# neuroailab/CounterfactualWorldModels

Measured on AMD Instinct MI355X. Metric: predicted frames/sec (2x224x224, ViT-B/8), higher is better.
Workload: dtype bf16; 1 GPU; ViT-base VMAE 8x8, batch=32 synthetic frame pairs (BASELINE configs[1]); predictor=base_8x8patch_2frames_1tube, per_gpu_batch=32, global_batch=32, n_vis=792, mode=parity, lanes=2 (the batch runs as two half batches on two HIP streams inside the library), arithmetic=split-bf16 (hi+lo) MFMA operands, 3 MFMAs/product, fp32 accumulate, parallelism=dp1 (independent frame pairs per rank, no collective), weights=random-init (deterministic synthetic generator)

## Files before the change

counterfactualworldmodels_amd/_lib.py:

```python
from __future__ import annotations

import ctypes as C
import os
import threading
from typing import Optional

import torch

from . import build as _build

MODE_FAST = 1
MODE_PARITY = 2
ERR_INVALID = -1
ERR_HIP = -2
ERR_MASK = -3
KCLASS_GEMM = 0
KCLASS_ATTENTION = 1
KCLASS_GEMM_WIDE = 2
KCLASS_GEMM_NARROW = 3
KCLASS_LAYERNORM, KCLASS_PATCH_GATHER, KCLASS_FILL_MASK, KCLASS_UNEMBED = 4, 5, 6, 7
KCLASS_CROSS_ATTN, KCLASS_SMALL_ATTN = 8, 9

_MODES = {"fast": MODE_FAST, "parity": MODE_PARITY, MODE_FAST: MODE_FAST, MODE_PARITY: MODE_PARITY}

# ... 446 lines not shown
DEV_FLOW_MOTION_STRIDED, DEV_FLOW_MOTION_TILE, DEV_FLOW_MOTION_ROWS16, DEV_FLOW_MOTION_ROWS32, DEV_FLOW_MOTION_ROWS64 = range(5)
DEV_FLOW_COUNT_PLANES, DEV_FLOW_COUNT_PLANES_VEC, DEV_FLOW_COUNT_PACKED, DEV_FLOW_COUNT_PACKED_VEC = range(4)
DEV_FLOW_FINISH_V1, DEV_FLOW_FINISH_V4 = range(2)
DEV_FLOW_ZERO_PLANES, DEV_FLOW_ZERO_PLANES_VEC, DEV_FLOW_ZERO_SCATTER = range(3)
DEV_FLOW_PACK_TRANSPOSE = 0


def new_dev_conj_args(cls):
    a = cls()
    a.struct_size = C.sizeof(cls)
    return a


def new_dev_raft_conv_args() -> CwmDevRaftConvArgs:
    a = CwmDevRaftConvArgs()
    a.struct_size = C.sizeof(CwmDevRaftConvArgs)
    return a


def new_forward_args() -> CwmForwardArgs:
    a = CwmForwardArgs()
    a.struct_size = C.sizeof(CwmForwardArgs)
    return a


def new_conj_forward_args() -> CwmConjForwardArgs:
    a = CwmConjForwardArgs()
    a.struct_size = C.sizeof(CwmConjForwardArgs)
    return a


class CwmKernelStats(C.Structure):
    _fields_ = [("launches", C.c_int64), ("total_ms", C.c_double), ("total_flops", C.c_double)]


SIGNATURES = {
    "cwm_model_create": (C.c_int, [C.POINTER(CwmConfig), C.POINTER(C.c_void_p)]),
    "cwm_model_destroy": (None, [C.c_void_p]),
    "cwm_model_load_weight": (C.c_int, [C.c_void_p, C.c_char_p, C.c_void_p, C.c_int, C.POINTER(C.c_int64), C.c_int]),
    "cwm_model_missing_weights": (C.c_int, [C.c_void_p, C.c_char_p, C.c_int]),
    "cwm_forward": (C.c_int, [C.c_void_p, C.POINTER(CwmForwardArgs)]),
    "cwm_model_set_lanes": (C.c_int, [C.c_void_p, C.c_int]),
    "cwm_model_set_ragged": (C.c_int, [C.c_void_p, C.c_int]),
    "cwm_model_set_option": (C.c_int, [C.c_void_p, C.c_char_p, C.c_int]),
    "cwm_conj_set_option": (C.c_int, [C.c_void_p, C.c_char_p, C.c_int]),
    "cwm_conj_create": (C.c_int, [C.POINTER(CwmConjConfig), C.POINTER(C.c_void_p)]),
    "cwm_conj_create_ex": (C.c_int, [C.POINTER(CwmConjConfig), C.POINTER(CwmConjVariant), C.POINTER(C.c_void_p)]),
    "cwm_conj_destroy": (None, [C.c_void_p]),
    "cwm_conj_load_weight": (C.c_int, [C.c_void_p, C.c_char_p, C.c_void_p, C.c_int, C.POINTER(C.c_int64), C.c_int]),
    "cwm_conj_missing_weights": (C.c_int, [C.c_void_p, C.c_char_p, C.c_int]),
    "cwm_conj_forward": (C.c_int, [C.c_void_p, C.POINTER(CwmConjForwardArgs)]),
    "cwm_conj_set_lanes": (C.c_int, [C.c_void_p, C.c_int]),
    "cwm_conj_timing_enable": (C.c_int, [C.c_void_p, C.c_int, C.c_int]),
    "cwm_conj_timing_collect": (C.c_int, [C.c_void_p, C.c_int, C.POINTER(CwmKernelStats)]),
    "cwm_timing_enable": (C.c_int, [C.c_void_p, C.c_int, C.c_int]),
    "cwm_timing_collect": (C.c_int, [C.c_void_p, C.c_int, C.POINTER(CwmKernelStats)]),
    "cwm_split_bf16": (C.c_int, [C.c_void_p, C.c_int64, C.c_void_p, C.c_void_p, C.c_void_p]),
    "cwm_linear": (
        C.c_int,
        [C.c_void_p, C.c_void_p, C.c_void_p, C.c_void_p, C.c_void_p, C.c_int, C.c_int, C.c_int, C.c_int, C.c_int, C.c_void_p],
    ),
    "cwm_attention": (C.c_int, [C.c_void_p, C.c_void_p, C.c_int, C.c_int, C.c_int, C.c_int, C.c_void_p]),
    "cwm_attention_ragged": (C.c_int, [C.c_void_p, C.c_void_p, C.c_void_p, C.c_int, C.c_int, C.c_int, C.c_int, C.c_void_p]),
    "cwm_layernorm": (C.c_int, [C.c_void_p, C.c_void_p, C.c_void_p, C.c_void_p, C.c_int, C.c_int, C.c_float, C.c_void_p]),
    "cwm_mask_to_perm": (C.c_int, [C.c_void_p, C.c_int, C.c_int, C.c_int, C.c_void_p, C.c_void_p]),
    "cwm_unembed": (
        C.c_int,
        [C.c_void_p, C.c_void_p, C.c_void_p, C.c_int, C.c_int, C.c_int, C.c_int, C.c_int, C.c_int, C.c_int, C.c_void_p, C.c_void_p],
    ),
    "cwm_mask_row_counts": (C.c_int, [C.c_void_p, C.c_int, C.c_int, C.c_void_p, C.c_void_p]),
    "cwm_mask_flip_picks": (C.c_int, [C.c_void_p, C.c_int, C.c_int, C.c_void_p, C.c_int, C.c_void_p]),
    "cwm_prompt_table_expand": (C.c_int, [C.c_void_p] + [C.c_int] * 5 + [C.c_void_p] * 4),
    "cwm_shift_prompts": (
        C.c_int,
        [C.c_void_p] + [C.c_int] * 9 + [C.c_void_p] * 6,
    ),
    "cwm_multi_shift_prompts": (
        C.c_int,
        [C.c_void_p] + [C.c_int] * 10 + [C.c_void_p, C.c_void_p, C.c_int, C.c_void_p, C.c_int] + [C.c_void_p] * 3,
    ),
    "cwm_flow_features": (C.c_int, [C.c_void_p, C.POINTER(C.c_int64)] + [C.c_int] * 6 + [C.c_void_p, C.c_void_p]),
    "cwm_flow_cov": (C.c_int, [C.c_void_p] + [C.c_int] * 6 + [C.c_void_p] * 4),
    "cwm_flow_transform_work_bytes": (C.c_size_t, [C.c_int, C.c_int, C.c_int]),
    "cwm_flow_transform": (C.c_int, [C.c_void_p] + [C.c_int] * 5 + [C.c_float, C.c_int, C.c_int, C.c_float, C.c_void_p, C.c_void_p]),
    "cwm_flow_motion_work_bytes": (C.c_size_t, [C.c_int, C.c_int]),
    "cwm_flow_motion_sum": (C.c_int, [C.c_void_p, C.POINTER(C.c_int64)] + [C.c_int] * 6 + [C.c_float, C.c_void_p, C.c_void_p, C.c_void_p]),
    "cwm_flow_map_finish": (C.c_int, [C.c_void_p, C.c_int, C.c_int, C.c_float, C.c_int, C.c_float, C.c_void_p]),
    "cwm_flow_filter_stats": (C.c_int, [C.c_void_p, C.POINTER(C.c_int64)] + [C.c_int] * 5 + [C.c_void_p, C.POINTER(C.c_int64), C.c_int, C.c_int] + [C.c_float] * 3
                              + [C.c_void_p] * 5),
    "cwm_flow_filter_apply": (C.c_int, [C.c_void_p, C.POINTER(C.c_int64)] + [C.c_int] * 5 + [C.c_void_p, C.c_void_p]),
    "cwm_flow_filter_pack": (C.c_int, [C.c_void_p, C.POINTER(C.c_int64)] + [C.c_int] * 5 + [C.c_void_p, C.c_void_p, C.c_void_p]),
    "cwm_comm_load": (C.c_int, [C.c_char_p]),
    "cwm_comm_version": (C.c_int, []),
    "cwm_comm_unique_id": (C.c_int, [C.c_void_p]),
    "cwm_comm_init": (C.c_int, [C.c_int, C.c_int, C.c_void_p, C.POINTER(C.c_void_p)]),
    "cwm_comm_destroy": (None, [C.c_void_p]),
    "cwm_comm_rank": (C.c_int, [C.c_void_p]),
    "cwm_comm_size": (C.c_int, [C.c_void_p]),
    "cwm_broadcast": (C.c_int, [C.c_void_p, C.c_void_p, C.c_size_t, C.c_int, C.c_void_p]),
    "cwm_allgather": (C.c_int, [C.c_void_p, C.c_void_p, C.c_void_p, C.c_size_t, C.c_void_p]),
    "cwm_allgatherv": (C.c_int, [C.c_void_p, C.c_void_p, C.c_void_p, C.POINTER(C.c_size_t), C.POINTER(C.c_size_t), C.c_void_p]),
    "cwm_allreduce_sum_f32": (C.c_int, [C.c_void_p, C.c_void_p, C.c_size_t, C.c_void_p]),
    "cwm_raft_create": (C.c_int, [C.POINTER(C.c_void_p)]),
    "cwm_raft_destroy": (None, [C.c_void_p]),
    "cwm_raft_load_weight": (C.c_int, [C.c_void_p, C.c_char_p, C.c_void_p, C.c_int, C.POINTER(C.c_int64), C.c_int]),
    "cwm_raft_missing_weights": (C.c_int, [C.c_void_p, C.c_char_p, C.c_int]),
    "cwm_raft_forward": (C.c_int, [C.c_void_p, C.POINTER(CwmRaftForwardArgs)]),
    "cwm_raft_forward_ex": (C.c_int, [C.c_void_p, C.POINTER(CwmRaftForwardExArgs)]),
    "cwm_raft_corr_lookup": (C.c_int, [C.c_void_p, C.c_void_p, C.c_void_p, C.c_int, C.c_int, C.c_int, C.c_void_p, C.c_void_p]),
    "cwm_raft_set_corr": (C.c_int, [C.c_void_p, C.c_int]),
    "cwm_raft_workspace_bytes": (C.c_int, [C.c_void_p, C.POINTER(C.c_uint64)]),
    "cwm_raft_corr_lookup_on_the_fly": (C.c_int, [C.c_void_p, C.c_void_p, C.c_void_p, C.c_int, C.c_int, C.c_int, C.c_void_p, C.c_void_p]),
    "cwm_raft_convex_upsample": (C.c_int, [C.c_void_p, C.c_void_p, C.c_int, C.c_int, C.c_int, C.c_void_p, C.c_void_p]),
    "cwm_raft_head_project": (C.c_int, [C.c_void_p, C.c_void_p, C.c_void_p, C.c_int64, C.c_void_p, C.c_void_p]),
    "cwm_raft_convex_upsample1": (C.c_int, [C.c_void_p, C.c_void_p, C.c_int, C.c_int, C.c_int, C.c_void_p, C.c_void_p]),
    "cwm_raft_forward_interpolate": (C.c_int, [C.c_void_p, C.c_int64, C.c_int64, C.c_int, C.c_int, C.c_int, C.c_void_p, C.c_void_p]),
    "cwm_last_error": (C.c_char_p, []),
    "cwm_version": (C.c_char_p, []),
    "cwm_source_hash": (C.c_char_p, []),
    "cwm_compiler_version": (C.c_char_p, []),
}
DEV_SIGNATURES = {
    "cwm_gemm_tile_override": (C.c_int, [C.c_int] * 6),
    "cwm_dev_gemm_plan": (C.c_int, [C.c_int] * 8 + [C.POINTER(CwmDevGemmPlanOut)]),
    "cwm_dev_flow_forms": (C.c_int, [C.POINTER(C.c_int64)] + [C.c_int] * 5 + [C.c_uint64, C.c_uint64, C.c_int, C.POINTER(C.c_int64), C.c_uint64, C.c_int, C.POINTER(CwmDevFlowFormsOut)]),
    "cwm_bench_gemm": (C.c_int, [C.c_int, C.c_int, C.c_int, C.c_int, C.c_int, C.c_int, C.POINTER(C.c_double)]),
    "cwm_bench_attention": (C.c_int, [C.c_int, C.c_int, C.c_int, C.c_int, C.c_int, C.POINTER(C.c_double)]),
    "cwm_debug_set": (C.c_int, [C.c_char_p, C.c_int]),
    "cwm_debug_get": (C.c_int, [C.c_char_p, C.POINTER(C.c_int)]),
    "cwm_dev_raft_conv": (C.c_int, [C.POINTER(CwmDevRaftConvArgs)]),
    "cwm_dev_raft_corr_lookup_operand": (C.c_int, [C.c_void_p, C.c_void_p, C.c_void_p, C.c_int, C.c_int, C.c_int, C.c_int, C.c_void_p, C.c_void_p]),
    "cwm_dev_raft_corr_lookup_on_the_fly_operand": (C.c_int, [C.c_void_p, C.c_void_p, C.c_void_p, C.c_int, C.c_int, C.c_int, C.c_int, C.c_void_p, C.c_void_p]),
    "cwm_dev_raft_instnorm_stats": (C.c_int, [C.c_void_p, C.c_int, C.c_int, C.c_int, C.c_float, C.c_void_p, C.c_void_p]),
    "cwm_dev_raft_residual_join": (C.c_int, [C.POINTER(CwmDevConvSrc), C.POINTER(CwmDevConvSrc), C.c_int, C.c_int, C.c_void_p, C.c_void_p]),
    "cwm_dev_raft_cnet_split": (C.c_int, [C.c_void_p, C.c_int64, C.c_void_p, C.c_void_p, C.c_void_p]),
    "cwm_dev_raft_motion_finish": (C.c_int, [C.c_void_p, C.c_void_p, C.c_int64, C.c_int, C.c_int, C.c_void_p]),
    "cwm_dev_raft_gru_update": (C.c_int, [C.c_void_p, C.c_void_p, C.c_void_p, C.c_int64, C.c_void_p]),
    "cwm_dev_raft_flow_update": (C.c_int, [C.c_void_p, C.c_void_p, C.c_int, C.c_int64, C.c_void_p]),
    "cwm_dev_gather": (C.c_int, [C.POINTER(CwmDevGatherArgs)]),
    "cwm_dev_conj_cross_attention": (C.c_int, [C.POINTER(CwmDevConjCrossAttentionArgs)]),
    "cwm_dev_conj_small_attention": (C.c_int, [C.POINTER(CwmDevConjSmallAttentionArgs)]),
    "cwm_dev_conj_pad": (C.c_int, [C.POINTER(CwmDevConjPadArgs)]),
    "cwm_dev_gemm": (C.c_int, [C.POINTER(CwmDevGemmArgs)]),
    "cwm_dev_attention": (C.c_int, [C.POINTER(CwmDevAttentionArgs)]),
    "cwm_dev_layernorm": (C.c_int, [C.POINTER(CwmDevLayernormArgs)]),
    "cwm_dev_fill_mask_tokens": (C.c_int, [C.c_void_p] * 4 + [C.c_int] * 4 + [C.c_void_p]),
    "cwm_dev_unembed": (C.c_int, [C.c_void_p, C.c_void_p] + [C.c_int64] * 3 + [C.c_void_p] + [C.c_int] * 7 + [C.c_void_p, C.c_void_p]),
    "cwm_dev_gather_ragged": (C.c_int, [C.POINTER(CwmDevGatherArgs), C.c_int, C.c_void_p]),
    "cwm_dev_attention_ragged": (C.c_int, [C.POINTER(CwmDevAttentionArgs), C.c_void_p]),
    "cwm_dev_fill_mask_tokens_ragged": (C.c_int, [C.c_void_p] * 5 + [C.c_int] * 4 + [C.c_void_p]),
    "cwm_dev_unembed_ragged": (C.c_int, [C.c_void_p, C.c_void_p] + [C.c_int64] * 3 + [C.c_void_p] + [C.c_int] * 8 + [C.c_void_p, C.c_void_p]),
}

OPTION_KEYS = ("gemm_tile", "gemm_debug", "gemm_staged", "gemm_direct", "attn_kernel", "attn_remap", "attn_tail", "attn_ksplit", "prune_last_block", "index_fused",
               "min_lane_rows", "conj_ctx_stream", "conj_attn")
GEMM_DEBUG_TIMING_ONLY = 1 | 2 | 8


def validate_option(key: str, value: int) -> None:
    if key not in OPTION_KEYS:
        raise CwmHipError(-1, "unknown option %s (known: %s)" % (key, ", ".join(OPTION_KEYS)))
    if key == "gemm_debug" and int(value) & GEMM_DEBUG_TIMING_ONLY:
        raise CwmHipError(-1, "gemm_debug bits 1, 2 and 8 are timing-only ablations (wrong outputs): development library only (cwm_debug_set)")


_lib: Optional[C.CDLL] = None
_dev_lib: Optional[C.CDLL] = None
_lock = threading.Lock()


class CwmHipError(RuntimeError):
    def __init__(self, code: int, msg: str):
        super().__init__(msg)
        self.code = code


def library_path() -> str:
    return os.environ.get("CWM_HIP_LIB", _build.LIB_PATH)


def get_lib() -> C.CDLL:
    global _lib
    if _lib is not None:
        return _lib
    with _lock:
        if _lib is not None:
            return _lib
        path = library_path()
        if not os.path.exists(path):
            try:
                _build.build_library()
            except Exception as e:
                raise RuntimeError(
                    "libcwm_hip.so is missing at %s and could not be built (%s). "
                    "Run `python -m counterfactualworldmodels_amd.build`." % (path, e)
                )
        lib = _bind(path)
        if path == _build.LIB_PATH and os.path.isdir(_build.CSRC):
            want = _build.source_hash()
            if lib.cwm_source_hash().decode() != want:
                try:
                    _build.build_library(force=False)
                except Exception as e:
                    raise RuntimeError("libcwm_hip.so at %s was built from other sources (%s != %s) and could not be rebuilt: %s"
                                       % (path, lib.cwm_source_hash().decode(), want, e))
                import _ctypes

                _ctypes.dlclose(lib._handle)
                lib = _bind(path)
                if lib.cwm_source_hash().decode() != want:
                    raise RuntimeError("libcwm_hip.so still does not match the sources after a rebuild")
        _warn_if_unlinted_compiler(lib)
        _lib = lib
        return lib


def _warn_if_unlinted_compiler(lib) -> None:
    try:
        rec = _build.lint_record().get("hipcc")
        comp = lib.cwm_compiler_version().decode()
    except Exception:
        return
    if rec and comp and rec != comp:
        import warnings

        warnings.warn("libcwm_hip.so was compiled by `%s`, but the ISA lint of its hand-counted waits last passed on `%s`: run `python tools/asm_lds_lint.py --record` "
                      "(and the GPU soak, tests/test_soak_gpu.py) before trusting this build" % (comp, rec), RuntimeWarning, stacklevel=3)


def dev_library_path() -> str:
    p = library_path()
    return os.environ.get("CWM_HIP_DEV_LIB", _build.DEV_LIB_PATH if p == _build.LIB_PATH else p[:-3] + "_dev.so")


def get_dev_lib() -> C.CDLL:
    global _dev_lib
    if _dev_lib is not None:
        return _dev_lib
    get_lib()
    with _lock:
        if _dev_lib is None:
            path = dev_library_path()
            if not os.path.exists(path):
                raise RuntimeError("libcwm_hip_dev.so is missing at %s: run `python -m counterfactualworldmodels_amd.build`" % path)
            lib = _bind(path, dict(SIGNATURES, **DEV_SIGNATURES))
            if path == _build.DEV_LIB_PATH and os.path.isdir(_build.CSRC) and lib.cwm_source_hash().decode() != _build.source_hash():
                raise RuntimeError("libcwm_hip_dev.so at %s was built from other sources than the tree holds: run `python -m counterfactualworldmodels_amd.build`" % path)
            _dev_lib = lib
    return _dev_lib


def _bind(path: str, signatures=None) -> C.CDLL:
    lib = C.CDLL(path)
    for name, (res, args) in (signatures or SIGNATURES).items():
        try:
            fn = getattr(lib, name)
        except AttributeError:
            if name == "cwm_source_hash":
                lib.cwm_source_hash = lambda: b"pre-hash"
                continue
            raise
        fn.restype = res
        fn.argtypes = args
    return lib


def check(rc: int, lib: Optional[C.CDLL] = None) -> None:
    if rc != 0:
        msg = (lib or get_lib()).cwm_last_error()
        if not msg and lib is None and _dev_lib is not None:
            msg = _dev_lib.cwm_last_error()
        raise CwmHipError(rc, (msg.decode() if msg else "") + " [cwm_hip rc=%d]" % rc)


def require_gpu() -> None:
    if not torch.cuda.is_available():
        raise RuntimeError(
            "counterfactualworldmodels_amd runs its predictor on an AMD GPU through libcwm_hip.so; "
            "no HIP device is visible and there is no CPU fallback."
        )


def ptr(t: Optional[torch.Tensor]) -> Optional[int]:
    return None if t is None else t.data_ptr()


def current_stream_handle(device=None) -> int:
    return torch.cuda.current_stream(device).cuda_stream
```

counterfactualworldmodels_amd/csrc/dev.hip:

```cpp
#include <atomic>
#include <map>
#include <mutex>
#include <tuple>

#include "../../include/cwm_hip_dev.h"
#include "engine.h"
#include "flow_view.h"

using namespace cwm;

void cwm_set_pretend_device(int d);

namespace {
__global__ void fill_random_bf16_kernel(bf16* dst, int64_t n, unsigned seed, float scale) {
    const int64_t i = (int64_t)blockIdx.x * blockDim.x + threadIdx.x;
    if (i >= n) return;
    unsigned x = (unsigned)i * 2654435761u + seed;
    x ^= x >> 16; x *= 0x7feb352du; x ^= x >> 15; x *= 0x846ca68bu; x ^= x >> 16;
    dst[i] = (bf16)(((float)(x & 0xFFFF) / 32768.0f - 1.0f) * scale);
}
__global__ void fill_random_f32_kernel(float* dst, int64_t n, unsigned seed, float scale) {
    const int64_t i = (int64_t)blockIdx.x * blockDim.x + threadIdx.x;
    if (i >= n) return;
    unsigned x = (unsigned)i * 2654435761u + seed;
// ... 425 lines not shown
    }
    if (rc) return rc;
    CWM_HIP_CHECK(hipStreamSynchronize(s));
    return CWM_OK;
}

extern "C" int cwm_dev_gather(const cwm_dev_gather_args* args) { return dev_gather(args, false, 0, nullptr); }

extern "C" int cwm_dev_gather_ragged(const cwm_dev_gather_args* args, int n_vis_min, int32_t* counts_dev) { return dev_gather(args, true, n_vis_min, counts_dev); }

namespace {
template <int PLANES>
__global__ void stage_operand_kernel(const float* src, int64_t rows, int K, bf16* out) {
    const int64_t i = ((int64_t)blockIdx.x * blockDim.x + threadIdx.x) * 4;
    if (i >= rows * K) return;
    const int64_t r = i / K;
    store_operand4<PLANES>(out, r, K, (int)(i - r * K), *reinterpret_cast<const f32x4*>(src + i));
}
int stage_operand(const float* src, int64_t rows, int K, bf16* out, int planes, hipStream_t s) {
    const unsigned grid = (unsigned)((rows * K / 4 + 255) / 256);
    if (planes == 2)
        hipLaunchKernelGGL(stage_operand_kernel<2>, dim3(grid), dim3(256), 0, s, src, rows, K, out);
    else
        hipLaunchKernelGGL(stage_operand_kernel<1>, dim3(grid), dim3(256), 0, s, src, rows, K, out);
    CWM_HIP_CHECK(hipGetLastError());
    return 0;
}
}

extern "C" int cwm_dev_conj_cross_attention(const cwm_dev_conj_cross_attention_args* args) {
    CWM_REQUIRE(args && args->struct_size == sizeof(cwm_dev_conj_cross_attention_args),
                "cwm_dev_conj_cross_attention: args->struct_size must be sizeof(cwm_dev_conj_cross_attention_args)");
    const cwm_dev_conj_cross_attention_args& a = *args;
    hipStream_t s = (hipStream_t)a.stream;
    CWM_REQUIRE(a.mode == CWM_MODE_FAST || a.mode == CWM_MODE_PARITY, "cwm_dev_conj_cross_attention: bad mode");
    const int planes = a.mode == CWM_MODE_PARITY ? 2 : 1;
    CWM_REQUIRE(a.impl == CWM_DEV_CONJ_VALU || a.impl == CWM_DEV_CONJ_MFMA, "cwm_dev_conj_cross_attention: unknown impl %d", a.impl);
    const bool mfma = a.impl == CWM_DEV_CONJ_MFMA;
    CWM_REQUIRE(a.roles >= 1 && a.roles <= 3 && (mfma || a.roles == 3), "cwm_dev_conj_cross_attention: roles = %d (MFMA: 1, 2 or 3; VALU: 3)", a.roles);
    CWM_REQUIRE(a.qk && a.v && a.qk_src && a.v_src && a.y && a.y_src, "cwm_dev_conj_cross_attention: null argument");
    CWM_REQUIRE(a.B > 0 && a.N > 0 && a.M > 0 && a.heads > 0 && a.head_dim > 0 && (int64_t)a.B * a.N * 4 * a.heads * a.head_dim < (1ll << 31),
                "cwm_dev_conj_cross_attention: bad geometry");
    const int D = a.heads * a.head_dim;
    CWM_REQUIRE(D % 32 == 0, "cwm_dev_conj_cross_attention: operand rows of %d columns (need a multiple of 32)", D);
    if (mfma) {
        CWM_REQUIRE(cross_attention_mfma_ok(a.head_dim, a.M), "cwm_dev_conj_cross_attention: the MFMA form has no kernel for head_dim %d, M %d", a.head_dim, a.M);
        CWM_REQUIRE(cross_attention_mfma_fits(a.B, a.N, a.heads, a.head_dim), "cwm_dev_conj_cross_attention: too large for the MFMA form's 32-bit offsets");
    } else {
        CWM_REQUIRE(cross_attention_ok(a.M, a.head_dim), "cwm_dev_conj_cross_attention: the VALU form refuses M %d, head_dim %d (%zu bytes of LDS)", a.M, a.head_dim,
                    cross_attention_lds_bytes(a.M, a.head_dim));
    }
    const int64_t rows = (int64_t)a.B * a.N;
    Scratch sc;
    CrossAttnParams p;
    memset(&p, 0, sizeof(p));
    p.qk = a.qk, p.v = a.v, p.qk_src = a.qk_src, p.v_src = a.v_src;
    p.B = a.B, p.N = a.N, p.M = a.M, p.heads = a.heads, p.head_dim = a.head_dim, p.scale = a.scale;
    p.y = (bf16*)a.y, p.y_plane = rows * D, p.y_src = (bf16*)a.y_src, p.y_src_plane = (int64_t)a.B * a.M * D;
    int rc;
    if (mfma) {
        bf16* qk_op = sc.get<bf16>((size_t)rows * 2 * D * planes);
        bf16* v_op = sc.get<bf16>((size_t)rows * D * planes);
        p.partial = sc.get<float>(cross_attention_mfma_partial_floats(a.B, a.heads, a.M, a.head_dim));
        CWM_REQUIRE(qk_op && v_op && p.partial, "cwm_dev_conj_cross_attention: out of device memory");
        if ((rc = stage_operand(a.qk, rows, 2 * D, qk_op, planes, s)) || (rc = stage_operand(a.v, rows, D, v_op, planes, s))) return rc;
        p.qk_op = qk_op, p.v_op = v_op;
        if ((rc = launch_cross_attention_mfma_roles(p, planes, s, s, a.roles))) return rc;
    } else {
        p.scores_t = sc.get<float>((size_t)a.B * a.heads * a.M * a.N);
        p.partial = sc.get<float>(cross_attention_partial_floats(a.B, a.heads, a.M, a.head_dim));
        CWM_REQUIRE(p.scores_t && p.partial, "cwm_dev_conj_cross_attention: out of device memory");
        if ((rc = launch_cross_attention(p, planes, s))) return rc;
    }
    CWM_HIP_CHECK(hipStreamSynchronize(s));
    return CWM_OK;
}

extern "C" int cwm_dev_conj_small_attention(const cwm_dev_conj_small_attention_args* args) {
    CWM_REQUIRE(args && args->struct_size == sizeof(cwm_dev_conj_small_attention_args),
                "cwm_dev_conj_small_attention: args->struct_size must be sizeof(cwm_dev_conj_small_attention_args)");
    const cwm_dev_conj_small_attention_args& a = *args;
    hipStream_t s = (hipStream_t)a.stream;
    CWM_REQUIRE(a.mode == CWM_MODE_FAST || a.mode == CWM_MODE_PARITY, "cwm_dev_conj_small_attention: bad mode");
    const int planes = a.mode == CWM_MODE_PARITY ? 2 : 1;
    CWM_REQUIRE(a.impl == CWM_DEV_CONJ_VALU || a.impl == CWM_DEV_CONJ_MFMA, "cwm_dev_conj_small_attention: unknown impl %d", a.impl);
    CWM_REQUIRE(a.qkv && a.o && a.B > 0 && a.heads > 0, "cwm_dev_conj_small_attention: bad argument");
    CWM_REQUIRE(a.n_tok > 0 && a.n_tok <= 64 && a.head_dim > 0 && a.head_dim <= 64, "cwm_dev_conj_small_attention: needs n_tok <= 64 and head_dim <= 64 (got %d, %d)",
                a.n_tok, a.head_dim);
    CWM_REQUIRE(a.impl == CWM_DEV_CONJ_VALU || small_attention_mfma_ok(a.n_tok, a.head_dim), "cwm_dev_conj_small_attention: the MFMA form needs head_dim 32 (got %d)",
                a.head_dim);
    const int D = a.heads * a.head_dim;
    CWM_REQUIRE(D % 4 == 0 && a.ldo % 32 == 0 && a.ldo >= D, "cwm_dev_conj_small_attention: %d columns in operand rows of ldo = %d (a multiple of 32)", D, a.ldo);
    SmallAttnParams p;
    memset(&p, 0, sizeof(p));
    p.qkv = a.qkv;
    p.B = a.B, p.n_tok = a.n_tok, p.heads = a.heads, p.head_dim = a.head_dim;
    p.o = (bf16*)a.o, p.o_plane = (int64_t)a.B * a.n_tok * a.ldo, p.ldo = a.ldo;
    if (int rc = a.impl == CWM_DEV_CONJ_MFMA ? launch_small_attention_mfma(p, planes, s) : launch_small_attention(p, planes, s)) return rc;
    CWM_HIP_CHECK(hipStreamSynchronize(s));
    return CWM_OK;
}

extern "C" int cwm_dev_conj_pad(const cwm_dev_conj_pad_args* args) {
    CWM_REQUIRE(args && args->struct_size == sizeof(cwm_dev_conj_pad_args), "cwm_dev_conj_pad: args->struct_size must be sizeof(cwm_dev_conj_pad_args)");
    const cwm_dev_conj_pad_args& a = *args;
    hipStream_t s = (hipStream_t)a.stream;
    CWM_REQUIRE(a.B > 0, "cwm_dev_conj_pad: bad batch");
    int rc = 0;
    if (a.kind == CWM_DEV_CONJ_PAD_MASK) {
        CWM_REQUIRE(a.mask && a.ext_mask && a.N > 0 && a.P >= 0 && a.vmax >= 0, "cwm_dev_conj_pad: bad pad-mask argument");
        rc = launch_pad_mask(a.mask, a.B, a.N, a.P, a.vmax, a.ext_mask, s);
    } else if (a.kind == CWM_DEV_CONJ_FIX_PAD_ROWS) {
        CWM_REQUIRE(a.x && a.perm && a.token && a.n_rows > 0 && a.D > 0 && a.perm_stride >= a.n_rows && a.n_real >= 0, "cwm_dev_conj_pad: bad fix-pad-rows argument");
        rc = launch_fix_pad_rows(a.x, a.perm, a.B, a.perm_stride, a.n_rows, a.n_real, a.D, a.token, s);
    } else if (a.kind == CWM_DEV_CONJ_ZERO_PAD_OUT_ROWS) {
        CWM_REQUIRE(a.x && a.perm && a.n_rows > 0 && a.D > 0 && a.n_vis >= 0 && a.perm_stride >= a.n_vis + a.n_rows && a.n_real >= 0,
                    "cwm_dev_conj_pad: bad zero-pad-out-rows argument");
        rc = launch_zero_pad_out_rows(a.x, a.perm, a.B, a.perm_stride, a.n_vis, a.n_rows, a.n_real, a.D, s);
    } else if (a.kind == CWM_DEV_CONJ_IMU_APPEND_DUMMY) {
        CWM_REQUIRE(a.imu && a.mask && a.dummy && a.out && a.ext_mask && a.C > 0 && a.L > 0 && a.T > 0 && a.N > 0, "cwm_dev_conj_pad: bad append-dummy argument");
        rc = launch_imu_append_dummy(a.imu, a.mask, a.dummy, a.B, a.C, a.L, a.T, a.N, a.out, a.ext_mask, s);
    } else {
        CWM_REQUIRE(false, "cwm_dev_conj_pad: unknown kind %d", a.kind);
    }
    if (rc) return rc;
    CWM_HIP_CHECK(hipStreamSynchronize(s));
    return CWM_OK;
}

extern "C" int cwm_dev_gemm(const cwm_dev_gemm_args* args) {
    CWM_REQUIRE(args && args->struct_size == sizeof(cwm_dev_gemm_args), "cwm_dev_gemm: args->struct_size must be sizeof(cwm_dev_gemm_args)");
    const cwm_dev_gemm_args& a = *args;
    hipStream_t s = (hipStream_t)a.stream;
    CWM_REQUIRE(a.mode == CWM_MODE_FAST || a.mode == CWM_MODE_PARITY, "cwm_dev_gemm: bad mode");
    const int planes = a.mode == CWM_MODE_PARITY ? 2 : 1;
    CWM_REQUIRE(a.a && a.w && a.M > 0 && a.N > 0 && a.K > 0 && a.epi >= EPI_F32 && a.epi <= EPI_QKV, "cwm_dev_gemm: bad argument");
    CWM_REQUIRE(a.rows_in >= 0 && a.out_row_offset >= 0 && (a.rows_in > 0 || (!a.resid_rowmap && a.out_row_offset == 0)),
                "cwm_dev_gemm: a row map or row offset needs rows_in > 0");
    if (a.rows_in > 0) {
        CWM_REQUIRE(a.M % a.rows_in == 0 && a.rows_in + a.out_row_offset <= a.rows_out, "cwm_dev_gemm: %d rows as samples of %d rows at offset %d of %d", a.M,
                    a.rows_in, a.out_row_offset, a.rows_out);
        CWM_REQUIRE(!a.resid_rowmap || a.map_stride >= a.rows_in, "cwm_dev_gemm: a residual row map of %d entries per sample for %d rows", a.map_stride, a.rows_in);
    }
    GemmParams p;
    memset(&p, 0, sizeof(p));
    p.M = a.M; p.N = a.N; p.K = p.lda = round_up(a.K, 64);
    p.epi = a.epi;
    p.rows_in = a.rows_in; p.rows_out = a.rows_out; p.out_row_offset = a.out_row_offset; p.map_stride = a.map_stride; p.resid_rowmap = a.resid_rowmap;
    if (a.epi == EPI_F32) {
        CWM_REQUIRE(a.C && a.ldc >= a.N && (!a.resid || a.ldr >= a.N), "cwm_dev_gemm: the fp32 output needs C and rows of at least N columns");
        CWM_REQUIRE(!a.resid_rowmap || a.resid, "cwm_dev_gemm: a residual row map without a residual");
        p.C = a.C; p.ldc = a.ldc; p.resid = a.resid; p.ldr = a.ldr;
    } else if (a.epi == EPI_QKV) {
        CWM_REQUIRE(a.q_out && a.k_out && a.v_out && a.heads > 0 && a.head_dim > 0 && a.n_tok > 0 && a.N == 3 * a.heads * a.head_dim && a.M % a.n_tok == 0,
                    "cwm_dev_gemm: the Q/K/V scatter needs the three outputs, N = 3 * heads * head_dim and whole samples of n_tok rows");
        CWM_REQUIRE(planes == 1 || a.qk_plane >= (int64_t)a.M * a.heads * a.head_dim, "cwm_dev_gemm: the lo plane would overlap the hi plane");
        p.q_out = (bf16*)a.q_out; p.k_out = (bf16*)a.k_out; p.v_out = (bf16*)a.v_out; p.qk_plane = a.qk_plane;
        p.qkv_dim = a.heads * a.head_dim; p.heads = a.heads; p.head_dim = a.head_dim; p.n_tok = a.n_tok; p.q_scale = a.q_scale;
    } else {
        CWM_REQUIRE(a.out && a.ldo >= a.N, "cwm_dev_gemm: the operand output needs out and rows of at least N columns");
        p.out_hi = (bf16*)a.out; p.ldo = a.ldo;
    }
    p.tune = &thread_tuning();
    GemmPlan plan;
    if (int rc = gemm_plan(p, planes, 0, gemm_cu_count(), &plan)) return rc;
    if (a.plan_forms) a.plan_forms[0] = plan.staged, a.plan_forms[1] = plan.direct;
    Scratch sc;
    LinearOperands op;
    if (int rc = stage_linear_operands(sc, "cwm_dev_gemm", a.a, a.w, a.bias, a.M, a.N, a.K, planes, s, &op)) return rc;
    p.A = op.A; p.W = op.W;
    p.bias = a.bias ? op.bias : nullptr;
    if (int rc = launch_gemm(p, planes, s)) return rc;
    CWM_HIP_CHECK(hipStreamSynchronize(s));
    return CWM_OK;
}

static int dev_attention(const cwm_dev_attention_args* args, const int* key_len) {
    CWM_REQUIRE(args && args->struct_size == sizeof(cwm_dev_attention_args), "cwm_dev_attention: args->struct_size must be sizeof(cwm_dev_attention_args)");
    const cwm_dev_attention_args& a = *args;
    CWM_REQUIRE(!key_len || a.n_q == 0, "cwm_dev_attention: per-row key counts (key_len) go with queries over all rows (n_q = 0), got n_q = %d", a.n_q);
    hipStream_t s = (hipStream_t)a.stream;
    CWM_REQUIRE(a.mode == CWM_MODE_FAST || a.mode == CWM_MODE_PARITY, "cwm_dev_attention: bad mode");
    const int planes = a.mode == CWM_MODE_PARITY ? 2 : 1;
    CWM_REQUIRE(a.qkv && a.o && a.B > 0 && a.N > 0 && a.H > 0, "cwm_dev_attention: bad argument");
    CWM_REQUIRE(a.q_off >= 0 && a.n_q >= 0 && a.q_off + a.n_q <= a.N && (a.n_q > 0 || a.q_off == 0), "cwm_dev_attention: query rows [%d, %d) of %d tokens", a.q_off,
                a.q_off + a.n_q, a.N);
    const int D = a.H * 64;
    CWM_REQUIRE(a.ldo >= D && a.ldo % (planes == 2 ? 32 : 4) == 0, "cwm_dev_attention: %d columns in operand rows of ldo = %d (a multiple of 32 in parity mode, of 4 in fast mode)",
                D, a.ldo);
    const int64_t qk_plane = (int64_t)a.B * a.N * D;
    Scratch sc;
    bf16* q = sc.get<bf16>(2 * qk_plane);
    bf16* k = sc.get<bf16>(2 * qk_plane);
    bf16* v = sc.get<bf16>(2 * qk_plane);
    CWM_REQUIRE(q && k && v, "cwm_dev_attention: out of device memory");
    if (int rc = launch_qkv_scatter(a.qkv, a.B, a.N, a.H, 0.125f, q, k, v, qk_plane, s)) return rc;
    AttnParams p;
    memset(&p, 0, sizeof(p));
    p.q = q; p.k = k; p.v = v; p.qk_plane = qk_plane;
    p.o = (bf16*)a.o; p.o_plane = (int64_t)a.B * (a.n_q ? a.n_q : a.N) * a.ldo; p.ldo = a.ldo;
    p.n_tok = a.N; p.heads = a.H; p.batch = a.B;
    p.q_off = a.q_off; p.n_q = a.n_q;
    p.key_len = key_len;
    p.tune = &thread_tuning();
    if (int rc = launch_attention(p, planes, s)) return rc;
    CWM_HIP_CHECK(hipStreamSynchronize(s));
    return CWM_OK;
}

extern "C" int cwm_dev_attention(const cwm_dev_attention_args* args) { return dev_attention(args, nullptr); }

extern "C" int cwm_dev_attention_ragged(const cwm_dev_attention_args* args, const int32_t* key_len_dev) {
    CWM_REQUIRE(key_len_dev, "cwm_dev_attention_ragged: null key_len_dev");
    return dev_attention(args, key_len_dev);
}

extern "C" int cwm_dev_layernorm(const cwm_dev_layernorm_args* args) {
    CWM_REQUIRE(args && args->struct_size == sizeof(cwm_dev_layernorm_args), "cwm_dev_layernorm: args->struct_size must be sizeof(cwm_dev_layernorm_args)");
    const cwm_dev_layernorm_args& a = *args;
    hipStream_t s = (hipStream_t)a.stream;
    CWM_REQUIRE(a.mode == CWM_MODE_FAST || a.mode == CWM_MODE_PARITY, "cwm_dev_layernorm: bad mode");
    const int planes = a.mode == CWM_MODE_PARITY ? 2 : 1;
    CWM_REQUIRE(a.x && a.gamma && a.beta && a.out && a.rows > 0 && a.D > 0 && a.ldx >= a.D, "cwm_dev_layernorm: bad argument");
    CWM_REQUIRE(a.rows_out_per_b >= 0 && a.in_offset >= 0 &&
                    (a.rows_out_per_b == 0 ? a.in_offset == 0 : a.rows % a.rows_out_per_b == 0 && a.in_offset + a.rows_out_per_b <= a.rows_in_per_b),
                "cwm_dev_layernorm: %d rows as samples of %d rows at offset %d of %d", a.rows, a.rows_out_per_b, a.in_offset, a.rows_in_per_b);
    LayerNormParams ln;
    memset(&ln, 0, sizeof(ln));
    ln.x = a.x; ln.ldx = a.ldx; ln.gamma = a.gamma; ln.beta = a.beta; ln.eps = a.eps; ln.D = a.D; ln.rows = a.rows;
    ln.rows_out_per_b = a.rows_out_per_b; ln.rows_in_per_b = a.rows_in_per_b; ln.in_offset = a.in_offset;
    ln.out = (bf16*)a.out; ln.out_plane = (int64_t)a.rows * a.ldo; ln.ldo = a.ldo; ln.out_f32 = a.out_f32;
    if (int rc = launch_layernorm(ln, planes, s)) return rc;
    CWM_HIP_CHECK(hipStreamSynchronize(s));
    return CWM_OK;
}

extern "C" int cwm_dev_fill_mask_tokens(float* x_full_dev, const float* mask_token_dev, const float* pos_dev, const int32_t* perm_dev, int B, int Nt, int n_vis,
                                        int D, void* stream) {
    CWM_REQUIRE(x_full_dev && mask_token_dev && pos_dev && perm_dev && B > 0 && D > 0 && n_vis >= 0 && n_vis <= Nt, "cwm_dev_fill_mask_tokens: bad argument");
    if (int rc = launch_fill_mask_tokens(x_full_dev, mask_token_dev, pos_dev, perm_dev, B, Nt, n_vis, D, (hipStream_t)stream)) return rc;
    CWM_HIP_CHECK(hipStreamSynchronize((hipStream_t)stream));
    return CWM_OK;
}

extern "C" int cwm_dev_fill_mask_tokens_ragged(float* x_full_dev, const float* mask_token_dev, const float* pos_dev, const int32_t* perm_dev,
                                               const int32_t* counts_dev, int B, int Nt, int n_vis_min, int D, void* stream) {
    CWM_REQUIRE(x_full_dev && mask_token_dev && pos_dev && perm_dev && B > 0 && Nt > 0 && D > 0, "cwm_dev_fill_mask_tokens_ragged: bad argument");
    if (int rc = launch_fill_mask_tokens_ragged(x_full_dev, mask_token_dev, pos_dev, perm_dev, counts_dev, B, Nt, n_vis_min, D, (hipStream_t)stream)) return rc;
    CWM_HIP_CHECK(hipStreamSynchronize((hipStream_t)stream));
    return CWM_OK;
}

static int dev_unembed(const float* y_tokens_dev, const float* x_dev, int64_t x_stride_b, int64_t x_stride_c, int64_t x_stride_t, const uint8_t* mask_dev, int B, int T,
                       int C, int H, int W, int P, int n_vis_min, int n_vis, float* out_dev, void* stream) {
    CWM_REQUIRE(y_tokens_dev && x_dev && mask_dev && out_dev && B > 0 && T > 0 && C > 0 && H > 0 && W > 0, "cwm_dev_unembed: bad argument");
    CWM_REQUIRE(P > 0 && H % P == 0 && W % P == 0, "cwm_dev_unembed: image size must be divisible by the patch size");
    CWM_REQUIRE(x_stride_c >= (int64_t)H * W && x_stride_t >= 0 && x_stride_b >= 0, "cwm_dev_unembed: channel planes of %d x %d pixels at a stride of %lld", H, W,
                (long long)x_stride_c);
    const int Nt = T * (H / P) * (W / P);
    CWM_REQUIRE(n_vis >= 0 && n_vis <= Nt, "cwm_dev_unembed: n_vis = %d of %d tokens", n_vis, Nt);
    hipStream_t s = (hipStream_t)stream;
    Scratch sc;
    int* perm = sc.get<int>((size_t)B * Nt);
    int* rank = sc.get<int>((size_t)B * Nt);
    int* err = sc.get<int>(4, true);
    int* counts = sc.get<int>((size_t)B);
    CWM_REQUIRE(perm && rank && err && counts, "cwm_dev_unembed: out of device memory");
    int rc;
    if ((rc = n_vis_min > 0 ? launch_mask_to_perm_ragged(mask_dev, B, Nt, n_vis_min, n_vis, perm, err, counts, s) : launch_mask_to_perm(mask_dev, B, Nt, n_vis, perm, err, s)))
        return rc;
    const int y0 = n_vis_min > 0 ? n_vis_min : n_vis;
    if ((rc = launch_perm_to_rank(perm, rank, B, Nt, s))) return rc;
    UnembedParams u;
    memset(&u, 0, sizeof(u));
    u.y = y_tokens_dev; u.x = x_dev; u.sb = x_stride_b; u.st = x_stride_t; u.sc = x_stride_c;
    u.mask = mask_dev; u.rank = rank; u.B = B; u.T = T; u.C = C; u.H = H; u.W = W; u.P = P; u.n_vis = y0; u.Nm = Nt - y0; u.out = out_dev;
    if ((rc = launch_unembed(u, s))) return rc;
    int herr = 0;
    CWM_HIP_CHECK(hipMemcpyAsync(&herr, err, sizeof(int), hipMemcpyDeviceToHost, s));
    CWM_HIP_CHECK(hipStreamSynchronize(s));
    if (herr) {
        if (n_vis_min > 0)
            cwm_set_error("mask rows do not all have between %d and n_vis=%d visible tokens", n_vis_min, n_vis);
        else
            cwm_set_error("mask rows do not all have n_vis=%d visible tokens", n_vis);
        return CWM_ERR_MASK;
    }
    return CWM_OK;
}

extern "C" int cwm_dev_unembed(const float* y_tokens_dev, const float* x_dev, int64_t x_stride_b, int64_t x_stride_c, int64_t x_stride_t, const uint8_t* mask_dev,
                               int B, int T, int C, int H, int W, int P, int n_vis, float* out_dev, void* stream) {
    return dev_unembed(y_tokens_dev, x_dev, x_stride_b, x_stride_c, x_stride_t, mask_dev, B, T, C, H, W, P, 0, n_vis, out_dev, stream);
}

extern "C" int cwm_dev_unembed_ragged(const float* y_tokens_dev, const float* x_dev, int64_t x_stride_b, int64_t x_stride_c, int64_t x_stride_t, const uint8_t* mask_dev,
                                      int B, int T, int C, int H, int W, int P, int n_vis_min, int n_vis, float* out_dev, void* stream) {
    CWM_REQUIRE(n_vis_min > 0, "cwm_dev_unembed_ragged: n_vis_min = %d (a ragged batch has a least count > 0)", n_vis_min);
    return dev_unembed(y_tokens_dev, x_dev, x_stride_b, x_stride_c, x_stride_t, mask_dev, B, T, C, H, W, P, n_vis_min, n_vis, out_dev, stream);
}
```

counterfactualworldmodels_amd/csrc/elementwise.hip:

```cpp
#include "common.h"
#include "kernels.h"
#include <algorithm>

namespace cwm {

template <int PLANES>
__global__ __launch_bounds__(256) void layernorm_kernel(const LayerNormParams p) {
    constexpr int MAXI = 2;
    const int lane = threadIdx.x & 63;
    const int r = blockIdx.x * 4 + (threadIdx.x >> 6);
    if (r >= p.rows) return;
    int in_row = r;
    if (p.rows_out_per_b > 0) {
        const int b = r / p.rows_out_per_b;
        in_row = b * p.rows_in_per_b + p.in_offset + (r - b * p.rows_out_per_b);
    }
    const float* x = p.x + (size_t)in_row * p.ldx;
    f32x4 v[MAXI][2];
    float s = 0.f;
#pragma unroll
    for (int i = 0; i < MAXI; ++i) {
        const int idx = lane * 8 + i * 512;
        if (idx < p.D) {
            v[i][0] = *reinterpret_cast<const f32x4*>(x + idx);
// ... 228 lines not shown
}

template <int PLANES>
__global__ __launch_bounds__(256) void index_gather_kernel(const PatchGatherParams p, const uint8_t* __restrict__ mask, int n_vis, int* __restrict__ perm_out,
                                                           int* __restrict__ rank_out, int* __restrict__ err_rows, int n_vis_min, int* __restrict__ counts) {
    extern __shared__ int vis_tab[];
    __shared__ int wave_tot[4];
    const int b = blockIdx.y, t = threadIdx.x;
    const int L = p.perm_stride ? p.perm_stride : p.Nt;
    const uint8_t* m = mask + (size_t)b * L;
    const int nw = min((int)gridDim.x, 256);
    const bool writer = (t % nw) == (int)blockIdx.x;
    int* pr = perm_out + (size_t)b * L;
    int* rk = rank_out ? rank_out + (size_t)b * L : nullptr;
    const bool vec = (L & 15) == 0 && L <= 256 * 32 && ((uintptr_t)mask & 15) == 0;
    const int per = !vec ? (L + 255) / 256 : L <= 256 * 16 ? 16 : 32;
    const int lo = min(t * per, L), hi = min(lo + per, L);
    u32x4 w0 = u32x4{0x01010101u, 0x01010101u, 0x01010101u, 0x01010101u}, w1 = w0;
    int c = 0;
    if (vec) {
        if (lo < L) w0 = *reinterpret_cast<const u32x4*>(m + lo);
        if (per == 32 && lo + 16 < L) w1 = *reinterpret_cast<const u32x4*>(m + lo + 16);
        auto zero_bytes = [](unsigned x) {
            const unsigned y = (x & 0x7F7F7F7Fu) + 0x7F7F7F7Fu;
            return __popc(~(y | x | 0x7F7F7F7Fu));
        };
#pragma unroll
        for (int q = 0; q < 4; ++q) c += zero_bytes(w0[q]) + zero_bytes(w1[q]);
    } else {
        for (int i = lo; i < hi; ++i) c += (m[i] == 0);
    }
    int total_vis;
    int v = block_exclusive_scan256(c, wave_tot, total_vis);
    auto emit = [&](int i, bool visible) {
        if (visible) {
            if (v < p.n_rows) vis_tab[v] = i;
            if (writer) {
                pr[v] = i;
                if (rk) rk[i] = v;
            }
            ++v;
        } else if (writer) {
            const int pos = total_vis + (i - v);
            pr[pos] = i;
            if (rk) rk[i] = pos;
        }
    };
    if (vec) {
#pragma unroll
        for (int k = 0; k < 32; ++k) {
            if (k < hi - lo) {
                const unsigned word = k < 16 ? w0[(k >> 2) & 3] : w1[(k >> 2) & 3];
                emit(lo + k, ((word >> (8 * (k & 3))) & 0xFFu) == 0);
            }
        }
    } else {
        for (int i = lo; i < hi; ++i) emit(i, m[i] == 0);
    }
    if (blockIdx.x == 0 && t == 0) {
        err_rows[b] = (n_vis_min > 0 ? (total_vis < n_vis_min || total_vis > n_vis) : total_vis != n_vis) ? 1 : 0;
        if (counts) counts[b] = total_vis;
    }
    __syncthreads();

    const int per_row = p.C * p.P;
    const int total = p.n_rows * per_row;
    for (int gid = blockIdx.x * 256 + t; gid < total; gid += gridDim.x * 256) {
        const int i = gid / per_row;
        patch_gather_item<PLANES>(p, b, (int64_t)b * p.n_rows + i, gid - i * per_row, i < total_vis ? vis_tab[i] : p.Nt);
    }
}

int launch_index_gather(const PatchGatherParams& p, const uint8_t* mask, int n_vis, int* perm, int* rank, int* err_rows, int planes, hipStream_t stream,
                        int n_vis_min, int* counts) {
    CWM_REQUIRE(n_vis_min == 0 || (n_vis_min > 0 && n_vis_min <= n_vis && counts), "index_gather: ragged rows need 0 < n_vis_min <= n_vis and a count array");
    CWM_REQUIRE(p.P % 4 == 0 && p.W % 4 == 0, "index_gather: patch size and width must be multiples of 4");
    CWM_REQUIRE(p.C == 3 || !p.normalize, "index_gather: imagenet normalisation needs 3 channels");
    CWM_REQUIRE(p.ld >= p.C * p.P * p.P && p.ld % 4 == 0, "index_gather: bad ld");
    CWM_REQUIRE(mask && perm && err_rows && p.n_rows > 0 && p.n_rows <= 12000, "index_gather: bad argument (rows per sample: %d)", p.n_rows);
    const int per_sample = (p.n_rows * p.C * p.P + 255) / 256;
    const dim3 grid((unsigned)per_sample, (unsigned)p.B);
    const size_t smem = (size_t)p.n_rows * sizeof(int);
    if (planes == 1)
        hipLaunchKernelGGL(index_gather_kernel<1>, grid, dim3(256), smem, stream, p, mask, n_vis, perm, rank, err_rows, n_vis_min, counts);
    else
        hipLaunchKernelGGL(index_gather_kernel<2>, grid, dim3(256), smem, stream, p, mask, n_vis, perm, rank, err_rows, n_vis_min, counts);
    CWM_HIP_CHECK(hipGetLastError());
    return 0;
}

__global__ __launch_bounds__(256) void fill_mask_tokens4_kernel(float* x_full, const float* mask_token, const float* pos, const int* perm, int Nt,
                                                                 int n_vis, int D, int64_t rows, int64_t rows_q) {
    const int d4 = D / 4;
    const int64_t gid = (int64_t)blockIdx.x * blockDim.x + threadIdx.x;
    if (gid >= rows_q * d4) return;
    const int64_t r0 = gid / d4;
    const int c4 = (int)(gid - r0 * d4);
    const int nm = Nt - n_vis;
    const float4 mt = *reinterpret_cast<const float4*>(mask_token + c4 * 4);
    constexpr int R = 8;
    size_t orow[R];
    int tau[R];
    bool live[R];
#pragma unroll
    for (int i = 0; i < R; ++i) {
        const int64_t row = r0 + i * rows_q;
        live[i] = row < rows;
        const int64_t rr = live[i] ? row : 0;
        const int b = (int)(rr / nm), j = (int)(rr - (int64_t)b * nm);
        orow[i] = (size_t)b * Nt + n_vis + j;
        tau[i] = perm[orow[i]];
    }
    float4 pe[R];
#pragma unroll
    for (int i = 0; i < R; ++i) pe[i] = *reinterpret_cast<const float4*>(pos + (size_t)tau[i] * D + c4 * 4);
#pragma unroll
    for (int i = 0; i < R; ++i)
        if (live[i]) *reinterpret_cast<float4*>(x_full + orow[i] * D + c4 * 4) = make_float4(mt.x + pe[i].x, mt.y + pe[i].y, mt.z + pe[i].z, mt.w + pe[i].w);
}

int launch_fill_mask_tokens(float* x_full, const float* mask_token, const float* pos, const int* perm, int B, int Nt, int n_vis, int D, hipStream_t stream) {
    CWM_REQUIRE(D % 4 == 0, "fill_mask_tokens: D must be a multiple of 4");
    const int64_t rows = (int64_t)B * (Nt - n_vis), rows_q = (rows + 7) / 8;
    if (rows == 0) return 0;
    hipLaunchKernelGGL(fill_mask_tokens4_kernel, dim3((unsigned)((rows_q * (D / 4) + 255) / 256)), dim3(256), 0, stream, x_full, mask_token, pos, perm, Nt,
                       n_vis, D, rows, rows_q);
    CWM_HIP_CHECK(hipGetLastError());
    return 0;
}

__global__ __launch_bounds__(256) void fill_mask_tokens_ragged_kernel(float* x_full, const float* mask_token, const float* pos, const int* perm,
                                                                      const int* counts, int Nt, int n_vis_min, int D, int64_t total) {
    const int d4 = D / 4;
    const int64_t gid = (int64_t)blockIdx.x * blockDim.x + threadIdx.x;
    if (gid >= total) return;
    const int64_t row = gid / d4;
    const int c4 = (int)(gid - row * d4);
    const int nm = Nt - n_vis_min;
    const int b = (int)(row / nm), j = n_vis_min + (int)(row - (int64_t)b * nm);
    if (j < counts[b]) return;
    const size_t orow = (size_t)b * Nt + j;
    const float4 mt = *reinterpret_cast<const float4*>(mask_token + c4 * 4);
    const float4 pe = *reinterpret_cast<const float4*>(pos + (size_t)perm[orow] * D + c4 * 4);
    *reinterpret_cast<float4*>(x_full + orow * D + c4 * 4) = make_float4(mt.x + pe.x, mt.y + pe.y, mt.z + pe.z, mt.w + pe.w);
}

int launch_fill_mask_tokens_ragged(float* x_full, const float* mask_token, const float* pos, const int* perm, const int* counts, int B, int Nt, int n_vis_min,
                                   int D, hipStream_t stream) {
    CWM_REQUIRE(D % 4 == 0 && counts && n_vis_min > 0 && n_vis_min <= Nt, "fill_mask_tokens (ragged): bad argument");
    const int64_t total = (int64_t)B * (Nt - n_vis_min) * (D / 4);
    if (total == 0) return 0;
    hipLaunchKernelGGL(fill_mask_tokens_ragged_kernel, dim3((unsigned)((total + 255) / 256)), dim3(256), 0, stream, x_full, mask_token, pos, perm, counts, Nt,
                       n_vis_min, D, total);
    CWM_HIP_CHECK(hipGetLastError());
    return 0;
}

struct __attribute__((packed, aligned(4))) Float4A4 {
    float v[4];
};

__global__ __launch_bounds__(256) void unembed_kernel(const UnembedParams p) {
    const int w4 = p.W / 4;
    const int64_t total = (int64_t)p.B * p.T * p.C * p.H * w4;
    const int64_t gid = (int64_t)blockIdx.x * blockDim.x + threadIdx.x;
    if (gid >= total) return;
    int64_t r = gid;
    const int x4 = (int)(r % w4); r /= w4;
    const int y = (int)(r % p.H); r /= p.H;
    const int c = (int)(r % p.C); r /= p.C;
    const int t = (int)(r % p.T);
    const int b = (int)(r / p.T);
    const int x0 = x4 * 4;
    const int gw = p.W / p.P;
    const int n = (p.H / p.P) * gw;
    const int Nt = p.T * n;
    const int tau = t * n + (y / p.P) * gw + (x0 / p.P);
    Float4A4 o;
    if (p.mask[(size_t)b * Nt + tau]) {
        const int j = max(p.rank[(size_t)b * Nt + tau] - p.n_vis, 0);
        const float* yp = p.y + ((size_t)b * p.Nm + j) * (p.P * p.P * p.C) + ((y % p.P) * p.P + (x0 % p.P)) * p.C + c;
        o = Float4A4{{yp[0], yp[p.C], yp[2 * p.C], yp[3 * p.C]}};
    } else {
        o = *reinterpret_cast<const Float4A4*>(p.x + b * p.sb + t * p.st + c * p.sc + (int64_t)y * p.W + x0);
    }
    *reinterpret_cast<Float4A4*>(p.out + ((((size_t)b * p.T + t) * p.C + c) * p.H + y) * p.W + x0) = o;
}

__global__ __launch_bounds__(256) void unembed3_kernel(const UnembedParams p) {
    const int w4 = p.W / 4, hh = p.H / 2;
    const int64_t total = (int64_t)p.B * p.T * hh * w4;
    const int64_t gid = (int64_t)blockIdx.x * blockDim.x + threadIdx.x;
    if (gid >= total) return;
    int64_t r = gid;
    const int x4 = (int)(r % w4); r /= w4;
    const int y0 = (int)(r % hh); r /= hh;
    const int t = (int)(r % p.T);
    const int b = (int)(r / p.T);
    const int x0 = x4 * 4;
    const int gw = p.W / p.P;
    const int n = (p.H / p.P) * gw;
    const int Nt = p.T * n;
    float4 o[2][3];
#pragma unroll
    for (int k = 0; k < 2; ++k) {
        const int y = y0 + k * hh;
        const int tau = t * n + (y / p.P) * gw + (x0 / p.P);
        if (p.mask[(size_t)b * Nt + tau]) {
            const int j = max(p.rank[(size_t)b * Nt + tau] - p.n_vis, 0);
            const float4* yp = reinterpret_cast<const float4*>(p.y + ((size_t)b * p.Nm + j) * (p.P * p.P * 3) + ((y % p.P) * p.P + (x0 % p.P)) * 3);
            const float4 a = yp[0], bb = yp[1], c = yp[2];
            o[k][0] = make_float4(a.x, a.w, bb.z, c.y);
            o[k][1] = make_float4(a.y, bb.x, bb.w, c.z);
            o[k][2] = make_float4(a.z, bb.y, c.x, c.w);
        } else {
            const float* src = p.x + b * p.sb + t * p.st + (int64_t)y * p.W + x0;
#pragma unroll
            for (int c = 0; c < 3; ++c) o[k][c] = *reinterpret_cast<const float4*>(src + c * p.sc);
        }
    }
#pragma unroll
    for (int k = 0; k < 2; ++k) {
        float* dst = p.out + (((size_t)b * p.T + t) * 3 * p.H + y0 + k * hh) * p.W + x0;
#pragma unroll
        for (int c = 0; c < 3; ++c) {
            const f32x4 v = f32x4{o[k][c].x, o[k][c].y, o[k][c].z, o[k][c].w};
            __builtin_nontemporal_store(v, reinterpret_cast<f32x4*>(dst + (size_t)c * p.H * p.W));
        }
    }
}

int launch_unembed(const UnembedParams& p, hipStream_t stream) {
    CWM_REQUIRE(p.P % 4 == 0 && p.W % 4 == 0, "unembed: patch size and width must be multiples of 4");
    if (p.C == 3 && p.H % 2 == 0 && (((uintptr_t)p.y | (uintptr_t)p.out | (uintptr_t)p.x) & 15) == 0 && (p.sc % 4 == 0) && (p.sb % 4 == 0) && (p.st % 4 == 0)) {
        const int64_t total3 = (int64_t)p.B * p.T * (p.H / 2) * (p.W / 4);
        hipLaunchKernelGGL(unembed3_kernel, dim3((unsigned)((total3 + 255) / 256)), dim3(256), 0, stream, p);
        CWM_HIP_CHECK(hipGetLastError());
        return 0;
    }
    const int64_t total = (int64_t)p.B * p.T * p.C * p.H * (p.W / 4);
    hipLaunchKernelGGL(unembed_kernel, dim3((unsigned)((total + 255) / 256)), dim3(256), 0, stream, p);
    CWM_HIP_CHECK(hipGetLastError());
    return 0;
}

__global__ __launch_bounds__(256) void shift_prompts_x_kernel(const ShiftPromptParams p) {
    const int w4 = p.W / 4, h4 = p.H / 4;
    const int64_t total = (int64_t)p.B * p.S * p.T * p.C * h4 * w4;
    const int64_t gid = (int64_t)blockIdx.x * blockDim.x + threadIdx.x;
    if (gid >= total) return;
    int64_t r = gid;
    const int x4 = (int)(r % w4); r /= w4;
    const int yq = (int)(r % h4); r /= h4;
    const int c = (int)(r % p.C); r /= p.C;
    const int t = (int)(r % p.T);
    const int i = (int)(r / p.T);
    const int b = i / p.S;
    const int x0 = x4 * 4, y = yq * 4;
    int ft = p.fix_passive == 1 ? 0 : t;
    int sy = y, sx = x0;
    const int gw = p.W / p.P, gh = p.H / p.P, n = gh * gw;
    if (t == p.frame) {
        const int dy = p.shifts[2 * i], dx = p.shifts[2 * i + 1];
        const int pi = y / p.P - dy, pj = x0 / p.P - dx;
        if (pi >= 0 && pi < gh && pj >= 0 && pj < gw && p.active[(size_t)i * p.T * n + (size_t)p.frame * n + pi * gw + pj] == 0) {
            sy = y - dy * p.P;
            sx = x0 - dx * p.P;
        }
    }
    if (p.fix_passive == 2) {
        if (p.masks[(size_t)i * p.T * n + (size_t)t * n + (sy / p.P) * gw + sx / p.P] == 0) ft = 0;
    }
    const float* src = p.x + ((((size_t)b * p.T + ft) * p.C + c) * p.H + sy) * p.W + sx;
    float* dst = p.x_out + ((((size_t)i * p.T + t) * p.C + c) * p.H + y) * p.W + x0;
    f32x4 v[4];
#pragma unroll
    for (int k = 0; k < 4; ++k) v[k] = *reinterpret_cast<const f32x4*>(src + (size_t)k * p.W);
#pragma unroll
    for (int k = 0; k < 4; ++k) __builtin_nontemporal_store(v[k], reinterpret_cast<f32x4*>(dst + (size_t)k * p.W));
}

__global__ __launch_bounds__(256) void shift_prompts_mask_kernel(const ShiftPromptParams p) {
    const int gw = p.W / p.P, gh = p.H / p.P, n = gh * gw, Nt = p.T * n;
    const int64_t total = (int64_t)p.B * p.S * Nt;
    const int64_t gid = (int64_t)blockIdx.x * blockDim.x + threadIdx.x;
    if (gid >= total) return;
    const int i = (int)(gid / Nt), tau = (int)(gid - (int64_t)i * Nt);
    const int t = tau / n, hw = tau - t * n;
    const uint8_t act = p.active[gid];
    const uint8_t m1 = act ? p.masks[gid] : 1;
    uint8_t mp = act;
    if (t == p.frame) {
        const int dy = p.shifts[2 * i], dx = p.shifts[2 * i + 1];
        const int pi = hw / gw - dy, pj = hw % gw - dx;
        mp = (pi >= 0 && pi < gh && pj >= 0 && pj < gw) ? p.active[(size_t)i * Nt + (size_t)t * n + pi * gw + pj] : 1;
    }
    p.mask_out[gid] = (m1 && mp) ? 1 : 0;
}

__global__ __launch_bounds__(256) void prompt_table_expand_kernel(const int* __restrict__ table, int S, int gh, int gw, int T, int frame, uint8_t* __restrict__ active,
                                                                  uint8_t* __restrict__ passive, int* __restrict__ shifts) {
    const int n = gh * gw;
    const int Nt = T * n;
    const int64_t gid = (int64_t)blockIdx.x * blockDim.x + threadIdx.x;
    if (gid >= (int64_t)S * Nt) return;
    const int i = (int)(gid / Nt), tau = (int)(gid - (int64_t)i * Nt);
// ... 223 lines not shown
```

counterfactualworldmodels_amd/csrc/engine.h:

```cpp
#pragma once
#include <math.h>
#include <stdio.h>
#include <string.h>

#include <algorithm>
#include <map>
#include <string>
#include <vector>

#include "../../include/cwm_hip.h"
#include "common.h"
#include "kernels.h"

namespace cwm {

static inline int round_up(int v, int m) { return (v + m - 1) / m * m; }

struct LinearW {
    bf16* w = nullptr;
    bf16* w_il = nullptr;
    int64_t plane = 0;
    int N = 0, K = 0, Npad = 0, Kpad = 0;
    float* bias = nullptr;
};

struct BlockW {
    float *ln1_g = nullptr, *ln1_b = nullptr, *ln2_g = nullptr, *ln2_b = nullptr;
    LinearW qkv, proj, fc1, fc2;
};

enum SlotKind { SLOT_MATRIX, SLOT_VECTOR, SLOT_IGNORED };

struct Slot {
    SlotKind kind = SLOT_VECTOR;
    std::vector<int64_t> shape;
    LinearW* lin = nullptr;
    float* dst = nullptr;
    int repeat = 1;
    int64_t numel = 0;
    bool loaded = false;
    bool optional = false;
};

struct EventPair {
    hipEvent_t a, b;
    double flops;
    int sub;
};

struct KernelTimer {
    bool enabled = false;
    std::vector<EventPair> pool;
    size_t used = 0;
    cwm_kernel_stats acc = {0, 0.0, 0.0};
};

struct StreamBuffers {
    bf16 *hbuf = nullptr, *gbuf = nullptr, *qbuf = nullptr, *kbuf = nullptr, *vbuf = nullptr;
    float* qkv_f32 = nullptr;
};

struct StreamW {
    int enc_dim = 0, dec_dim = 0, enc_heads = 0, dec_heads = 0, n_tok = 0, max_pad = 0, out_dim = 0, embed_k = 0, embed_kpad = 0;
    std::vector<BlockW> enc, dec;
    LinearW embed, e2d, head;
    float *enc_norm_g = nullptr, *enc_norm_b = nullptr, *dec_norm_g = nullptr, *dec_norm_b = nullptr;
    float *mask_token = nullptr, *null_enc = nullptr;
    float *pos_enc_ext = nullptr, *pos_dec_ext = nullptr;
    int n_slots() const { return n_tok + max_pad; }
};

struct StreamWs {
    uint8_t* ext_mask = nullptr;
    int* perm = nullptr;
    bf16* tokens_in = nullptr;
    float *x_enc = nullptr, *x_dec = nullptr;
    StreamBuffers sb;
};

template <typename Visit>
int for_each_stream_buffer(const StreamW& S, StreamWs& w, int vcap, int mlp_ratio, bool small, Visit&& visit) {
    const size_t rows_e = (size_t)vcap, rows_d = (size_t)S.n_slots();
    const size_t act = std::max(rows_e * S.enc_dim, rows_d * S.dec_dim);
    int rc;
    if ((rc = visit(w.ext_mask, rows_d)) || (rc = visit(w.perm, rows_d)) || (rc = visit(w.tokens_in, 2 * rows_e * S.embed_kpad)) ||
        (rc = visit(w.x_enc, rows_e * S.enc_dim)) || (rc = visit(w.x_dec, rows_d * S.dec_dim)) || (rc = visit(w.sb.hbuf, 2 * act)) ||
        (rc = visit(w.sb.gbuf, 2 * act * mlp_ratio)))
        return rc;
    if (small) return visit(w.sb.qkv_f32, 3 * act);
    if ((rc = visit(w.sb.qbuf, 2 * act)) || (rc = visit(w.sb.kbuf, 2 * act))) return rc;
    return visit(w.sb.vbuf, 2 * act);
}

constexpr int kMinLaneRows = 3000;
constexpr int kMinLaneRowsConj = 12000;

struct Lanes {
    static constexpr int kMax = 4;
    hipStream_t streams[kMax - 1] = {};
    hipEvent_t ev_fork = nullptr, ev_join[kMax - 1] = {};
    int forked = 1;
    ~Lanes();
    int fork(hipStream_t caller, int n_lanes);
    hipStream_t stream(int l, hipStream_t caller) const { return l == 0 ? caller : streams[l - 1]; }
    int join(hipStream_t caller);
};

struct Engine {
    int device = 0;
    int overlapped = 0;
    Tuning tune = thread_tuning();
    float ln_eps = 1e-6f;
    std::map<std::string, Slot> slots;
    uint64_t loads = 0;
    std::vector<void*> allocs;
    std::vector<void*> ws_allocs;
    uint64_t ws_bytes = 0;
    KernelTimer timers[CWM_KCLASS_COUNT];
    struct SplitKWs {
        float* slabs;
        unsigned* counts;
        uint64_t last_use;
    };
    uint64_t splitk_clock = 0;
    static constexpr size_t kMaxSplitKStreams = 8;
    std::map<hipStream_t, SplitKWs> splitk_ws;

    ~Engine();
    int alloc(void** p, size_t bytes, bool zero, bool workspace);
    template <typename T>
    int ws(T** p, size_t count) {
        void* v = nullptr;
        if (int rc = alloc(&v, count * sizeof(T), true, true)) return rc;
        *p = (T*)v;
        return 0;
    }
    int free_workspace();

    int make_linear(LinearW& L, int N, int K, bool bias);
    int make_vec(float** v, int n);
    void add_matrix_slot(const std::string& key, LinearW* L, std::vector<int64_t> shape);
    void add_vec_slot(const std::string& key, float* dst, std::vector<int64_t> shape, int repeat = 1);
    void add_ignored_slot(const std::string& key, std::vector<int64_t> shape);
    int make_block(BlockW& b, const std::string& pre, int D, int hidden);
    int make_sinusoid(float** dst, int n_pos, int d, int extra_rows = 0);
    int make_pos_embedding_f32(float** dst, int n_pos, int d, int extra_rows = 0);
    int make_stream(StreamW& S, const std::string& pre, int embed_k, std::vector<int64_t> embed_shape, int depth_e, int depth_d, int mlp_ratio,
                    bool sinusoid_f64, bool null_tokens);

    int load_weight(const char* key, const float* data, int on_device, const int64_t* shape, int ndim);
    int missing_weights(char* buf, int buflen);
    int require_weights(const char* fn);
    int set_option(const char* fn, const char* key, int value);

    int run_gemm(const GemmParams& p, int planes, hipStream_t s);
    int attach_splitk_workspace(GemmParams& p, hipStream_t s);
    int run_attention(const AttnParams& p, int planes, hipStream_t s);
    int run_layernorm(const LayerNormParams& p, int planes, hipStream_t s);
    int run_patch_gather(const PatchGatherParams& p, int planes, hipStream_t s);
    int run_index_gather(const PatchGatherParams& p, const uint8_t* mask, int n_vis, int* perm, int* rank, int* err_rows, int planes, hipStream_t s,
                         int n_vis_min = 0, int* counts = nullptr);
    int run_fill_mask_tokens(float* x_full, const float* mask_token, const float* pos, const int* perm, int B, int Nt, int n_vis, int D, hipStream_t s);
    int run_unembed(const UnembedParams& p, hipStream_t s);
    template <typename F>
    int timed(int kclass, double work, hipStream_t s, F&& launch) {
        EventPair* e = nullptr;
        if (int rc = timer_begin(kclass, work, s, &e)) return rc;
        if (int rc = launch()) return rc;
        return timer_end(e, s);
    }
    int timer_begin(int kclass, double work, hipStream_t s, EventPair** out);
    int timer_end(EventPair* e, hipStream_t s);
    int layernorm_to(const float* x, int rows, int D, const float* g, const float* b, bf16* out, int planes, hipStream_t s);
    int linear_f32(const bf16* A, int rows, int K, const LinearW& L, float* C, const float* resid, int planes, hipStream_t s);
    int linear_operand(const bf16* A, int rows, int K, const LinearW& L, bf16* out, int planes, hipStream_t s);
    int linear_gelu(const bf16* A, int rows, int K, const LinearW& L, bf16* out, int planes, hipStream_t s);
    int run_mlp(const float* ln_g, const float* ln_b, const LinearW& fc1, const LinearW& fc2, float* x, int B, int n_tok, int D, int planes, StreamBuffers& sb,
                hipStream_t s, int n_keep = 0);
    int run_block(const BlockW& w, float* x, int B, int n_tok, int D, int H, int planes, StreamBuffers& sb, hipStream_t s, int n_keep = 0,
                  const int* key_len = nullptr);
    int run_block_small(const BlockW& w, float* x, int B, int n_tok, int D, int H, int planes, StreamBuffers& sb, hipStream_t s);
    int embed_stream(const StreamW& S, const StreamWs& w, int B, int n_vis, int planes, hipStream_t s);
    int to_decoder(const StreamW& S, const StreamWs& w, int B, int n_vis, int planes, hipStream_t s, const int* counts = nullptr, int n_vis_min = 0);
    int head_rows(const StreamW& S, const StreamWs& w, int B, int n_out, float* out, int planes, hipStream_t s);

    int timing_enable(int kclass, int enable);
    int timing_collect(int kclass, cwm_kernel_stats* out);
};

template <typename Args>
int copy_args(Args& dst, const Args* src, size_t min_size, const char* fn, const char* note = "") {
    CWM_REQUIRE(src->struct_size >= min_size && src->struct_size <= 4096, "%s: args->struct_size = %u is not a %s_args (set it to sizeof(%s_args)%s)", fn,
                src->struct_size, fn, fn, note);
    memset(&dst, 0, sizeof(dst));
    memcpy(&dst, src, std::min<size_t>(src->struct_size, sizeof(dst)));
    return 0;
}

struct WsAlloc {
    Engine& E;
    size_t batch;
    template <typename T>
    int operator()(T*& p, size_t per_b) const { return E.ws(&p, per_b * batch); }
};
struct WsShift {
    size_t b0;
    template <typename T>
    int operator()(T*& p, size_t per_b) const {
        p += per_b * b0;
        return 0;
    }
};

GemmParams gemm_base(const bf16* A, int lda, const LinearW& L, int M, int planes);

int launch_pack_weight(const float* src, int N, int K, bf16* hi, bf16* il, int Npad, int Kpad, hipStream_t stream);

struct Scratch {
    std::vector<void*> ptrs;
    ~Scratch() {
        for (void* p : ptrs) (void)hipFree(p);
    }
    template <typename T>
    T* get(size_t count, bool zero = false) {
        void* p = nullptr;
        if (hipMalloc(&p, count * sizeof(T) + 16) != hipSuccess) return nullptr;
        ptrs.push_back(p);
        if (zero) (void)hipMemset(p, 0, count * sizeof(T));
        return (T*)p;
    }
};
struct LinearOperands {
    bf16 *A, *W;
    float* bias;
    int Kp, Np;
};
int stage_linear_operands(Scratch& sc, const char* who, const float* a, const float* w, const float* bias, int M, int N, int K, int planes, hipStream_t s,
                          LinearOperands* out);
int launch_qkv_scatter(const float* qkv, int B, int N, int H, float scale, bf16* q, bf16* k, bf16* v, int64_t qk_plane, hipStream_t s);

}
```

counterfactualworldmodels_amd/csrc/engine.hip:

```cpp
#include <stdarg.h>

#include "engine.h"

using namespace cwm;

static thread_local char g_err[1024] = "";

void cwm_set_error(const char* fmt, ...) {
    va_list ap;
    va_start(ap, fmt);
    vsnprintf(g_err, sizeof(g_err), fmt, ap);
    va_end(ap);
}

extern "C" const char* cwm_last_error(void) { return g_err; }

#include <mutex>
#include <set>
int cwm_set_max_lds(const void* kernel, int bytes) {
    static std::mutex mu;
    static std::set<std::pair<int, const void*>> done;
    int dev = 0;
    CWM_HIP_CHECK(hipGetDevice(&dev));
    std::lock_guard<std::mutex> lock(mu);
    if (done.count({dev, kernel})) return 0;
    CWM_HIP_CHECK(hipFuncSetAttribute(kernel, hipFuncAttributeMaxDynamicSharedMemorySize, bytes));
    done.insert({dev, kernel});
    return 0;
}
static thread_local int g_pretend_device = -1;
void cwm_set_pretend_device(int d) { g_pretend_device = d; }
int cwm_require_device(int handle_device, const char* what) {
    int cur = -1;
    CWM_HIP_CHECK(hipGetDevice(&cur));
    if (g_pretend_device >= 0) cur = g_pretend_device;
    CWM_REQUIRE(cur == handle_device, "%s: the handle was created on HIP device %d but the calling thread's current device is %d (hipSetDevice(%d) first)", what,
                handle_device, cur, handle_device);
    return 0;
}
extern "C" const char* cwm_version(void) { return "cwm_hip 0.10.4 gfx950"; }
#ifndef CWM_SRC_HASH
#define CWM_SRC_HASH "unknown"
#endif
extern "C" const char* cwm_source_hash(void) { return CWM_SRC_HASH; }
#ifndef CWM_HIPCC_VERSION
#define CWM_HIPCC_VERSION "unknown"
#endif
extern "C" const char* cwm_compiler_version(void) { return CWM_HIPCC_VERSION; }

namespace cwm {

const Tuning& default_tuning() {
    static const Tuning t;
    return t;
}
Tuning& thread_tuning() {
    static thread_local Tuning t;
    return t;
}
namespace {
struct TuningField { const char* name; int Tuning::*member; };
}
static const TuningField* tuning_field(const char* key) {
    typedef TuningField Field;
    static const Field fields[] = {{"gemm_tile", &Tuning::gemm_tile}, {"gemm_debug", &Tuning::gemm_debug}, {"gemm_staged", &Tuning::gemm_staged},
                                   {"gemm_direct", &Tuning::gemm_direct}, {"attn_kernel", &Tuning::attn_kernel}, {"attn_remap", &Tuning::attn_remap},
                                   {"attn_tail", &Tuning::attn_tail}, {"attn_ksplit", &Tuning::attn_ksplit}, {"prune_last_block", &Tuning::prune_last_block}, {"index_fused", &Tuning::index_fused},
                                   {"min_lane_rows", &Tuning::min_lane_rows}, {"conj_ctx_stream", &Tuning::conj_ctx_stream}, {"conj_attn", &Tuning::conj_attn}};
    for (const Field& f : fields)
        if (!strcmp(key, f.name)) return &f;
    return nullptr;
}
int tuning_set(Tuning& t, const char* key, int value) {
    const TuningField* f = tuning_field(key);
    if (!f) return -1;
    t.*(f->member) = value;
    return 0;
}
int tuning_set_production(Tuning& t, const char* key, int value) {
    if (!strcmp(key, "gemm_debug") && (value & (1 | 2 | 8))) return -2;
    return tuning_set(t, key, value);
}
int tuning_get(const Tuning& t, const char* key, int* value) {
    const TuningField* f = tuning_field(key);
    if (!f) return -1;
    *value = t.*(f->member);
    return 0;
}

__global__ void pack_weight_kernel(const float* src, int N, int K, bf16* hi, bf16* il, int Npad, int Kpad) {
    const int64_t i = (int64_t)blockIdx.x * blockDim.x + threadIdx.x;
    if (i >= (int64_t)Npad * Kpad) return;
    const int n = (int)(i / Kpad), k = (int)(i - (int64_t)n * Kpad);
    float v = (n < N && k < K) ? src[(size_t)n * K + k] : 0.f;
    if (hi) store_operand<1>(hi, n, Kpad, k, v);
    if (il) store_operand<2>(il, n, Kpad, k, v);
}

int launch_pack_weight(const float* src, int N, int K, bf16* hi, bf16* il, int Npad, int Kpad, hipStream_t stream) {
    const int64_t total = (int64_t)Npad * Kpad;
    hipLaunchKernelGGL(pack_weight_kernel, dim3((unsigned)((total + 255) / 256)), dim3(256), 0, stream, src, N, K, hi, il, Npad, Kpad);
    CWM_HIP_CHECK(hipGetLastError());
    return 0;
}

Engine::~Engine() {
    (void)hipDeviceSynchronize();
    for (void* p : allocs) (void)hipFree(p);
    for (void* p : ws_allocs) (void)hipFree(p);
    for (auto& kv : splitk_ws) {
        (void)hipFree(kv.second.slabs);
        (void)hipFree(kv.second.counts);
    }
    for (auto& t : timers)
        for (auto& e : t.pool) {
            (void)hipEventDestroy(e.a);
            (void)hipEventDestroy(e.b);
        }
}

int Engine::alloc(void** p, size_t bytes, bool zero, bool workspace) {
    CWM_HIP_CHECK(hipMalloc(p, bytes ? bytes : 16));
    (workspace ? ws_allocs : allocs).push_back(*p);
    if (workspace) ws_bytes += bytes;
    if (zero) CWM_HIP_CHECK(hipMemset(*p, 0, bytes ? bytes : 16));
    return 0;
}

int Engine::free_workspace() {
    CWM_HIP_CHECK(hipDeviceSynchronize());
    for (void* p : ws_allocs) (void)hipFree(p);
    ws_allocs.clear();
    ws_bytes = 0;
    return 0;
}

int Engine::make_linear(LinearW& L, int N, int K, bool bias) {
    L.N = N;
    L.K = K;
    L.Npad = round_up(N, 256);
    L.Kpad = round_up(K, 64);
    L.plane = (int64_t)L.Npad * L.Kpad;
    void* p;
    if (int rc = alloc(&p, (size_t)L.plane * sizeof(bf16), true, false)) return rc;
    L.w = (bf16*)p;
    if (int rc = alloc(&p, (size_t)2 * L.plane * sizeof(bf16), true, false)) return rc;
    L.w_il = (bf16*)p;
    if (bias) {
        if (int rc = alloc(&p, (size_t)L.Npad * sizeof(float), true, false)) return rc;
        L.bias = (float*)p;
    }
    return 0;
}

int Engine::make_vec(float** v, int n) {
    void* p;
    if (int rc = alloc(&p, (size_t)n * sizeof(float), true, false)) return rc;
    *v = (float*)p;
    return 0;
}

void Engine::add_matrix_slot(const std::string& key, LinearW* L, std::vector<int64_t> shape) {
    Slot s;
    s.kind = SLOT_MATRIX;
    s.shape = shape;
    s.lin = L;
    s.numel = (int64_t)L->N * L->K;
    slots[key] = s;
}

void Engine::add_vec_slot(const std::string& key, float* dst, std::vector<int64_t> shape, int repeat) {
    Slot s;
    s.kind = SLOT_VECTOR;
    s.shape = shape;
    s.dst = dst;
    s.repeat = repeat;
    s.numel = 1;
    for (auto d : shape) s.numel *= d;
    slots[key] = s;
}

void Engine::add_ignored_slot(const std::string& key, std::vector<int64_t> shape) {
    Slot s;
    s.kind = SLOT_IGNORED;
    s.shape = shape;
    s.numel = 1;
    for (auto d : shape) s.numel *= d;
    slots[key] = s;
}

int Engine::make_block(BlockW& b, const std::string& pre, int D, int hidden) {
    int rc;
    if ((rc = make_vec(&b.ln1_g, D)) || (rc = make_vec(&b.ln1_b, D)) || (rc = make_vec(&b.ln2_g, D)) || (rc = make_vec(&b.ln2_b, D)))
        return rc;
    if ((rc = make_linear(b.qkv, 3 * D, D, true)) || (rc = make_linear(b.proj, D, D, true)) || (rc = make_linear(b.fc1, hidden, D, true)) ||
        (rc = make_linear(b.fc2, D, hidden, true)))
        return rc;
    add_vec_slot(pre + "norm1.weight", b.ln1_g, {D});
    add_vec_slot(pre + "norm1.bias", b.ln1_b, {D});
    add_vec_slot(pre + "norm2.weight", b.ln2_g, {D});
    add_vec_slot(pre + "norm2.bias", b.ln2_b, {D});
    add_vec_slot(pre + "attn.q_bias", b.qkv.bias, {D});
    add_vec_slot(pre + "attn.v_bias", b.qkv.bias + 2 * D, {D});
    add_matrix_slot(pre + "attn.qkv.weight", &b.qkv, {3 * D, D});
    add_matrix_slot(pre + "attn.proj.weight", &b.proj, {D, D});
    add_vec_slot(pre + "attn.proj.bias", b.proj.bias, {D});
    add_matrix_slot(pre + "mlp.fc1.weight", &b.fc1, {hidden, D});
    add_vec_slot(pre + "mlp.fc1.bias", b.fc1.bias, {hidden});
    add_matrix_slot(pre + "mlp.fc2.weight", &b.fc2, {D, hidden});
    add_vec_slot(pre + "mlp.fc2.bias", b.fc2.bias, {D});
    return 0;
}

int Engine::make_sinusoid(float** dst, int n_pos, int d, int extra_rows) {
    std::vector<float> tab((size_t)(n_pos + extra_rows) * d, 0.f);
    for (int pos = 0; pos < n_pos; ++pos)
        for (int j = 0; j < d; ++j) {
            const double ang = (double)pos / pow(10000.0, 2.0 * (double)(j / 2) / (double)d);
            tab[(size_t)pos * d + j] = (float)((j & 1) ? cos(ang) : sin(ang));
        }
// ... 58 lines not shown
}

int Engine::load_weight(const char* key, const float* data, int on_device, const int64_t* shape, int ndim) {
    CWM_REQUIRE(key && data && shape, "load_weight: null argument");
    if (int rc = cwm_require_device(device, "load_weight")) return rc;
    auto it = slots.find(key);
    CWM_REQUIRE(it != slots.end(), "unexpected key in state_dict: %s", key);
    Slot& s = it->second;
    bool same = (int)s.shape.size() == ndim;
    for (int i = 0; same && i < ndim; ++i) same = s.shape[i] == shape[i];
    CWM_REQUIRE(same, "size mismatch for %s", key);
    if (s.kind == SLOT_IGNORED) {
        s.loaded = true;
        return CWM_OK;
    }
    if (s.kind == SLOT_VECTOR) {
        for (int r = 0; r < s.repeat; ++r)
            CWM_HIP_CHECK(hipMemcpy(s.dst + (size_t)r * s.numel, data, (size_t)s.numel * sizeof(float),
                                    on_device ? hipMemcpyDeviceToDevice : hipMemcpyHostToDevice));
    } else {
        LinearW& L = *s.lin;
        const float* src = data;
        float* tmp = nullptr;
        if (!on_device) {
            CWM_HIP_CHECK(hipMalloc((void**)&tmp, (size_t)s.numel * sizeof(float)));
            hipError_t e = hipMemcpy(tmp, data, (size_t)s.numel * sizeof(float), hipMemcpyHostToDevice);
            if (e != hipSuccess) {
                (void)hipFree(tmp);
                cwm_set_error("hipMemcpy failed: %s", hipGetErrorString(e));
                return CWM_ERR_HIP;
            }
            src = tmp;
        }
        const int64_t total = (int64_t)L.Npad * L.Kpad;
        hipLaunchKernelGGL(pack_weight_kernel, dim3((unsigned)((total + 255) / 256)), dim3(256), 0, 0, src, L.N, L.K, L.w, L.w_il, L.Npad,
                           L.Kpad);
        hipError_t e = hipDeviceSynchronize();
        if (tmp) (void)hipFree(tmp);
        if (e != hipSuccess) {
            cwm_set_error("pack_weight failed: %s", hipGetErrorString(e));
            return CWM_ERR_HIP;
        }
    }
    s.loaded = true;
    ++loads;
    return CWM_OK;
}

int Engine::missing_weights(char* buf, int buflen) {
    int missing = 0;
    if (buf && buflen > 0) buf[0] = 0;
    for (auto& kv : slots)
        if (!kv.second.loaded && !kv.second.optional) {
            if (!missing && buf && buflen > 0) snprintf(buf, buflen, "%s", kv.first.c_str());
            ++missing;
        }
    return missing;
}

int Engine::require_weights(const char* fn) {
    char miss[256];
    const int nmiss = missing_weights(miss, sizeof(miss));
    CWM_REQUIRE(nmiss == 0, "%s: %d state-dict tensors not loaded (first: %s)", fn, nmiss, miss);
    return 0;
}

int Engine::set_option(const char* fn, const char* key, int value) {
    const int rc = tuning_set_production(tune, key, value);
    CWM_REQUIRE(rc != -2, "%s: gemm_debug bits 1, 2 and 8 are timing-only ablations (wrong outputs): development library only (cwm_debug_set)", fn);
    CWM_REQUIRE(rc == 0, "%s: unknown option %s", fn, key);
    return 0;
}

Lanes::~Lanes() {
    for (auto s : streams)
        if (s) (void)hipStreamDestroy(s);
    if (ev_fork) (void)hipEventDestroy(ev_fork);
    for (auto e : ev_join)
        if (e) (void)hipEventDestroy(e);
}

int Lanes::fork(hipStream_t caller, int n_lanes) {
    CWM_REQUIRE(n_lanes >= 1 && n_lanes <= kMax, "Lanes::fork: %d lanes", n_lanes);
    if (n_lanes >= 2) {
        if (!ev_fork) CWM_HIP_CHECK(hipEventCreateWithFlags(&ev_fork, hipEventDisableTiming));
        CWM_HIP_CHECK(hipEventRecord(ev_fork, caller));
        for (int l = 1; l < n_lanes; ++l) {
            if (!streams[l - 1]) {
                CWM_HIP_CHECK(hipStreamCreateWithFlags(&streams[l - 1], hipStreamNonBlocking));
                CWM_HIP_CHECK(hipEventCreateWithFlags(&ev_join[l - 1], hipEventDisableTiming));
            }
            CWM_HIP_CHECK(hipStreamWaitEvent(streams[l - 1], ev_fork, 0));
        }
    }
    forked = n_lanes;
    return 0;
}

int Lanes::join(hipStream_t caller) {
    const int n = forked;
    forked = 1;
    for (int l = 1; l < n; ++l) {
        CWM_HIP_CHECK(hipEventRecord(ev_join[l - 1], streams[l - 1]));
        CWM_HIP_CHECK(hipStreamWaitEvent(caller, ev_join[l - 1], 0));
    }
    return 0;
}

int Engine::timer_begin(int kclass, double flops, hipStream_t s, EventPair** out) {
    KernelTimer& t = timers[kclass];
    *out = nullptr;
    if (!t.enabled) return 0;
    if (t.used == t.pool.size()) {
        EventPair e;
        CWM_HIP_CHECK(hipEventCreate(&e.a));
        CWM_HIP_CHECK(hipEventCreate(&e.b));
        t.pool.push_back(e);
    }
    EventPair& e = t.pool[t.used++];
    e.flops = flops;
    e.sub = 0;
    CWM_HIP_CHECK(hipEventRecord(e.a, s));
    *out = &e;
    return 0;
}

int Engine::timer_end(EventPair* e, hipStream_t s) {
    if (e) CWM_HIP_CHECK(hipEventRecord(e->b, s));
    return 0;
}

int Engine::attach_splitk_workspace(GemmParams& p, hipStream_t s) {
    auto it = splitk_ws.find(s);
    if (it == splitk_ws.end()) {
        if (splitk_ws.size() >= kMaxSplitKStreams) {
            auto victim = splitk_ws.begin();
            for (auto w = splitk_ws.begin(); w != splitk_ws.end(); ++w)
                if (w->second.last_use < victim->second.last_use) victim = w;
            const SplitKWs old = victim->second;
            splitk_ws.erase(victim);
            (void)hipFree(old.slabs);
            (void)hipFree(old.counts);
        }
        SplitKWs w = {nullptr, nullptr, 0};
        if (int rc = splitk_workspace_alloc(&w.slabs, &w.counts, s)) return rc;
        it = splitk_ws.emplace(s, w).first;
    }
    it->second.last_use = ++splitk_clock;
    p.sk2_slabs = it->second.slabs;
    p.sk2_count = it->second.counts;
    return 0;
}

int Engine::run_gemm(const GemmParams& p_in, int planes, hipStream_t s) {
    GemmParams p = p_in;
    p.overlapped = overlapped;
    p.tune = &tune;
    GemmPlan plan;
    if (int rc = gemm_plan(p, planes, 0, gemm_cu_count(), &plan)) return rc;
    if (plan.splits_k())
        if (int rc = attach_splitk_workspace(p, s)) return rc;
    for (int i = 0; i < plan.nparts; ++i) {
        const GemmPlan::Part& part = plan.part[i];
        EventPair* e;
        if (int rc = timer_begin(CWM_KCLASS_GEMM, 2.0 * part.M * (double)p.N * p.K, s, &e)) return rc;
        if (e) e->sub = part.kernel == GEMM_KERNEL_8PHASE ? CWM_KCLASS_GEMM_WIDE : CWM_KCLASS_GEMM_NARROW;
        if (int rc = launch_gemm_part(p, planes, plan, i, s)) return rc;
        if (int rc = timer_end(e, s)) return rc;
    }
    return 0;
}

int Engine::run_attention(const AttnParams& p_in, int planes, hipStream_t s) {
    AttnParams p = p_in;
    p.tune = &tune;
    EventPair* e;
    const double fl = 4.0 * (double)p.n_tok * p.n_tok * 64.0 * p.heads * p.batch;
    if (int rc = timer_begin(CWM_KCLASS_ATTENTION, fl, s, &e)) return rc;
    if (int rc = launch_attention(p, planes, s)) return rc;
    return timer_end(e, s);
}

int Engine::run_layernorm(const LayerNormParams& p, int planes, hipStream_t s) {
    if (tune.gemm_debug & 8) return 0;
    return timed(CWM_KCLASS_LAYERNORM, (double)p.rows * p.D * (4.0 + 2.0 * planes), s, [&] { return launch_layernorm(p, planes, s); });
}

int Engine::run_patch_gather(const PatchGatherParams& p, int planes, hipStream_t s) {
    return timed(CWM_KCLASS_PATCH_GATHER, (double)p.B * p.n_rows * p.C * p.P * p.P * (4.0 + 2.0 * planes), s, [&] { return launch_patch_gather(p, planes, s); });
}

int Engine::run_index_gather(const PatchGatherParams& p, const uint8_t* mask, int n_vis, int* perm, int* rank, int* err_rows, int planes, hipStream_t s,
                             int n_vis_min, int* counts) {
    const int L = p.perm_stride ? p.perm_stride : p.Nt;
    return timed(CWM_KCLASS_PATCH_GATHER, (double)p.B * p.n_rows * p.C * p.P * p.P * (4.0 + 2.0 * planes) + (double)p.B * L * (1.0 + 4.0 + (rank ? 4.0 : 0.0)), s,
                 [&] { return launch_index_gather(p, mask, n_vis, perm, rank, err_rows, planes, s, n_vis_min, counts); });
}

int Engine::run_fill_mask_tokens(float* x_full, const float* mask_token, const float* pos, const int* perm, int B, int Nt, int n_vis, int D,
                                 hipStream_t s) {
    return timed(CWM_KCLASS_FILL_MASK, (double)B * (Nt - n_vis) * D * 4.0, s,
                 [&] { return launch_fill_mask_tokens(x_full, mask_token, pos, perm, B, Nt, n_vis, D, s); });
}

int Engine::run_unembed(const UnembedParams& p, hipStream_t s) {
    return timed(CWM_KCLASS_UNEMBED, (double)p.B * p.T * p.C * p.H * p.W * 8.0, s, [&] { return launch_unembed(p, s); });
}

int Engine::timing_enable(int kclass, int enable) {
    CWM_REQUIRE(kclass >= 0 && kclass < CWM_KCLASS_COUNT, "timing_enable: bad kernel class");
    KernelTimer& t = timers[kclass];
    t.enabled = enable != 0;
    while (enable && t.pool.size() < 512) {
        EventPair e;
        CWM_HIP_CHECK(hipEventCreate(&e.a));
        CWM_HIP_CHECK(hipEventCreate(&e.b));
        e.flops = 0;
        e.sub = 0;
        t.pool.push_back(e);
    }
    return CWM_OK;
}

int Engine::timing_collect(int kclass, cwm_kernel_stats* out) {
    CWM_REQUIRE(out && kclass >= 0 && kclass < CWM_KCLASS_COUNT, "timing_collect: bad argument");
    KernelTimer& t = timers[kclass];
    for (size_t i = 0; i < t.used; ++i) {
        CWM_HIP_CHECK(hipEventSynchronize(t.pool[i].b));
        float ms = 0.f;
        CWM_HIP_CHECK(hipEventElapsedTime(&ms, t.pool[i].a, t.pool[i].b));
        t.acc.launches += 1;
        t.acc.total_ms += ms;
        t.acc.total_flops += t.pool[i].flops;
        if (t.pool[i].sub > 0 && t.pool[i].sub < CWM_KCLASS_COUNT) {
            cwm_kernel_stats& sa = timers[t.pool[i].sub].acc;
            sa.launches += 1;
            sa.total_ms += ms;
            sa.total_flops += t.pool[i].flops;
        }
    }
    t.used = 0;
    *out = t.acc;
    t.acc = {0, 0.0, 0.0};
    return CWM_OK;
}

GemmParams gemm_base(const bf16* A, int lda, const LinearW& L, int M, int planes) {
    GemmParams p;
    memset(&p, 0, sizeof(p));
    p.A = A;
    p.lda = lda;
    p.W = planes == 2 ? L.w_il : L.w;
    p.M = M;
    p.N = L.N;
    p.K = L.Kpad;
    p.bias = L.bias;
    return p;
}

int Engine::layernorm_to(const float* x, int rows, int D, const float* g, const float* b, bf16* out, int planes, hipStream_t s) {
    LayerNormParams ln;
    memset(&ln, 0, sizeof(ln));
    ln.x = x; ln.ldx = D; ln.gamma = g; ln.beta = b; ln.eps = ln_eps; ln.D = D; ln.rows = rows;
    ln.out = out; ln.out_plane = (int64_t)rows * D; ln.ldo = D;
    return run_layernorm(ln, planes, s);
}

int Engine::linear_f32(const bf16* A, int rows, int K, const LinearW& L, float* C, const float* resid, int planes, hipStream_t s) {
    GemmParams g = gemm_base(A, K, L, rows, planes);
    g.epi = EPI_F32; g.C = C; g.ldc = L.N; g.resid = resid; g.ldr = L.N;
    return run_gemm(g, planes, s);
}

int Engine::linear_operand(const bf16* A, int rows, int K, const LinearW& L, bf16* out, int planes, hipStream_t s) {
    GemmParams g = gemm_base(A, K, L, rows, planes);
    g.epi = EPI_BF16; g.out_hi = out; g.out_plane = (int64_t)rows * L.N; g.ldo = L.N;
    return run_gemm(g, planes, s);
}

int Engine::linear_gelu(const bf16* A, int rows, int K, const LinearW& L, bf16* out, int planes, hipStream_t s) {
    GemmParams g = gemm_base(A, K, L, rows, planes);
    g.epi = EPI_BF16_GELU; g.out_hi = out; g.out_plane = (int64_t)rows * L.N; g.ldo = L.N;
    return run_gemm(g, planes, s);
}

namespace {
struct KeptRows {
    bool part;
    int n_out, first;
    KeptRows(int n_tok, int n_keep) : part(n_keep > 0 && n_keep < n_tok), n_out(part ? n_keep : n_tok), first(n_tok - n_out) {}
};
}

static int residual_gemm(Engine& E, const bf16* A, int K, const LinearW& L, float* x, int B, int n_tok, const KeptRows& kr, int planes, hipStream_t s) {
    GemmParams r = gemm_base(A, K, L, B * kr.n_out, planes);
    r.epi = EPI_F32; r.C = x; r.ldc = L.N; r.resid = x; r.ldr = L.N;
    if (kr.part) { r.rows_in = kr.n_out; r.rows_out = n_tok; r.out_row_offset = kr.first; }
    return E.run_gemm(r, planes, s);
}

int Engine::run_mlp(const float* ln_g, const float* ln_b, const LinearW& fc1, const LinearW& fc2, float* x, int B, int n_tok, int D, int planes,
                    StreamBuffers& sb, hipStream_t s, int n_keep) {
    const KeptRows kr(n_tok, n_keep);
    const int Mo = B * kr.n_out;
    int rc;
    LayerNormParams ln;
    memset(&ln, 0, sizeof(ln));
    ln.x = x; ln.ldx = D; ln.gamma = ln_g; ln.beta = ln_b; ln.eps = ln_eps; ln.D = D; ln.rows = Mo;
    ln.out = sb.hbuf; ln.out_plane = (int64_t)Mo * D; ln.ldo = D;
    if (kr.part) { ln.rows_out_per_b = kr.n_out; ln.rows_in_per_b = n_tok; ln.in_offset = kr.first; }
    if ((rc = run_layernorm(ln, planes, s))) return rc;
    if ((rc = linear_gelu(sb.hbuf, Mo, D, fc1, sb.gbuf, planes, s))) return rc;
    return residual_gemm(*this, sb.gbuf, fc1.N, fc2, x, B, n_tok, kr, planes, s);
}

int Engine::run_block(const BlockW& w, float* x, int B, int n_tok, int D, int H, int planes, StreamBuffers& sb, hipStream_t s, int n_keep, const int* key_len) {
    const int M = B * n_tok;
    const int64_t hplane = (int64_t)M * D;
    const KeptRows kr(n_tok, n_keep);
    int rc;
    if ((rc = layernorm_to(x, M, D, w.ln1_g, w.ln1_b, sb.hbuf, planes, s))) return rc;

    GemmParams g = gemm_base(sb.hbuf, D, w.qkv, M, planes);
    g.epi = EPI_QKV;
    g.rows_in = n_tok; g.rows_out = n_tok; g.map_stride = n_tok;
    g.q_out = sb.qbuf; g.k_out = sb.kbuf; g.v_out = sb.vbuf;
    g.qk_plane = hplane;
    g.qkv_dim = D; g.heads = H; g.head_dim = D / H; g.n_tok = n_tok;
    g.q_scale = 1.0f / sqrtf((float)(D / H));
    if ((rc = run_gemm(g, planes, s))) return rc;

    AttnParams a;
    memset(&a, 0, sizeof(a));
    a.q = sb.qbuf; a.k = sb.kbuf; a.v = sb.vbuf; a.qk_plane = hplane;
    a.o = sb.hbuf; a.o_plane = (int64_t)B * kr.n_out * D; a.ldo = D; a.n_tok = n_tok; a.heads = H; a.batch = B;
    if (kr.part) { a.q_off = kr.first; a.n_q = kr.n_out; }
    a.key_len = key_len;
    if ((rc = run_attention(a, planes, s))) return rc;

    if ((rc = residual_gemm(*this, sb.hbuf, D, w.proj, x, B, n_tok, kr, planes, s))) return rc;
    return run_mlp(w.ln2_g, w.ln2_b, w.fc1, w.fc2, x, B, n_tok, D, planes, sb, s, n_keep);
}

int Engine::run_block_small(const BlockW& w, float* x, int B, int n_tok, int D, int H, int planes, StreamBuffers& sb, hipStream_t s) {
    const int M = B * n_tok;
    int rc;
    if ((rc = layernorm_to(x, M, D, w.ln1_g, w.ln1_b, sb.hbuf, planes, s))) return rc;
    GemmParams g = gemm_base(sb.hbuf, D, w.qkv, M, planes);
    g.epi = EPI_F32; g.C = sb.qkv_f32; g.ldc = 3 * D;
    if ((rc = run_gemm(g, planes, s))) return rc;

    SmallAttnParams a;
    memset(&a, 0, sizeof(a));
    a.qkv = sb.qkv_f32; a.B = B; a.n_tok = n_tok; a.heads = H; a.head_dim = D / H;
    a.o = sb.hbuf; a.o_plane = (int64_t)M * D; a.ldo = D;
    if ((rc = timed(CWM_KCLASS_SMALL_ATTN, 4.0 * (double)B * H * n_tok * n_tok * (D / H), s, [&] {
             return (tune.conj_attn && small_attention_mfma_ok(n_tok, D / H) && D % 32 == 0) ? launch_small_attention_mfma(a, planes, s) : launch_small_attention(a, planes, s);
         })))
        return rc;

    if ((rc = linear_f32(sb.hbuf, M, D, w.proj, x, x, planes, s))) return rc;
    return run_mlp(w.ln2_g, w.ln2_b, w.fc1, w.fc2, x, B, n_tok, D, planes, sb, s);
}

int Engine::embed_stream(const StreamW& S, const StreamWs& w, int B, int n_vis, int planes, hipStream_t s) {
    const int next = S.n_slots();
    GemmParams g = gemm_base(w.tokens_in, S.embed_kpad, S.embed, B * n_vis, planes);
    g.epi = EPI_F32; g.C = w.x_enc; g.ldc = S.enc_dim;
    g.resid = S.pos_enc_ext; g.ldr = S.enc_dim; g.resid_rowmap = w.perm; g.rows_in = n_vis; g.rows_out = n_vis; g.map_stride = next;
    if (int rc = run_gemm(g, planes, s)) return rc;
    if (S.max_pad == 0) return 0;
    return launch_fix_pad_rows(w.x_enc, w.perm, B, next, n_vis, S.n_tok, S.enc_dim, S.null_enc, s);
}

int Engine::to_decoder(const StreamW& S, const StreamWs& w, int B, int n_vis, int planes, hipStream_t s, const int* counts, int n_vis_min) {
    const int next = S.n_slots();
    int rc;
    if ((rc = layernorm_to(w.x_enc, B * n_vis, S.enc_dim, S.enc_norm_g, S.enc_norm_b, w.sb.hbuf, planes, s))) return rc;
    GemmParams g = gemm_base(w.sb.hbuf, S.enc_dim, S.e2d, B * n_vis, planes);
    g.epi = EPI_F32; g.C = w.x_dec; g.ldc = S.dec_dim;
    g.resid = S.pos_dec_ext; g.ldr = S.dec_dim; g.resid_rowmap = w.perm; g.rows_in = n_vis; g.rows_out = next; g.map_stride = next;
    if ((rc = run_gemm(g, planes, s))) return rc;
    if (counts)
        return timed(CWM_KCLASS_FILL_MASK, (double)B * (next - n_vis_min) * S.dec_dim * 4.0, s,
                     [&] { return launch_fill_mask_tokens_ragged(w.x_dec, S.mask_token, S.pos_dec_ext, w.perm, counts, B, next, n_vis_min, S.dec_dim, s); });
    return run_fill_mask_tokens(w.x_dec, S.mask_token, S.pos_dec_ext, w.perm, B, next, n_vis, S.dec_dim, s);
}

int Engine::head_rows(const StreamW& S, const StreamWs& w, int B, int n_out, float* out, int planes, hipStream_t s) {
    const int next = S.n_slots();
    LayerNormParams ln;
    memset(&ln, 0, sizeof(ln));
    ln.x = w.x_dec; ln.ldx = S.dec_dim; ln.gamma = S.dec_norm_g; ln.beta = S.dec_norm_b; ln.eps = ln_eps; ln.D = S.dec_dim;
    ln.rows = B * n_out; ln.rows_out_per_b = n_out; ln.rows_in_per_b = next; ln.in_offset = next - n_out;
    ln.out = w.sb.hbuf; ln.out_plane = (int64_t)B * n_out * S.dec_dim; ln.ldo = S.dec_dim;
    if (int rc = run_layernorm(ln, planes, s)) return rc;
    GemmParams g = gemm_base(w.sb.hbuf, S.dec_dim, S.head, B * n_out, planes);
    g.epi = EPI_F32; g.C = out; g.ldc = S.out_dim;
    return run_gemm(g, planes, s);
}

}
```

counterfactualworldmodels_amd/csrc/gemm.hip:

```cpp
#include <atomic>
#include <map>
#include <mutex>
#include <tuple>
#include <utility>

#include "gemm_device.h"
#include <cstdio>
#include <algorithm>

namespace cwm {

#ifdef CWM_GEMM_PROF
__device__ unsigned long long g_gemm_blocks[8192 * 4];
int gemm_prof_dump() {
    static unsigned long long h[8192 * 4];
    if (hipMemcpyFromSymbol(h, HIP_SYMBOL(g_gemm_blocks), sizeof(h)) != hipSuccess) return -1;
    FILE* f = fopen("/tmp/gemm_blocks.bin", "wb");
    if (!f) return -1;
    fwrite(h, 1, sizeof(h), f);
    fclose(f);
    return 0;
}
#define GEMM_PROF_BEGIN() const unsigned long long prof_t0 = __builtin_amdgcn_s_memtime(), prof_r0 = __builtin_amdgcn_s_memrealtime(); unsigned long long prof_main = 0
#define GEMM_PROF_MAIN() prof_main = __builtin_amdgcn_s_memtime() - prof_t0
// ... 65 lines not shown
        w_src[jj] = (unsigned)(n0 + (wperm ? w_row_perm(row) : row)) * (unsigned)(p.K * PLANES) + logical * 8;
    }
    auto issue_tile = [&](int stage, int k0) {
        char* sb = smem + stage * STAGE_BYTES;
        const bf16* ab = p.A + k0;
        const bf16* wb = p.W + k0;
#pragma unroll
        for (int jj = 0; jj < NIA; ++jj)
            __builtin_amdgcn_global_load_lds((gbl_void*)(ab + a_src[jj]), (lds_void*)(sb + (wave * NIA + jj) * 1024), 16, 0, 0);
#pragma unroll
        for (int jj = 0; jj < NIB; ++jj)
            __builtin_amdgcn_global_load_lds((gbl_void*)(wb + w_src[jj]), (lds_void*)(sb + A_BYTES + (wave * NIB + jj) * 1024), 16, 0, 0);
    };
    f32x4 acc[FM][FN];
#pragma unroll
    for (int i = 0; i < FM; ++i)
#pragma unroll
        for (int j = 0; j < FN; ++j) acc[i][j] = f32x4{0.f, 0.f, 0.f, 0.f};

    const int frow = lane & 15, fq = lane >> 4;
    int a_base[2], b_base[2];
#pragma unroll
    for (int half = 0; half < 2; ++half) {
        a_base[half] = lds_off<64>(wr * (16 * FM) + frow, half * 4 + fq);
        b_base[half] = A_BYTES + lds_off<64>(wc * (16 * FN) + frow, half * 4 + fq);
    }

    const int nk_all = p.K / BK;
    const int kt0 = (STAGES > 2) ? (int)((int64_t)nk_all * part / nsplit) : 0;
    const int nk = (STAGES > 2) ? (int)((int64_t)nk_all * (part + 1) / nsplit) - kt0 : nk_all;
#pragma unroll
    for (int st = 0; st < STAGES - 1; ++st)
        if (st < nk) issue_tile(st, (kt0 + st) * 64);
    for (int t = 0; t < nk; ++t) {
        const int cur = STAGES == 2 ? (t & 1) : t % STAGES;
        if constexpr (STAGES == 2) {
            __syncthreads();
            if (t + 1 < nk) issue_tile(cur ^ 1, (t + 1) * 64);
        } else {
            constexpr int PER = NIA + NIB;
            const int younger = min(nk - 1 - t, STAGES - 2);
            if (younger >= 2) asm volatile("s_waitcnt vmcnt(%0)" ::"n"(2 * PER) : "memory");
            else if (younger == 1) asm volatile("s_waitcnt vmcnt(%0)" ::"n"(PER) : "memory");
            else asm volatile("s_waitcnt vmcnt(0)" ::: "memory");
            __builtin_amdgcn_sched_barrier(0);
            __builtin_amdgcn_s_barrier();
            __builtin_amdgcn_sched_barrier(0);
            if (t + STAGES - 1 < nk) issue_tile((t + STAGES - 1) % STAGES, (kt0 + t + STAGES - 1) * 64);
        }
        const char* base = smem + cur * STAGE_BYTES;
        constexpr int KSTEPS = BK / 32, UNITS = KSTEPS * FM, DIST = (PLANES == 1) ? 3 : 2;
        bf16x8 bfr[KSTEPS][PLANES][FN];
        bf16x8 afu[UNITS][PLANES];
#pragma unroll
        for (int pl = 0; pl < PLANES; ++pl)
#pragma unroll
            for (int j = 0; j < FN; ++j) bfr[0][pl][j] = *reinterpret_cast<const bf16x8*>(base + b_base[pl] + j * 2048);
#pragma unroll
        for (int u = 0; u < DIST && u < UNITS; ++u)
#pragma unroll
            for (int pl = 0; pl < PLANES; ++pl)
                afu[u][pl] = *reinterpret_cast<const bf16x8*>(base + a_base[PLANES == 1 ? u / FM : pl] + (u % FM) * 2048);
#pragma unroll
        for (int u = 0; u < UNITS; ++u) {
            const int kk = u / FM, i = u % FM;
            if (u + DIST < UNITS) {
#pragma unroll
                for (int pl = 0; pl < PLANES; ++pl)
                    afu[u + DIST][pl] =
                        *reinterpret_cast<const bf16x8*>(base + a_base[PLANES == 1 ? (u + DIST) / FM : pl] + ((u + DIST) % FM) * 2048);
            }
            if (PLANES == 1 && KSTEPS == 2 && u == FM - DIST) {
#pragma unroll
                for (int j = 0; j < FN; ++j) bfr[KSTEPS - 1][0][j] = *reinterpret_cast<const bf16x8*>(base + b_base[1] + j * 2048);
            }
#pragma unroll
            for (int j = 0; j < FN; ++j) {
                if constexpr (PLANES == 2) {
                    acc[i][j] = __builtin_amdgcn_mfma_f32_16x16x32_bf16(bfr[kk][0][j], afu[u][1], acc[i][j], 0, 0, 0);
                    acc[i][j] = __builtin_amdgcn_mfma_f32_16x16x32_bf16(bfr[kk][1][j], afu[u][0], acc[i][j], 0, 0, 0);
                }
                acc[i][j] = __builtin_amdgcn_mfma_f32_16x16x32_bf16(bfr[kk][0][j], afu[u][0], acc[i][j], 0, 0, 0);
            }
            __builtin_amdgcn_sched_barrier(0);
        }
    }
    if (p.debug & 2) {
#pragma unroll
        for (int i = 0; i < FM; ++i)
#pragma unroll
            for (int j = 0; j < FN; ++j) asm volatile("" ::"v"(acc[i][j]));
        return;
    }
    GEMM_PROF_MAIN();
    static_assert(STAGES <= 4, "the counted waits above cover at most 3 tiles in flight");
    if constexpr (STAGES > 2) {
        if (nsplit > 1) {
            const int tile_id = (int)blockIdx.x / nsplit;
            float* slab = sk_slabs + ((size_t)tile_id * nsplit + part) * (BM * BN) + (size_t)wave * (FM * FN * 256) + lane * 4;
#pragma unroll
            for (int i = 0; i < FM; ++i)
#pragma unroll
                for (int j = 0; j < FN; ++j) *reinterpret_cast<f32x4*>(slab + (i * FN + j) * 256) = acc[i][j];
            asm volatile("s_waitcnt vmcnt(0)" ::: "memory");
            __syncthreads();
            int* flag = reinterpret_cast<int*>(smem);
            if (tid == 0) {
                __builtin_amdgcn_fence(__ATOMIC_RELEASE, "agent");
                asm volatile("s_waitcnt vmcnt(0)" ::: "memory");
                const unsigned prev = __hip_atomic_fetch_add(sk_count + tile_id, 1u, __ATOMIC_RELAXED, __HIP_MEMORY_SCOPE_AGENT);
                const bool last = prev == (unsigned)(nsplit - 1);
                if (last) {
                    __builtin_amdgcn_fence(__ATOMIC_ACQUIRE, "agent");
                    asm volatile("s_waitcnt vmcnt(0)" ::: "memory");
                    __hip_atomic_store(sk_count + tile_id, 0u, __ATOMIC_RELAXED, __HIP_MEMORY_SCOPE_AGENT);
                }
                *flag = last ? 1 : 0;
            }
            __syncthreads();
            if (*flag == 0) return;
            const float* base_slab = sk_slabs + (size_t)tile_id * nsplit * (BM * BN) + (size_t)wave * (FM * FN * 256) + lane * 4;
#pragma unroll
            for (int i = 0; i < FM; ++i)
#pragma unroll
                for (int j = 0; j < FN; ++j) acc[i][j] = *reinterpret_cast<const f32x4*>(base_slab + (i * FN + j) * 256);
            for (int q = 1; q < nsplit; ++q) {
                const float* sl = base_slab + (size_t)q * (BM * BN);
#pragma unroll
                for (int i = 0; i < FM; ++i)
#pragma unroll
                    for (int j = 0; j < FN; ++j) acc[i][j] += *reinterpret_cast<const f32x4*>(sl + (i * FN + j) * 256);
            }
        }
    }
    if (p.direct) {
        __syncthreads();
        int4* tab = reinterpret_cast<int4*>(smem);
        epilogue_row_table(p, tab, m0, BM, tid);
        __syncthreads();
        epilogue_direct_tile<PLANES, FM, FN>(p, acc, tab, wr * (16 * FM), n0 + wc * (16 * FN), lane);
    } else if (p.staged) {
        __syncthreads();
        int4* tab = reinterpret_cast<int4*>(smem + NWAVES * 8192);
        epilogue_row_table(p, tab, m0, BM, tid);
        __syncthreads();
        epilogue_staged<PLANES, FM, FN>(p, acc, smem + wave * 8192, tab, wr * (16 * FM), n0 + wc * (16 * FN), lane);
    } else {
        epilogue_rows<PLANES, FM, FN>(p, acc, m0, n0, wr, wc, lane);
    }
    GEMM_PROF_END();
}


template <int PLANES, bool HALF>
__device__ __forceinline__ void gemm8p_tile(const GemmParams& p, char* smem, int m0, int n0) {
    GEMM_PROF_BEGIN();
    constexpr int HALF_BYTES = 128 * 128;
    constexpr int BUF_BYTES = 4 * HALF_BYTES;
    const int tid = threadIdx.x;
    const int lane = tid & 63;
    const int wave = __builtin_amdgcn_readfirstlane(tid >> 6);
    const int wr = wave >> 2, wc = wave & 3;

    const bool wperm = p.direct && p.epi != EPI_F32;
    unsigned src[4][2];
#pragma unroll
    for (int h = 0; h < 2; ++h)
#pragma unroll
        for (int jj = 0; jj < 2; ++jj) {
            const int row = wave * 16 + jj * 8 + lane / 8;
            const int logical = (lane % 8) ^ lds_swizzle<64>(row);
            src[h][jj] = (unsigned)(p.m_offset + min(m0 + h * 128 + row, p.M - 1)) * (unsigned)(p.lda * PLANES) + logical * 8;
            src[2 + h][jj] = (unsigned)(n0 + h * 128 + (wperm ? w_row_perm(row) : row)) * (unsigned)(p.K * PLANES) + logical * 8;
        }
    auto stage = [&](auto half_c, int buf, int kt) {
        constexpr int half = decltype(half_c)::value;
        const bf16* gb = (half < 2 ? p.A : p.W) + (size_t)kt * 64;
        char* sb = smem + buf * BUF_BYTES + half * HALF_BYTES + wave * 2048;
#pragma unroll
        for (int jj = 0; jj < 2; ++jj)
            __builtin_amdgcn_global_load_lds((gbl_void*)(gb + src[half][jj]), (lds_void*)(sb + jj * 1024), 16, 0, 0);
    };
    using H_A0 = std::integral_constant<int, 0>;
    using H_A1 = std::integral_constant<int, 1>;
    using H_W0 = std::integral_constant<int, 2>;
    using H_W1 = std::integral_constant<int, 3>;

    const int frow = lane & 15, fq = lane >> 4;
    int a_base[2], b_base[2];
#pragma unroll
    for (int h = 0; h < 2; ++h) {
        a_base[h] = lds_off<64>(wr * 64 + frow, h * 4 + fq);
        b_base[h] = 2 * HALF_BYTES + lds_off<64>(wc * 32 + frow, h * 4 + fq);
    }
    bf16x8 af[2][4], bw0[2][2], bw1[2][2];
    auto read_a = [&](const char* base, int qm) {
#pragma unroll
        for (int h = 0; h < 2; ++h)
#pragma unroll
            for (int i = 0; i < 4; ++i) af[h][i] = *reinterpret_cast<const bf16x8*>(base + qm * HALF_BYTES + a_base[h] + i * 2048);
    };
    auto read_w = [&](const char* base, int qn, bf16x8 (&bw)[2][2]) {
#pragma unroll
        for (int h = 0; h < 2; ++h)
#pragma unroll
            for (int j = 0; j < 2; ++j) bw[h][j] = *reinterpret_cast<const bf16x8*>(base + qn * HALF_BYTES + b_base[h] + j * 2048);
    };

    f32x4 acc[2][2][4][2];
#pragma unroll
    for (int a = 0; a < 2; ++a)
#pragma unroll
        for (int b = 0; b < 2; ++b)
#pragma unroll
            for (int i = 0; i < 4; ++i)
#pragma unroll
                for (int j = 0; j < 2; ++j) acc[a][b][i][j] = f32x4{0.f, 0.f, 0.f, 0.f};

    auto mfma_quadrant = [&](f32x4 (&c)[4][2], const bf16x8 (&bw)[2][2]) {
        __builtin_amdgcn_s_setprio(1);
        if constexpr (PLANES == 1) {
#pragma unroll
            for (int h = 0; h < 2; ++h)
#pragma unroll
                for (int i = 0; i < 4; ++i)
#pragma unroll
                    for (int j = 0; j < 2; ++j) c[i][j] = __builtin_amdgcn_mfma_f32_16x16x32_bf16(bw[h][j], af[h][i], c[i][j], 0, 0, 0);
        } else {
#pragma unroll
            for (int i = 0; i < 4; ++i)
#pragma unroll
                for (int j = 0; j < 2; ++j) {
                    c[i][j] = __builtin_amdgcn_mfma_f32_16x16x32_bf16(bw[0][j], af[1][i], c[i][j], 0, 0, 0);
                    c[i][j] = __builtin_amdgcn_mfma_f32_16x16x32_bf16(bw[1][j], af[0][i], c[i][j], 0, 0, 0);
                    c[i][j] = __builtin_amdgcn_mfma_f32_16x16x32_bf16(bw[0][j], af[0][i], c[i][j], 0, 0, 0);
                }
        }
        __builtin_amdgcn_s_setprio(0);
    };
#define CWM_PHASE_BARRIER()                   \
    do {                                      \
        __builtin_amdgcn_sched_barrier(0);    \
        __builtin_amdgcn_s_barrier();         \
        __builtin_amdgcn_sched_barrier(0);    \
    } while (0)

    const int nk = p.K / (64 / PLANES);
    if constexpr (!HALF) {
        stage(H_A0{}, 0, 0);
        stage(H_W0{}, 0, 0);
        stage(H_W1{}, 0, 0);
        stage(H_A1{}, 0, 0);
        if (nk > 1) {
            stage(H_A0{}, 1, 1);
            stage(H_W0{}, 1, 1);
            stage(H_W1{}, 1, 1);
            asm volatile("s_waitcnt vmcnt(6)" ::: "memory");
        } else {
            asm volatile("s_waitcnt vmcnt(0)" ::: "memory");
        }
    } else {
        stage(H_A0{}, 0, 0);
        stage(H_W0{}, 0, 0);
        stage(H_A1{}, 0, 0);
        if (nk > 1) {
            stage(H_A0{}, 1, 1);
            stage(H_W0{}, 1, 1);
            asm volatile("s_waitcnt vmcnt(4)" ::: "memory");
        } else {
            asm volatile("s_waitcnt vmcnt(0)" ::: "memory");
        }
    }
    CWM_PHASE_BARRIER();
    if (wr == 1) CWM_PHASE_BARRIER();

    for (int t = 0; t < nk; ++t) {
        const int buf = t & 1;
        const char* base = smem + buf * BUF_BYTES;
        read_w(base, 0, bw0);
        read_a(base, 0);
        if (t + 1 < nk) stage(H_A1{}, buf ^ 1, t + 1);
        CWM_PHASE_BARRIER();
        mfma_quadrant(acc[0][0], bw0);
        CWM_PHASE_BARRIER();
        if constexpr (!HALF) read_w(base, 1, bw1);
        if (t + 2 < nk) stage(H_A0{}, buf, t + 2);
        CWM_PHASE_BARRIER();
        if constexpr (!HALF) mfma_quadrant(acc[0][1], bw1);
        CWM_PHASE_BARRIER();
        read_a(base, 1);
        if (t + 2 < nk) stage(H_W0{}, buf, t + 2);
        CWM_PHASE_BARRIER();
        if constexpr (!HALF) mfma_quadrant(acc[1][1], bw1);
        CWM_PHASE_BARRIER();
        if (t + 2 >= nk) {
            asm volatile("s_waitcnt vmcnt(0)" ::: "memory");
        } else if constexpr (HALF) {
            asm volatile("s_waitcnt vmcnt(4)" ::: "memory");
        } else {
            stage(H_W1{}, buf, t + 2);
            asm volatile("s_waitcnt vmcnt(6)" ::: "memory");
        }
        CWM_PHASE_BARRIER();
        mfma_quadrant(acc[1][0], bw0);
        CWM_PHASE_BARRIER();
    }
    if (wr == 0) CWM_PHASE_BARRIER();
#undef CWM_PHASE_BARRIER

    if (p.debug & 2) {
#pragma unroll
        for (int qm = 0; qm < 2; ++qm)
#pragma unroll
            for (int qn = 0; qn < 2; ++qn)
#pragma unroll
                for (int i = 0; i < 4; ++i)
#pragma unroll
                    for (int j = 0; j < 2; ++j) asm volatile("" ::"v"(acc[qm][qn][i][j]));
        return;
    }
    GEMM_PROF_MAIN();
    if (p.direct) {
        int4* tab = reinterpret_cast<int4*>(smem);
        epilogue_row_table(p, tab, m0, 256, tid);
        __syncthreads();
        if constexpr (HALF)
            epilogue_direct<PLANES, 2>(
                p, [&](int pi, int i, int j) { return acc[pi][0][i][j]; }, [&](int pi) { return pi * 128 + wr * 64; }, [&](int) { return n0 + wc * 32; }, tab, lane);
        else
            epilogue_direct<PLANES, 4>(
                p, [&](int pi, int i, int j) { return acc[pi >> 1][pi & 1][i][j]; }, [&](int pi) { return (pi >> 1) * 128 + wr * 64; },
                [&](int pi) { return n0 + (pi & 1) * 128 + wc * 32; }, tab, lane);
        GEMM_PROF_END();
        return;
    }
    if (p.staged) {
        int4* tab = reinterpret_cast<int4*>(smem + 8 * 8192);
        epilogue_row_table(p, tab, m0, 256, tid);
        __syncthreads();
        if constexpr (HALF)
            epilogue_piece_seq<PLANES, 2>(
                p, [&](int pi, int i, int j) { return acc[pi][0][i][j]; }, [&](int pi) { return pi * 128 + wr * 64; }, [&](int) { return n0 + wc * 32; },
                smem + wave * 8192, tab, lane);
        else
            epilogue_piece_seq<PLANES, 4>(
                p, [&](int pi, int i, int j) { return acc[pi >> 1][pi & 1][i][j]; }, [&](int pi) { return (pi >> 1) * 128 + wr * 64; },
                [&](int pi) { return n0 + (pi & 1) * 128 + wc * 32; }, smem + wave * 8192, tab, lane);
        GEMM_PROF_END();
        return;
    }
    const int ncol = (lane >> 4) * 4;
#pragma unroll
    for (int qm = 0; qm < 2; ++qm)
#pragma unroll
        for (int i = 0; i < 4; ++i) {
            const int m = m0 + qm * 128 + wr * 64 + i * 16 + (lane & 15);
            if (m >= p.M) continue;
            const RowMap rm = map_row(p, m + p.m_offset);
#pragma unroll
            for (int qn = 0; qn < 2; ++qn)
#pragma unroll
                for (int j = 0; j < 2; ++j) {
                    const int nb = n0 + qn * 128 + wc * 32 + j * 16;
                    if (nb >= p.N) continue;
                    epilogue_frag<PLANES>(p, rm, nb, ncol, acc[qm][qn][i][j]);
                }
        }
}

template <int PLANES>
__global__ __launch_bounds__(512, 2) void gemm8p_kernel(const GemmParams p) {
    extern __shared__ __attribute__((aligned(16))) char smem[];
    const int tiles_m = (p.M + 255) / 256;
    const int tiles_n = (p.N + 255) / 256;
    const int id = xcd_remap(blockIdx.x, tiles_m * tiles_n);
    constexpr int GROUP_M = 4;
    const int group_sz = GROUP_M * tiles_n;
    const int g = id / group_sz;
    const int first_m = g * GROUP_M;
    const int gm = min(tiles_m - first_m, GROUP_M);
    const int in_g = id - g * group_sz;
    const int m0 = (first_m + (in_g % gm)) * 256, n0 = (in_g / gm) * 256;
    if (n0 + 128 >= p.N && !(p.debug & 1024)) gemm8p_tile<PLANES, true>(p, smem, m0, n0);
    else gemm8p_tile<PLANES, false>(p, smem, m0, n0);
}

int splitk_workspace_alloc(float** slabs, unsigned** counts, hipStream_t stream) {
    CWM_HIP_CHECK(hipMalloc((void**)slabs, (size_t)kSplitKSlots * 128 * 128 * sizeof(float)));
    CWM_HIP_CHECK(hipMalloc((void**)counts, kSplitKSlots * sizeof(unsigned)));
    CWM_HIP_CHECK(hipMemsetAsync(*counts, 0, kSplitKSlots * sizeof(unsigned), stream));
    return 0;
}

static inline const Tuning& tn(const GemmParams& p) { return p.tune ? *p.tune : default_tuning(); }

int gemm_cu_count() {
    static int cus = 0;
    if (cus == 0) {
        int dev = 0;
        hipDeviceProp_t prop;
        if (hipGetDevice(&dev) != hipSuccess || hipGetDeviceProperties(&prop, dev) != hipSuccess) return 256;
        cus = prop.multiProcessorCount & ~7;
        if (cus < 8) cus = 256;
    }
    return cus;
}

int gemm_plan(const GemmParams& p, int planes, int forced_cfg, int cus, GemmPlan* plan) {
    const Tuning& t = tn(p);
    CWM_REQUIRE(planes == 1 || planes == 2, "gemm: planes must be 1 or 2");
    CWM_REQUIRE(p.K % 64 == 0, "gemm: K=%d must be a multiple of 64", p.K);
    CWM_REQUIRE(p.lda % 8 == 0, "gemm: lda=%d must be a multiple of 8", p.lda);
    CWM_REQUIRE(p.M > 0 && p.N > 0, "gemm: empty problem M=%d N=%d", p.M, p.N);
    CWM_REQUIRE(p.N % 16 == 0, "gemm: N=%d must be a multiple of 16", p.N);
    if (p.epi == EPI_F32) {
        CWM_REQUIRE(p.ldc % 4 == 0 && (!p.resid || p.ldr % 4 == 0), "gemm: ldc/ldr must be multiples of 4");
    } else if (p.epi == EPI_QKV) {
        CWM_REQUIRE(p.rows_in == p.n_tok && p.N == 3 * p.qkv_dim && p.head_dim % 4 == 0, "gemm: bad QKV epilogue setup");
        CWM_REQUIRE(p.qkv_dim % 16 == 0, "gemm: QKV epilogue needs the model width (%d) to be a multiple of 16", p.qkv_dim);
    } else {
        CWM_REQUIRE(p.ldo % 4 == 0, "gemm: ldo must be a multiple of 4");
        CWM_REQUIRE(planes == 1 || p.ldo % 32 == 0, "gemm: split-bf16 output rows are whole [32 hi | 32 lo] blocks: ldo=%d must be a multiple of 32", p.ldo);
    }
    plan->staged = 0;
    if (t.gemm_staged) {
        if (p.epi == EPI_F32) plan->staged = 1;
        else if (p.epi == EPI_QKV) plan->staged = (p.qkv_dim % 32 == 0 && p.head_dim % 32 == 0);
        else plan->staged = (p.ldo % 8 == 0);
    }
    CWM_REQUIRE((int64_t)(p.m_offset + p.M) * p.lda * planes < (1ll << 32) && (int64_t)(((p.N + 255) / 256) * 256) * p.K * planes < (1ll << 32),
                "gemm: operand too large for 32-bit element offsets (M=%d lda=%d N=%d K=%d planes=%d): split the batch", p.m_offset + p.M, p.lda,
                p.N, p.K, planes);
    plan->direct = (t.gemm_direct && plan->staged && (p.epi != EPI_F32 || t.gemm_direct >= 2)) ? 1 : 0;

    int cfg = forced_cfg > 0 ? forced_cfg : t.gemm_tile;
    if (cfg == 0 && t.tile_hook) cfg = t.tile_hook(p.M, p.N, p.K, p.epi, p.overlapped ? 1 : 0);
    if (cfg == 0) {
        cfg = 1;
        const bool bf16_out = p.epi != EPI_F32;
        const bool half_ok = !(t.gemm_debug & 1024) && p.N >= 384 && p.N % 256 == 128;
        if (p.K >= ((bf16_out && !(t.gemm_debug & 512)) ? 256 : 512) && p.M >= 512 && (p.N >= 1024 || (p.N >= 512 && p.N % 256 == 0) || half_ok)) {
            const int64_t tiles_m = (p.M + 255) / 256, tiles_n = (p.N + 255) / 256;
            const int64_t tiles = (half_ok && p.N % 256 == 128) ? tiles_m * (tiles_n - 1) + (tiles_m * 3 + 4) / 5 : tiles_m * tiles_n;
            if (tiles < cus) {
                const bool long_or_direct = bf16_out || p.K >= 1024;
                cfg = (tiles * 2 >= cus || (p.overlapped && long_or_direct && tiles * 5 >= cus * 2)) ? 4 : 1;
            } else if (p.overlapped && !(t.gemm_debug & 128)) {
                cfg = 4;
            } else {
                const int last = (int)(tiles % cus);
                const bool full_enough = (bf16_out || p.K >= 1024) ? last * 2 >= cus : last * 5 >= cus * 4;
                if (last == 0 || full_enough) cfg = 4;
                else if (half_ok && p.N < 512) cfg = tiles < 2 * cus ? 1 : 4;
                else if (p.K >= 1024 || p.N >= 1024) cfg = 6;
            }
        }
    }
    plan->nparts = 1;
    plan->part[0].m_offset = p.m_offset;
    plan->part[0].M = p.M;
    if (cfg == 6) {
        const int tiles_n = (p.N + 255) / 256, tiles_m = (p.M + 255) / 256;
        const int rounds = (tiles_m * tiles_n) / cus;
        const int big_rows = std::min(tiles_m - 1, rounds * cus / tiles_n);
        if (rounds >= 1 && big_rows >= 1) {
            plan->nparts = 2;
            plan->part[0].M = big_rows * 256;
            plan->part[1].m_offset = p.m_offset + big_rows * 256;
            plan->part[1].M = p.M - big_rows * 256;
        } else {
            cfg = 1;
        }
    }
    CWM_REQUIRE(cfg == 1 || cfg == 4 || cfg == 6, "gemm: unknown tile configuration %d (1: 128x128, 4: 256x256 8-phase, 6: mixed)", cfg);
    plan->cfg = cfg;
    for (int i = 0; i < plan->nparts; ++i) {
        GemmPlan::Part& part = plan->part[i];
        part.splitk = 1;
        if (cfg == 4 || (cfg == 6 && i == 0)) {
            part.kernel = GEMM_KERNEL_8PHASE;
            continue;
        }
        part.kernel = GEMM_KERNEL_128;
        const int tiles128 = ((part.M + 127) / 128) * ((p.N + 127) / 128);
        if ((t.gemm_debug & 4) || tiles128 > cus) continue;
        const int bm = (tiles128 * 2 <= cus && part.M > 64 && !(t.gemm_debug & 256)) ? 64 : 128;
        part.kernel = bm == 64 ? GEMM_KERNEL_DEEP64 : GEMM_KERNEL_DEEP128;
        if (t.gemm_debug & 32) continue;
        const int tiles = ((part.M + bm - 1) / bm) * ((p.N + 127) / 128);
        const int nk_all = p.K / (64 / planes);
        const int sk = std::min(std::min(cus / tiles, nk_all / 12), 8);
        if (sk >= 3) part.splitk = sk;
    }
    return 0;
}

int launch_gemm_part(const GemmParams& p_in, int planes, const GemmPlan& plan, int i, hipStream_t stream) {
    typedef void (*kern_t)(const GemmParams);
    struct Shape {
        kern_t kernel[2];
        int bm, bn, threads;
        size_t smem;
    };
    static const Shape shapes[4] = {
        {{gemm_bf16_kernel<1, 128, 128, 2, 4>, gemm_bf16_kernel<2, 128, 128, 2, 4>}, 128, 128, 512, (size_t)2 * (128 + 128) * 128 + 4096},
        {{gemm_bf16_kernel<1, 128, 128, 2, 4, 4>, gemm_bf16_kernel<2, 128, 128, 2, 4, 4>}, 128, 128, 512, (size_t)4 * (128 + 128) * 128},
        {{gemm_bf16_kernel<1, 64, 128, 1, 4, 4>, gemm_bf16_kernel<2, 64, 128, 1, 4, 4>}, 64, 128, 256, (size_t)4 * (64 + 128) * 128},
        {{gemm8p_kernel<1>, gemm8p_kernel<2>}, 256, 256, 512, (size_t)2 * 4 * 128 * 128},
    };
    static_assert((size_t)2 * (128 + 128) * 128 + 4096 >= (size_t)8 * 8192 + (size_t)128 * 16 + (size_t)128 * 8,
                  "gemm: dynamic LDS too small for the staged epilogue (wave buffers + row table)");
    const GemmPlan::Part& part = plan.part[i];
    const Shape& k = shapes[part.kernel];
    GemmParams p = p_in;
    p.m_offset = part.m_offset;
    p.M = part.M;
    p.splitk = part.splitk;
    p.staged = plan.staged;
    p.direct = plan.direct;
    p.debug = tn(p).gemm_debug;
    CWM_REQUIRE(part.splitk == 1 || (p.sk2_slabs && p.sk2_count), "gemm: a launch that splits K needs the caller's split-K workspace");
    if (int rc = cwm_set_max_lds((const void*)k.kernel[planes - 1], (int)k.smem)) return rc;
    const int tiles = ((p.M + k.bm - 1) / k.bm) * ((p.N + k.bn - 1) / k.bn);
    hipLaunchKernelGGL(k.kernel[planes - 1], dim3(tiles * part.splitk), dim3(k.threads), k.smem, stream, p);
    CWM_HIP_CHECK(hipGetLastError());
    return 0;
}

int launch_gemm(const GemmParams& p_in, int planes, hipStream_t stream) {
    GemmPlan plan;
    if (int rc = gemm_plan(p_in, planes, 0, gemm_cu_count(), &plan)) return rc;
    GemmParams p = p_in;
    if (plan.splits_k() && !p.sk2_slabs) {
        struct Ws { float* slabs; unsigned* counts; };
        static std::mutex mu;
        static std::map<std::pair<int, hipStream_t>, Ws> table;
        int dev = 0;
        CWM_HIP_CHECK(hipGetDevice(&dev));
        std::lock_guard<std::mutex> lock(mu);
        auto it = table.find(std::make_pair(dev, stream));
        if (it == table.end()) {
            Ws w = {nullptr, nullptr};
            if (int rc = splitk_workspace_alloc(&w.slabs, &w.counts, stream)) return rc;
            it = table.emplace(std::make_pair(dev, stream), w).first;
        }
        p.sk2_slabs = it->second.slabs;
        p.sk2_count = it->second.counts;
    }
    for (int i = 0; i < plan.nparts; ++i)
        if (int rc = launch_gemm_part(p, planes, plan, i, stream)) return rc;
    return 0;
}

}
```

counterfactualworldmodels_amd/csrc/kernels.h:

```cpp
#pragma once
#include "common.h"

namespace cwm {

struct Tuning {
    int gemm_tile = 0;
    int gemm_debug = 0;
    int gemm_staged = 1;
    int gemm_direct = 1;
    int attn_kernel = 0;
    int attn_remap = 1;
    int attn_tail = 1;
    int attn_ksplit = 1;
    int index_fused = 1;
    int prune_last_block = 1;
    int min_lane_rows = 0;
    int conj_ctx_stream = 1;
    int conj_attn = 1;
    int (*tile_hook)(int M, int N, int K, int epi, int overlapped) = nullptr;
};
const Tuning& default_tuning();
Tuning& thread_tuning();
int tuning_set(Tuning& t, const char* key, int value);
int tuning_set_production(Tuning& t, const char* key, int value);
int tuning_get(const Tuning& t, const char* key, int* value);

enum GemmEpilogue : int {
    EPI_F32 = 0,
    EPI_BF16_GELU = 1,
    EPI_BF16 = 2,
    EPI_QKV = 3,
};

struct GemmParams {
    const bf16* A;
    const bf16* W;
    int lda;
    int M, N, K;
    int m_offset;
    const float* bias;
    int epi;
    int rows_in, rows_out, map_stride;
    int out_row_offset;
    const int* resid_rowmap;
    float* C;
    int ldc;
    const float* resid;
    int ldr;
    bf16* out_hi;
    int64_t out_plane;
    int ldo;
    bf16* q_out;
    bf16* k_out;
    bf16* v_out;
    int64_t qk_plane;
    int qkv_dim, heads, head_dim, n_tok;
    float q_scale;
    int splitk;
    float* sk2_slabs;
    unsigned* sk2_count;
    int staged;
    int direct;
    int overlapped;
    int debug;
    const Tuning* tune;
};

constexpr int kSplitKSlots = 512;
int splitk_workspace_alloc(float** slabs, unsigned** counts, hipStream_t stream);
enum GemmKernel : int {
    GEMM_KERNEL_128 = 0,
    GEMM_KERNEL_DEEP128 = 1,
    GEMM_KERNEL_DEEP64 = 2,
    GEMM_KERNEL_8PHASE = 3,
};
struct GemmPlan {
    int cfg;
    int nparts;
    struct Part {
        int m_offset, M;
        int kernel;
        int splitk;
    } part[2];
    int staged, direct;
    bool splits_k() const { return part[0].splitk > 1 || (nparts == 2 && part[1].splitk > 1); }
};
int gemm_plan(const GemmParams& p, int planes, int forced_cfg, int cus, GemmPlan* plan);
int launch_gemm_part(const GemmParams& p, int planes, const GemmPlan& plan, int i, hipStream_t stream);
int launch_gemm(const GemmParams& p, int planes, hipStream_t stream);
int gemm_cu_count();
int gemm_prof_dump();

struct AttnParams {
    const bf16* q;
    const bf16* k;
    const bf16* v;
    int64_t qk_plane;
    bf16* o;
    int64_t o_plane;
    int ldo;
    int n_tok, heads, batch;
    int remap;
    int q_off, n_q;
    int ks_main, ks_parts, ks_nqb;
    float* ks_scratch;
    int tail_split;
    const Tuning* tune;
    const int* key_len;
};

int launch_attention(const AttnParams& p, int planes, hipStream_t stream);
int attention_pipe_prof(int i);
int launch_attention_pipe(const AttnParams& p, int planes, hipStream_t stream);

struct LayerNormParams {
    const float* x;
    int ldx;
    const float* gamma;
    const float* beta;
    float eps;
    int D;
    int rows;
    int rows_out_per_b, rows_in_per_b, in_offset;
    bf16* out;
    int64_t out_plane;
    int ldo;
    float* out_f32;
};

int launch_layernorm(const LayerNormParams& p, int planes, hipStream_t stream);

int launch_mask_to_perm(const uint8_t* mask, int B, int Nt, int n_vis, int* perm, int* err, hipStream_t stream);
int launch_mask_row_counts(const uint8_t* mask, int B, int Nt, int* counts, hipStream_t stream);
int launch_mask_flip_picks(uint8_t* mask, int B, int Nt, const int* table, int n_rows, hipStream_t stream);

struct PatchGatherParams {
    const float* x;
    int64_t sb, sc, st;
    int normalize;
    int C, H, W, P;
    const int* perm;
    int Nt, n_rows;
    int perm_stride;
    int B;
    bf16* out;
    int64_t out_plane;
    int ld;
};

int launch_patch_gather(const PatchGatherParams& p, int planes, hipStream_t stream);

struct FlowRgbGatherParams {
    const float* fwd;
    const float* bwd;
    int64_t f_sb, f_sc, b_sb, b_sc;
    const float* x;
    int64_t sb, sc;
    int normalize;
    int H, W, P;
    const int* perm;
    int Nt, n_rows, perm_stride, B;
    bf16* out;
    int64_t out_plane;
    int ld;
};
int launch_flow_rgb_gather(const FlowRgbGatherParams& p, int planes, hipStream_t stream);
int launch_index_gather(const PatchGatherParams& p, const uint8_t* mask, int n_vis, int* perm, int* rank, int* err_rows, int planes, hipStream_t stream,
                        int n_vis_min = 0, int* counts = nullptr);
int launch_mask_to_perm_ragged(const uint8_t* mask, int B, int Nt, int n_vis_min, int n_vis, int* perm, int* err, int* counts, hipStream_t stream);

int launch_fill_mask_tokens(float* x_full, const float* mask_token, const float* pos, const int* perm, int B, int Nt, int n_vis, int D, hipStream_t stream);
int launch_fill_mask_tokens_ragged(float* x_full, const float* mask_token, const float* pos, const int* perm, const int* counts, int B, int Nt, int n_vis_min,
                                   int D, hipStream_t stream);

struct UnembedParams {
    const float* y;
    const float* x;
    int64_t sb, sc, st;
    const uint8_t* mask;
    const int* rank;
    int B, T, C, H, W, P, n_vis, Nm;
    float* out;
};

int launch_unembed(const UnembedParams& p, hipStream_t stream);

struct ShiftPromptParams {
    const float* x;
    int B, S, T, C, H, W, P, frame, fix_passive;
    const uint8_t* active;
    const uint8_t* masks;
    const int* shifts;
    float* x_out;
    uint8_t* mask_out;
};

int launch_shift_prompts(const ShiftPromptParams& p, hipStream_t stream);
int launch_prompt_table_expand(const int* table, int S, int gh, int gw, int T, int frame, uint8_t* active, uint8_t* passive, int* shifts, hipStream_t stream);

constexpr int kMultiShiftMaxSteps = 8;
struct MultiShiftParams {
    const float* x;
    int B, S, K, T, C, H, W, P, frame, fix_passive, mask_steps;
    const uint8_t* points;
    const uint8_t* masks;
    const int* shifts;
    float* x_out;
    uint8_t* mask_out;
};

int launch_multi_shift_prompts(const MultiShiftParams& p, hipStream_t stream);

struct SmallAttnParams {
    const float* qkv;
    int B, n_tok, heads, head_dim;
    bf16* o;
    int64_t o_plane;
    int ldo;
};
int launch_small_attention(const SmallAttnParams& p, int planes, hipStream_t stream);
int launch_small_attention_mfma(const SmallAttnParams& p, int planes, hipStream_t stream);
bool small_attention_mfma_ok(int n_tok, int head_dim);

int launch_pad_mask(const uint8_t* mask, int B, int N, int P, int vmax, uint8_t* ext_mask, hipStream_t stream);
int launch_fix_pad_rows(float* x, const int* perm, int B, int perm_stride, int n_rows, int n_real, int D, const float* token, hipStream_t stream);
int launch_zero_pad_out_rows(float* y, const int* perm, int B, int perm_stride, int n_vis, int n_out, int n_real, int D, hipStream_t stream);

struct ImuGatherParams {
    const float* imu;
    int B, C, L, tubelet;
    const int* perm;
    int perm_stride, n_rows, n_real;
    bf16* out;
    int64_t out_plane;
    int ld;
};
int launch_imu_gather(const ImuGatherParams& p, int planes, hipStream_t stream);
int launch_imu_append_dummy(const float* imu, const uint8_t* mask, const float* dummy, int B, int C, int L, int T, int n, float* out, uint8_t* mask_out,
                            hipStream_t stream);

struct CrossAttnParams {
    const float* qk;
    const float* v;
    const bf16* qk_op;
    const bf16* v_op;
    const float* qk_src;
    const float* v_src;
    int B, N, M, heads, head_dim;
    float scale;
    bf16* y;
    int64_t y_plane;
    bf16* y_src;
    int64_t y_src_plane;
    float* scores_t;
    float* partial;
};
int launch_cross_attention(const CrossAttnParams& p, int planes, hipStream_t stream);
size_t cross_attention_partial_floats(int B, int heads, int M, int head_dim);
size_t cross_attention_lds_bytes(int M, int head_dim);
bool cross_attention_ok(int M, int head_dim);
int launch_cross_attention_mfma(const CrossAttnParams& p, int planes, hipStream_t stream);
int launch_cross_attention_mfma_roles(const CrossAttnParams& p, int planes, hipStream_t stream_a, hipStream_t stream_b, int roles);
bool cross_attention_mfma_ok(int head_dim, int M);
bool cross_attention_mfma_fits(int B, int N, int heads, int head_dim);
size_t cross_attention_mfma_partial_floats(int B, int heads, int M, int head_dim);

int launch_perm_to_rank(const int* perm, int* rank, int B, int Nt, hipStream_t stream);

int launch_split_bf16(const float* x, int64_t n, bf16* hi, bf16* lo, hipStream_t stream);

struct ConvSrc {
    const float* p;
    int ld, C;
    const float* stats;
    int relu;
    const float* gate;
    int gate_ld;
    const float* coords;
};
struct ImageSrc {
    const float* base[2];
    int64_t sb[2], st[2], sc[2];
    int P, ppg;
    float scale;
};
struct Im2colParams {
    ConvSrc src[2];
    int nsrc;
    ImageSrc image;
    int img0;
    int n_img, H, W, OH, OW, kh, kw, stride, pad_h, pad_w;
    int c_lo, c_hi;
    bf16* A;
    int Kpad;
};
struct CorrLookupParams {
    const float* pyr[4];
    int h[4], w[4], levels;
    const float* coords;
    int64_t M;
    bf16* A;
    int Kpad;
    float* out;
    int out_ld;
};
struct CorrOnTheFlyParams {
    const float* fmap1;
    const float* fmap2[4];
    int h[4], w[4];
    const float* coords;
    int64_t M, hw8;
    bf16* A;
    int Kpad;
    float* out;
    int out_ld;
};
struct ConvexUpParams {
    const float* coords;
    const float* value;
    const float* mask;
    int mask_ld;
    float mask_scale;
    int C, P, ppg, h8, w8;
    float* out;
    int64_t out_sb, out_st, out_sc;
};
// ... 35 lines not shown
```

counterfactualworldmodels_amd/csrc/model.hip:

```cpp
#include <stddef.h>

#include "engine.h"

using namespace cwm;

struct ModelWs {
    StreamWs st;
    int* rank = nullptr;
    int* err = nullptr;
    int* counts = nullptr;
};

struct cwm_model {
    Engine eng;
    cwm_config cfg;
    StreamW st;
    int ws_batch = 0, ws_nvis = 0;
    ModelWs ws;
    int lanes = 2;
    int ragged_min = 0;
    static constexpr int kMaxLanes = Lanes::kMax;
    Lanes lane_set;
};

namespace {

template <typename Visit>
int for_each_buffer(const cwm_model* m, ModelWs& w, int n_vis_cap, Visit&& visit) {
    if (int rc = for_each_stream_buffer(m->st, w.st, n_vis_cap, m->cfg.mlp_ratio, false, visit)) return rc;
    return visit(w.rank, (size_t)m->st.n_tok);
}

int ensure_workspace(cwm_model* m, int B, int n_vis) {
    if (B <= m->ws_batch && n_vis <= m->ws_nvis && m->ws_batch > 0) return 0;
    Engine& E = m->eng;
    const int Bc = std::max(B, m->ws_batch), Nv = std::max(n_vis, m->ws_nvis);
    m->ws_batch = 0;
    int rc;
    if ((rc = E.free_workspace()) || (rc = for_each_buffer(m, m->ws, Nv, WsAlloc{E, (size_t)Bc}))) return rc;
    if ((rc = E.ws(&m->ws.err, (size_t)2 * Bc + 8))) return rc;
    m->ws.counts = m->ws.err + Bc + 4;
    m->ws_batch = Bc;
    m->ws_nvis = Nv;
    CWM_HIP_CHECK(hipDeviceSynchronize());
    return 0;
}

ModelWs lane_ws(const cwm_model* m, int b0) {
    ModelWs w = m->ws;
    (void)for_each_buffer(m, w, m->ws_nvis, WsShift{(size_t)b0});
    w.err += b0;
    w.counts += b0;
    return w;
}

}

extern "C" int cwm_model_create(const cwm_config* cfg, cwm_model** out) {
    CWM_REQUIRE(cfg && out, "cwm_model_create: null argument");
    const cwm_config& c = *cfg;
    CWM_REQUIRE(c.patch > 0 && c.img_h % c.patch == 0 && c.img_w % c.patch == 0, "image size (%d,%d) must be divisible by patch size %d",
                c.img_h, c.img_w, c.patch);
    CWM_REQUIRE(c.patch % 4 == 0 && c.img_w % 4 == 0, "patch size must be a multiple of 4");
    CWM_REQUIRE(c.enc_heads > 0 && c.dec_heads > 0 && c.enc_dim == 64 * c.enc_heads && c.dec_dim == 64 * c.dec_heads,
                "this build supports head_dim 64 only (enc %d/%d, dec %d/%d)", c.enc_dim, c.enc_heads, c.dec_dim, c.dec_heads);
    CWM_REQUIRE(c.enc_dim <= 1024 && c.dec_dim <= 1024 && c.enc_dim % 64 == 0 && c.dec_dim % 64 == 0, "embed dims must be multiples of 64, <= 1024");
    CWM_REQUIRE(c.in_chans == 3 && c.num_frames >= 1 && c.mlp_ratio >= 1 && c.enc_depth >= 1 && c.dec_depth >= 1, "unsupported config");
    cwm_model* m = new cwm_model();
    m->cfg = c;
    Engine& E = m->eng;
    E.ln_eps = c.ln_eps;
    CWM_HIP_CHECK(hipGetDevice(&E.device));
    StreamW& S = m->st;
    S.enc_dim = c.enc_dim; S.dec_dim = c.dec_dim; S.enc_heads = c.enc_heads; S.dec_heads = c.dec_heads;
    S.n_tok = (c.img_h / c.patch) * (c.img_w / c.patch) * c.num_frames; S.out_dim = c.in_chans * c.patch * c.patch;
    const int rc = E.make_stream(S, "", c.in_chans * c.patch * c.patch, {c.enc_dim, c.in_chans, 1, c.patch, c.patch}, c.enc_depth, c.dec_depth, c.mlp_ratio,
                                 true, false);
    if (rc) {
        cwm_model_destroy(m);
        return rc;
    }
    *out = m;
    return CWM_OK;
}

extern "C" void cwm_model_destroy(cwm_model* m) { delete m; }

extern "C" int cwm_model_load_weight(cwm_model* m, const char* key, const float* data, int on_device, const int64_t* shape, int ndim) {
    CWM_REQUIRE(m, "cwm_model_load_weight: null model");
    return m->eng.load_weight(key, data, on_device, shape, ndim);
}

extern "C" int cwm_model_missing_weights(cwm_model* m, char* buf, int buflen) { return m->eng.missing_weights(buf, buflen); }


static int forward_lane(cwm_model* m, const cwm_forward_args* a, int b0, int B, ModelWs lw, hipStream_t s, int stage_lo, int stage_hi) {
    const cwm_config& c = m->cfg;
    const StreamW& S = m->st;
    StreamWs& w = lw.st;
    const int rg_min = m->ragged_min;
    const int* counts = rg_min > 0 ? lw.counts : nullptr;
    const int Nt = S.n_tok, Nv = a->n_vis, Nm = Nt - (rg_min > 0 ? rg_min : Nv);
    const int Nret = Nm > 0 ? Nm : Nt;
    Engine& E = m->eng;
    const int planes = a->mode == CWM_MODE_PARITY ? 2 : 1;
    const float* x_in = a->x_dev + (int64_t)b0 * a->x_stride_b;
    const uint8_t* mask_in = a->mask_dev + (size_t)b0 * Nt;
    float* y_tokens = a->y_tokens_dev + (size_t)b0 * Nret * S.out_dim;
    int rc;
    auto in_range = [&](int st) { return st >= stage_lo && st < stage_hi; };
    const int st_e2d = c.enc_depth + 1, st_head = c.enc_depth + c.dec_depth + 2;

    if (in_range(0)) {
    PatchGatherParams pg;
    memset(&pg, 0, sizeof(pg));
    pg.x = x_in; pg.sb = a->x_stride_b; pg.sc = a->x_stride_c; pg.st = a->x_stride_t; pg.normalize = a->normalize;
    pg.C = c.in_chans; pg.H = c.img_h; pg.W = c.img_w; pg.P = c.patch; pg.perm = w.perm; pg.Nt = Nt; pg.n_rows = Nv; pg.B = B;
    pg.out = w.tokens_in; pg.out_plane = (int64_t)B * Nv * S.embed_kpad; pg.ld = S.embed_kpad;
    if (E.tune.index_fused) {
        if ((rc = E.run_index_gather(pg, mask_in, Nv, w.perm, a->y_video_dev ? lw.rank : nullptr, lw.err, planes, s, rg_min, lw.counts))) return rc;
    } else {
        CWM_HIP_CHECK(hipMemsetAsync(lw.err, 0, (size_t)B * sizeof(int), s));
        if ((rc = rg_min > 0 ? launch_mask_to_perm_ragged(mask_in, B, Nt, rg_min, Nv, w.perm, lw.err, lw.counts, s) : launch_mask_to_perm(mask_in, B, Nt, Nv, w.perm, lw.err, s)))
            return rc;
        if ((rc = E.run_patch_gather(pg, planes, s))) return rc;
        if (a->y_video_dev && (rc = launch_perm_to_rank(w.perm, lw.rank, B, Nt, s))) return rc;
    }
    if ((rc = E.embed_stream(S, w, B, Nv, planes, s))) return rc;
    }

    for (int i = 0; i < c.enc_depth; ++i)
        if (in_range(1 + i) && (rc = E.run_block(S.enc[i], w.x_enc, B, Nv, S.enc_dim, S.enc_heads, planes, w.sb, s, 0, counts))) return rc;

    if (in_range(st_e2d) && (rc = E.to_decoder(S, w, B, Nv, planes, s, counts, rg_min))) return rc;

    const bool pruned = Nm > 0 && E.tune.prune_last_block;
    for (int i = 0; i < c.dec_depth; ++i) {
        const int keep = (i == c.dec_depth - 1 && pruned) ? Nm : 0;
        if (in_range(st_e2d + 1 + i) && (rc = E.run_block(S.dec[i], w.x_dec, B, Nt, S.dec_dim, S.dec_heads, planes, w.sb, s, keep))) return rc;
    }
    if (!in_range(st_head)) return CWM_OK;
    if ((rc = E.head_rows(S, w, B, Nret, y_tokens, planes, s))) return rc;

    if (a->y_video_dev) {
        const float* xr = a->xraw_dev ? a->xraw_dev + (int64_t)b0 * a->x_stride_b : x_in;
        UnembedParams u;
        memset(&u, 0, sizeof(u));
        u.y = y_tokens; u.x = xr; u.sb = a->x_stride_b; u.sc = a->x_stride_c; u.st = a->x_stride_t;
        u.mask = mask_in; u.rank = lw.rank; u.B = B; u.T = c.num_frames; u.C = c.in_chans; u.H = c.img_h; u.W = c.img_w;
        u.P = c.patch; u.n_vis = Nt - Nm; u.Nm = Nm;
        u.out = a->y_video_dev + (size_t)b0 * c.num_frames * c.in_chans * c.img_h * c.img_w;
        if ((rc = E.run_unembed(u, s))) return rc;
    }
    return CWM_OK;
}

extern "C" int cwm_forward(cwm_model* m, const cwm_forward_args* a_in) {
    CWM_REQUIRE(m && a_in, "cwm_forward: null argument");
    cwm_forward_args a_copy;
    if (int rc = copy_args(a_copy, a_in, offsetof(cwm_forward_args, stream) + sizeof(void*), "cwm_forward", "; callers built against the 0.5 header must be rebuilt"))
        return rc;
    const cwm_forward_args* a = &a_copy;
    if (int rc = cwm_require_device(m->eng.device, "cwm_forward")) return rc;
    CWM_REQUIRE(a->x_dev && a->mask_dev && a->y_tokens_dev, "cwm_forward: x_dev, mask_dev and y_tokens_dev are required");
    CWM_REQUIRE(a->mode == CWM_MODE_FAST || a->mode == CWM_MODE_PARITY, "cwm_forward: bad mode %d", a->mode);
    const cwm_config& c = m->cfg;
    const int B = a->batch, Nt = m->st.n_tok, Nv = a->n_vis, Nm = Nt - Nv;
    CWM_REQUIRE(B > 0, "cwm_forward: batch must be positive");
    CWM_REQUIRE(m->ragged_min <= Nv, "cwm_forward: the handle takes rows of at least %d visible tokens (cwm_model_set_ragged), more than the call's cap n_vis = %d",
                m->ragged_min, Nv);
    CWM_REQUIRE(Nv > 0 && Nm >= 0, "cwm_forward: need 0 < n_vis (%d) <= num tokens (%d)", Nv, Nt);
    CWM_REQUIRE(Nm > 0 || !a->y_video_dev, "cwm_forward: no token is masked, there is no predicted patch to un-embed");
    CWM_REQUIRE(!a->y_video_dev || a->xraw_dev || a->normalize, "cwm_forward: y_video_dev needs the raw frames (xraw_dev) when normalize=0");
    if (int rc = m->eng.require_weights("cwm_forward")) return rc;
    if (int rc = ensure_workspace(m, B, Nv)) return rc;
    hipStream_t s = (hipStream_t)a->stream;

    const int min_rows = m->eng.tune.min_lane_rows > 0 ? m->eng.tune.min_lane_rows : kMinLaneRows;
    int n_lanes = 1;
    while (n_lanes < m->lanes && n_lanes < B && (int64_t)(B / (n_lanes + 1)) * Nv >= min_rows) ++n_lanes;
    int first[cwm_model::kMaxLanes + 1];
    for (int l = 0; l <= n_lanes; ++l) first[l] = (int)(((int64_t)B * l + n_lanes - 1) / n_lanes);
    if (int rc = m->lane_set.fork(s, n_lanes)) return rc;
    m->eng.overlapped = n_lanes >= 2;
    int rc = 0;
    const int n_stages = c.enc_depth + c.dec_depth + 3;
    for (int st = 0; st < n_stages && !rc; ++st)
        for (int l = 0; l < n_lanes && !rc; ++l)
            rc = forward_lane(m, a, first[l], first[l + 1] - first[l], lane_ws(m, first[l]), m->lane_set.stream(l, s), st, st + 1);
    m->eng.overlapped = 0;
    if (int jrc = m->lane_set.join(s)) return jrc;
    if (rc) return rc;

    if (a->check) {
        std::vector<int> herr((size_t)B, 0);
        CWM_HIP_CHECK(hipMemcpyAsync(herr.data(), m->ws.err, (size_t)B * sizeof(int), hipMemcpyDeviceToHost, s));
        CWM_HIP_CHECK(hipStreamSynchronize(s));
        if (m->ragged_min > 0 && std::any_of(herr.begin(), herr.end(), [](int e) { return e != 0; })) {
            cwm_set_error("mask rows do not all have between %d (cwm_model_set_ragged) and n_vis=%d visible tokens", m->ragged_min, Nv);
            return CWM_ERR_MASK;
        }
        if (std::any_of(herr.begin(), herr.end(), [](int e) { return e != 0; })) {
            cwm_set_error("mask rows do not all have n_vis=%d visible tokens (shape '[%d, -1, %d]' is invalid for the gathered input)", Nv, B,
                          c.enc_dim);
            return CWM_ERR_MASK;
        }
    }
    return CWM_OK;
}

extern "C" int cwm_model_set_lanes(cwm_model* m, int lanes) {
    CWM_REQUIRE(m && lanes >= 1 && lanes <= cwm_model::kMaxLanes, "cwm_model_set_lanes: lanes must be 1 .. %d", cwm_model::kMaxLanes);
    m->lanes = lanes;
    return CWM_OK;
}

extern "C" int cwm_model_set_ragged(cwm_model* m, int n_vis_min) {
    CWM_REQUIRE(m && n_vis_min >= 0 && n_vis_min <= m->st.n_tok, "cwm_model_set_ragged: n_vis_min must be 0 (rectangular batches) or a visible count up to %d",
                m ? m->st.n_tok : 0);
    m->ragged_min = n_vis_min;
    return CWM_OK;
}

extern "C" int cwm_model_set_option(cwm_model* m, const char* key, int value) {
    CWM_REQUIRE(m && key, "cwm_model_set_option: null argument");
    return m->eng.set_option("cwm_model_set_option", key, value);
}

extern "C" int cwm_timing_enable(cwm_model* m, int kclass, int enable) {
    CWM_REQUIRE(m, "cwm_timing_enable: null model");
    return m->eng.timing_enable(kclass, enable);
}

extern "C" int cwm_timing_collect(cwm_model* m, int kclass, cwm_kernel_stats* out) {
    CWM_REQUIRE(m, "cwm_timing_collect: null model");
    return m->eng.timing_collect(kclass, out);
}

namespace {
template <int PLANES>
__global__ void pad_split_rows_kernel(const float* src, int rows, int K, bf16* out, int Kpad) {
    const int64_t i = (int64_t)blockIdx.x * blockDim.x + threadIdx.x;
    if (i >= (int64_t)rows * Kpad) return;
    const int r = (int)(i / Kpad), k = (int)(i - (int64_t)r * Kpad);
    const float v = k < K ? src[(size_t)r * K + k] : 0.f;
    store_operand<PLANES>(out, r, Kpad, k, v);
}

__global__ void qkv_scatter_kernel(const float* qkv, int B, int N, int H, float scale, bf16* q, bf16* k, bf16* v_out, int64_t qk_plane) {
    const int64_t i = (int64_t)blockIdx.x * blockDim.x + threadIdx.x;
    const int D = H * 64;
    if (i >= (int64_t)B * N * 3 * D) return;
    const int c = (int)(i % (3 * D));
    const int64_t row = i / (3 * D);
    const int b = (int)(row / N), n = (int)(row - (int64_t)b * N);
    const int which = c / D, cc = c - which * D, h = cc / 64, d = cc - h * 64;
    float v = qkv[i];
    if (which == 0) v *= scale;
    bf16 hi, lo;
    split_bf16(v, hi, lo);
    bf16* dst = which == 0 ? q : which == 1 ? k : v_out;
    const size_t o = ((size_t)(b * H + h) * N + n) * 64 + d;
    dst[o] = hi;
    dst[o + qk_plane] = lo;
}

template <int PLANES>
__global__ void merge_planes_kernel(const bf16* in, float* out, int rows, int ld, int ld_in) {
    const int64_t i = (int64_t)blockIdx.x * blockDim.x + threadIdx.x;
    if (i >= (int64_t)rows * ld) return;
    const int r = (int)(i / ld), c = (int)(i - (int64_t)r * ld);
    const bf16* s = in + a_pos<PLANES>(r, ld_in, c);
    out[i] = (float)s[0] + (PLANES == 2 ? (float)s[kLoOffset] : 0.f);
}

__global__ void key_len_check_kernel(const int* key_len, int B, int N, int* bad) {
    const int b = blockIdx.x * blockDim.x + threadIdx.x;
    if (b < B && (key_len[b] < 1 || key_len[b] > N)) bad[0] = 1;
}

template <int PLANES>
__global__ void merge_planes_ragged_kernel(const bf16* in, float* out, int B, int N, int ld, const int* key_len, const int* bad) {
    const int64_t i = (int64_t)blockIdx.x * blockDim.x + threadIdx.x;
    if (i >= (int64_t)B * N * ld || bad[0]) return;
    const int r = (int)(i / ld), c = (int)(i - (int64_t)r * ld);
    const int b = r / N;
    if (r - b * N >= key_len[b]) return;
    const bf16* s = in + a_pos<PLANES>(r, ld, c);
    out[i] = (float)s[0] + (PLANES == 2 ? (float)s[kLoOffset] : 0.f);
}
}

int cwm::stage_linear_operands(Scratch& sc, const char* who, const float* a, const float* w, const float* bias, int M, int N, int K, int planes, hipStream_t s,
                               LinearOperands* out) {
    const int Kp = round_up(K, 64), Np = round_up(N, 256);
    out->Kp = Kp;
    out->Np = Np;
    out->A = sc.get<bf16>((size_t)2 * M * Kp);
    out->W = sc.get<bf16>((size_t)2 * Np * Kp);
    out->bias = sc.get<float>(Np, true);
    CWM_REQUIRE(out->A && out->W && out->bias, "%s: out of device memory", who);
    const unsigned gridA = (unsigned)(((int64_t)M * Kp + 255) / 256);
    if (planes == 2)
        hipLaunchKernelGGL(pad_split_rows_kernel<2>, dim3(gridA), dim3(256), 0, s, a, M, K, out->A, Kp);
    else
        hipLaunchKernelGGL(pad_split_rows_kernel<1>, dim3(gridA), dim3(256), 0, s, a, M, K, out->A, Kp);
    if (int rc = launch_pack_weight(w, N, K, planes == 1 ? out->W : nullptr, planes == 2 ? out->W : nullptr, Np, Kp, s)) return rc;
    if (bias) CWM_HIP_CHECK(hipMemcpyAsync(out->bias, bias, (size_t)N * sizeof(float), hipMemcpyDeviceToDevice, s));
    return 0;
}

int cwm::launch_qkv_scatter(const float* qkv, int B, int N, int H, float scale, bf16* q, bf16* k, bf16* v, int64_t qk_plane, hipStream_t s) {
    const int64_t total = (int64_t)B * N * 3 * H * 64;
    hipLaunchKernelGGL(qkv_scatter_kernel, dim3((unsigned)((total + 255) / 256)), dim3(256), 0, s, qkv, B, N, H, scale, q, k, v, qk_plane);
    CWM_HIP_CHECK(hipGetLastError());
    return 0;
}

extern "C" int cwm_split_bf16(const float* x_dev, int64_t n, void* hi_dev, void* lo_dev, void* stream) {
    CWM_REQUIRE(x_dev && hi_dev && n >= 0, "cwm_split_bf16: bad argument");
    return launch_split_bf16(x_dev, n, (bf16*)hi_dev, (bf16*)lo_dev, (hipStream_t)stream);
}

extern "C" int cwm_linear(const float* a_dev, const float* w_dev, const float* bias_dev, const float* resid_dev, float* c_dev, int M,
                          int N, int K, int gelu, int mode, void* stream) {
    CWM_REQUIRE(a_dev && w_dev && c_dev && M > 0 && N > 0 && K > 0, "cwm_linear: bad argument");
    CWM_REQUIRE(mode == CWM_MODE_FAST || mode == CWM_MODE_PARITY, "cwm_linear: bad mode");
    hipStream_t s = (hipStream_t)stream;
    const int planes = mode == CWM_MODE_PARITY ? 2 : 1;
    Scratch sc;
    LinearOperands op;
    if (int rc = stage_linear_operands(sc, "cwm_linear", a_dev, w_dev, bias_dev, M, N, K, planes, s, &op)) return rc;
    const int ldg = round_up(N, 32);
    bf16* G = gelu ? sc.get<bf16>((size_t)2 * M * ldg) : nullptr;
    CWM_REQUIRE(!gelu || G, "cwm_linear: out of device memory");
    GemmParams p;
    memset(&p, 0, sizeof(p));
    p.A = op.A; p.lda = op.Kp; p.W = op.W;
    p.M = M; p.N = N; p.K = op.Kp; p.bias = op.bias;
    if (gelu) {
        p.epi = EPI_BF16_GELU; p.out_hi = G; p.ldo = ldg;
    } else {
// ... 188 lines not shown
```

Before: 1932 frames/s.

## Precompute decoder-block-0 QKV for mask tokens into a cached table and gather

Decoder block 0 sees mask-token rows whose input is only mask_token plus a positional embedding, so their layernorm and QKV projection depend on position alone. This change computes them once per weight load into a per-position table. Each forward then runs layernorm and the QKV GEMM only on the visible rows and scatters the masked rows' Q/K/V from the table with a gather kernel. It also adds a half-height GEMM tile variant for the last M tile, to avoid wasted MFMA work on partial row blocks. The costs are extra persistent memory, a one-time table build, and new branches in the QKV validation and epilogue paths.

```diff
diff --git a/counterfactualworldmodels_amd/_lib.py b/counterfactualworldmodels_amd/_lib.py
--- a/counterfactualworldmodels_amd/_lib.py
+++ b/counterfactualworldmodels_amd/_lib.py
@@ -622,7 +622,7 @@
     "cwm_dev_unembed_ragged": (C.c_int, [C.c_void_p, C.c_void_p] + [C.c_int64] * 3 + [C.c_void_p] + [C.c_int] * 8 + [C.c_void_p, C.c_void_p]),
 }
 
-OPTION_KEYS = ("gemm_tile", "gemm_debug", "gemm_staged", "gemm_direct", "attn_kernel", "attn_remap", "attn_tail", "attn_ksplit", "prune_last_block", "index_fused",
+OPTION_KEYS = ("gemm_tile", "gemm_debug", "gemm_staged", "gemm_direct", "attn_kernel", "attn_remap", "attn_tail", "attn_ksplit", "prune_last_block", "mask_token_tables","index_fused",
                "min_lane_rows", "conj_ctx_stream", "conj_attn")
 GEMM_DEBUG_TIMING_ONLY = 1 | 2 | 8
 
diff --git a/counterfactualworldmodels_amd/csrc/dev.hip b/counterfactualworldmodels_amd/csrc/dev.hip
--- a/counterfactualworldmodels_amd/csrc/dev.hip
+++ b/counterfactualworldmodels_amd/csrc/dev.hip
@@ -601,9 +601,11 @@
         CWM_REQUIRE(!a.resid_rowmap || a.resid, "cwm_dev_gemm: a residual row map without a residual");
         p.C = a.C; p.ldc = a.ldc; p.resid = a.resid; p.ldr = a.ldr;
     } else if (a.epi == EPI_QKV) {
-        CWM_REQUIRE(a.q_out && a.k_out && a.v_out && a.heads > 0 && a.head_dim > 0 && a.n_tok > 0 && a.N == 3 * a.heads * a.head_dim && a.M % a.n_tok == 0,
-                    "cwm_dev_gemm: the Q/K/V scatter needs the three outputs, N = 3 * heads * head_dim and whole samples of n_tok rows");
-        CWM_REQUIRE(planes == 1 || a.qk_plane >= (int64_t)a.M * a.heads * a.head_dim, "cwm_dev_gemm: the lo plane would overlap the hi plane");
+        CWM_REQUIRE(a.q_out && a.k_out && a.v_out && a.heads > 0 && a.head_dim > 0 && a.n_tok > 0 && a.N == 3 * a.heads * a.head_dim &&
+                        (a.rows_in > 0 ? a.rows_in <= a.n_tok : a.M % a.n_tok == 0),
+                    "cwm_dev_gemm: the Q/K/V scatter needs the three outputs, N = 3 * heads * head_dim and whole samples of n_tok rows (or of their first rows_in)");
+        CWM_REQUIRE(planes == 1 || a.qk_plane >= (int64_t)(a.rows_in > 0 ? a.M / a.rows_in : a.M / a.n_tok) * a.n_tok * a.heads * a.head_dim,
+                    "cwm_dev_gemm: the lo plane would overlap the hi plane");
         p.q_out = (bf16*)a.q_out; p.k_out = (bf16*)a.k_out; p.v_out = (bf16*)a.v_out; p.qk_plane = a.qk_plane;
         p.qkv_dim = a.heads * a.head_dim; p.heads = a.heads; p.head_dim = a.head_dim; p.n_tok = a.n_tok; p.q_scale = a.q_scale;
     } else {
diff --git a/counterfactualworldmodels_amd/csrc/elementwise.hip b/counterfactualworldmodels_amd/csrc/elementwise.hip
--- a/counterfactualworldmodels_amd/csrc/elementwise.hip
+++ b/counterfactualworldmodels_amd/csrc/elementwise.hip
@@ -404,6 +404,63 @@
     if (total == 0) return 0;
     hipLaunchKernelGGL(fill_mask_tokens_ragged_kernel, dim3((unsigned)((total + 255) / 256)), dim3(256), 0, stream, x_full, mask_token, pos, perm, counts, Nt,
                        n_vis_min, D, total);
+    CWM_HIP_CHECK(hipGetLastError());
+    return 0;
+}
+
+__global__ __launch_bounds__(256) void dec0_gather_kernel(const bf16* tab, const int* perm, bf16* q, bf16* k, bf16* v, int64_t qk_plane, int Nt, int n_vis, int H,
+                                                          int planes, int64_t rows, int64_t rows_q) {
+    const int cpr = 3 * planes * H * 8;
+    const int64_t gid = (int64_t)blockIdx.x * blockDim.x + threadIdx.x;
+    if (gid >= rows_q * cpr) return;
+    const int64_t r0 = gid / cpr;
+    const int c = (int)(gid - r0 * cpr);
+    const int e = c & 7, h = (c >> 3) % H, wp = (c >> 3) / H;
+    const int which = wp / planes, pl = wp - which * planes;
+    const int nm = Nt - n_vis;
+    const bf16* src = tab + ((size_t)wp * H + h) * Nt * 64 + e * 8;
+    bf16* dst = (which == 0 ? q : which == 1 ? k : v) + (size_t)pl * qk_plane + e * 8;
+    constexpr int R = 4;
+    typedef __attribute__((ext_vector_type(4))) unsigned u32x4;
+    size_t orow[R];
+    int tau[R];
+    bool live[R];
+#pragma unroll
+    for (int i = 0; i < R; ++i) {
+        const int64_t row = r0 + i * rows_q;
+        live[i] = row < rows;
+        const int64_t rr = live[i] ? row : 0;
+        const int b = (int)(rr / nm), j = n_vis + (int)(rr - (int64_t)b * nm);
+        orow[i] = ((size_t)b * H + h) * Nt + j;
+        tau[i] = perm[(size_t)b * Nt + j];
+    }
+    u32x4 val[R];
+#pragma unroll
+    for (int i = 0; i < R; ++i) val[i] = *reinterpret_cast<const u32x4*>(src + (size_t)min(max(tau[i], 0), Nt - 1) * 64);
+#pragma unroll
+    for (int i = 0; i < R; ++i)
+        if (live[i]) *reinterpret_cast<u32x4*>(dst + orow[i] * 64) = val[i];
+}
+
+int launch_dec0_gather(const bf16* tab, const int* perm, bf16* q, bf16* k, bf16* v, int64_t qk_plane, int B, int Nt, int n_vis, int H, int planes, hipStream_t stream) {
+    CWM_REQUIRE(tab && perm && q && k && v && B > 0 && H > 0 && n_vis >= 0 && n_vis <= Nt && (planes == 1 || planes == 2) && qk_plane % 8 == 0,
+                "dec0_gather: bad argument");
+    const int64_t rows = (int64_t)B * (Nt - n_vis), rows_q = (rows + 3) / 4;
+    if (rows == 0) return 0;
+    const int64_t total = rows_q * 3 * planes * H * 8;
+    hipLaunchKernelGGL(dec0_gather_kernel, dim3((unsigned)((total + 255) / 256)), dim3(256), 0, stream, tab, perm, q, k, v, qk_plane, Nt, n_vis, H, planes, rows, rows_q);
+    CWM_HIP_CHECK(hipGetLastError());
+    return 0;
+}
+
+__global__ void iota_kernel(int* perm, int n) {
+    const int i = blockIdx.x * blockDim.x + threadIdx.x;
+    if (i < n) perm[i] = i;
+}
+
+int launch_iota(int* perm, int n, hipStream_t stream) {
+    CWM_REQUIRE(perm && n > 0, "iota: bad argument");
+    hipLaunchKernelGGL(iota_kernel, dim3((unsigned)((n + 255) / 256)), dim3(256), 0, stream, perm, n);
     CWM_HIP_CHECK(hipGetLastError());
     return 0;
 }
diff --git a/counterfactualworldmodels_amd/csrc/engine.h b/counterfactualworldmodels_amd/csrc/engine.h
--- a/counterfactualworldmodels_amd/csrc/engine.h
+++ b/counterfactualworldmodels_amd/csrc/engine.h
@@ -125,6 +125,12 @@
     uint64_t splitk_clock = 0;
     static constexpr size_t kMaxSplitKStreams = 8;
     std::map<hipStream_t, SplitKWs> splitk_ws;
+    struct Dec0Table {
+        bf16* qkv = nullptr;
+        uint64_t loads = 0;
+        bool built = false;
+    };
+    Dec0Table dec0_tab[2];
 
     ~Engine();
     int alloc(void** p, size_t bytes, bool zero, bool workspace);
@@ -153,7 +159,7 @@
     int require_weights(const char* fn);
     int set_option(const char* fn, const char* key, int value);
 
-    int run_gemm(const GemmParams& p, int planes, hipStream_t s);
+    int run_gemm(const GemmParams& p, int planes, hipStream_t s, bool book = true);
     int attach_splitk_workspace(GemmParams& p, hipStream_t s);
     int run_attention(const AttnParams& p, int planes, hipStream_t s);
     int run_layernorm(const LayerNormParams& p, int planes, hipStream_t s);
@@ -178,7 +184,8 @@
     int run_mlp(const float* ln_g, const float* ln_b, const LinearW& fc1, const LinearW& fc2, float* x, int B, int n_tok, int D, int planes, StreamBuffers& sb,
                 hipStream_t s, int n_keep = 0);
     int run_block(const BlockW& w, float* x, int B, int n_tok, int D, int H, int planes, StreamBuffers& sb, hipStream_t s, int n_keep = 0,
-                  const int* key_len = nullptr);
+                  const int* key_len = nullptr, const bf16* tab_rows = nullptr, int tab_vis = 0, const int* tab_perm = nullptr);
+    int dec0_table(const StreamW& S, int planes, float* x_tmp, bf16* h_tmp, int* perm_tmp, hipStream_t s, const bf16** tab);
     int run_block_small(const BlockW& w, float* x, int B, int n_tok, int D, int H, int planes, StreamBuffers& sb, hipStream_t s);
     int embed_stream(const StreamW& S, const StreamWs& w, int B, int n_vis, int planes, hipStream_t s);
     int to_decoder(const StreamW& S, const StreamWs& w, int B, int n_vis, int planes, hipStream_t s, const int* counts = nullptr, int n_vis_min = 0);
diff --git a/counterfactualworldmodels_amd/csrc/engine.hip b/counterfactualworldmodels_amd/csrc/engine.hip
--- a/counterfactualworldmodels_amd/csrc/engine.hip
+++ b/counterfactualworldmodels_amd/csrc/engine.hip
@@ -65,7 +65,7 @@
     typedef TuningField Field;
     static const Field fields[] = {{"gemm_tile", &Tuning::gemm_tile}, {"gemm_debug", &Tuning::gemm_debug}, {"gemm_staged", &Tuning::gemm_staged},
                                    {"gemm_direct", &Tuning::gemm_direct}, {"attn_kernel", &Tuning::attn_kernel}, {"attn_remap", &Tuning::attn_remap},
-                                   {"attn_tail", &Tuning::attn_tail}, {"attn_ksplit", &Tuning::attn_ksplit}, {"prune_last_block", &Tuning::prune_last_block}, {"index_fused", &Tuning::index_fused},
+                                   {"attn_tail", &Tuning::attn_tail}, {"attn_ksplit", &Tuning::attn_ksplit}, {"prune_last_block", &Tuning::prune_last_block}, {"mask_token_tables", &Tuning::mask_token_tables}, {"index_fused", &Tuning::index_fused},
                                    {"min_lane_rows", &Tuning::min_lane_rows}, {"conj_ctx_stream", &Tuning::conj_ctx_stream}, {"conj_attn", &Tuning::conj_attn}};
     for (const Field& f : fields)
         if (!strcmp(key, f.name)) return &f;
@@ -430,7 +430,7 @@
     return 0;
 }
 
-int Engine::run_gemm(const GemmParams& p_in, int planes, hipStream_t s) {
+int Engine::run_gemm(const GemmParams& p_in, int planes, hipStream_t s, bool book) {
     GemmParams p = p_in;
     p.overlapped = overlapped;
     p.tune = &tune;
@@ -440,8 +440,9 @@
         if (int rc = attach_splitk_workspace(p, s)) return rc;
     for (int i = 0; i < plan.nparts; ++i) {
         const GemmPlan::Part& part = plan.part[i];
-        EventPair* e;
-        if (int rc = timer_begin(CWM_KCLASS_GEMM, 2.0 * part.M * (double)p.N * p.K, s, &e)) return rc;
+        EventPair* e = nullptr;
+        if (book)
+            if (int rc = timer_begin(CWM_KCLASS_GEMM, 2.0 * part.M * (double)p.N * p.K, s, &e)) return rc;
         if (e) e->sub = part.kernel == GEMM_KERNEL_8PHASE ? CWM_KCLASS_GEMM_WIDE : CWM_KCLASS_GEMM_NARROW;
         if (int rc = launch_gemm_part(p, planes, plan, i, s)) return rc;
         if (int rc = timer_end(e, s)) return rc;
@@ -592,21 +593,31 @@
     return residual_gemm(*this, sb.gbuf, fc1.N, fc2, x, B, n_tok, kr, planes, s);
 }
 
-int Engine::run_block(const BlockW& w, float* x, int B, int n_tok, int D, int H, int planes, StreamBuffers& sb, hipStream_t s, int n_keep, const int* key_len) {
+int Engine::run_block(const BlockW& w, float* x, int B, int n_tok, int D, int H, int planes, StreamBuffers& sb, hipStream_t s, int n_keep, const int* key_len,
+                      const bf16* tab_rows, int tab_vis, const int* tab_perm) {
     const int M = B * n_tok;
     const int64_t hplane = (int64_t)M * D;
     const KeptRows kr(n_tok, n_keep);
+    const int n_in = tab_rows ? tab_vis : n_tok, Mi = B * n_in;
     int rc;
-    if ((rc = layernorm_to(x, M, D, w.ln1_g, w.ln1_b, sb.hbuf, planes, s))) return rc;
-
-    GemmParams g = gemm_base(sb.hbuf, D, w.qkv, M, planes);
+    LayerNormParams ln;
+    memset(&ln, 0, sizeof(ln));
+    ln.x = x; ln.ldx = D; ln.gamma = w.ln1_g; ln.beta = w.ln1_b; ln.eps = ln_eps; ln.D = D; ln.rows = Mi;
+    ln.out = sb.hbuf; ln.out_plane = (int64_t)Mi * D; ln.ldo = D;
+    if (tab_rows) { ln.rows_out_per_b = n_in; ln.rows_in_per_b = n_tok; ln.in_offset = 0; }
+    if ((rc = run_layernorm(ln, planes, s))) return rc;
+
+    GemmParams g = gemm_base(sb.hbuf, D, w.qkv, Mi, planes);
     g.epi = EPI_QKV;
-    g.rows_in = n_tok; g.rows_out = n_tok; g.map_stride = n_tok;
+    g.rows_in = n_in; g.rows_out = n_tok; g.map_stride = n_tok;
     g.q_out = sb.qbuf; g.k_out = sb.kbuf; g.v_out = sb.vbuf;
     g.qk_plane = hplane;
     g.qkv_dim = D; g.heads = H; g.head_dim = D / H; g.n_tok = n_tok;
-    g.q_scale = 1.0f / sqrtf((float)(D / H));
-    if ((rc = run_gemm(g, planes, s))) return rc;
+    g.q_scale = 1.0f / sqrtf((float)(D / H));    if ((rc = run_gemm(g, planes, s))) return rc;
+    if (tab_rows && (rc = timed(CWM_KCLASS_FILL_MASK, (double)B * (n_tok - n_in) * 3.0 * D * 2.0 * planes, s, [&] {
+                         return launch_dec0_gather(tab_rows, tab_perm, sb.qbuf, sb.kbuf, sb.vbuf, hplane, B, n_tok, n_in, H, planes, s);
+                     })))
+        return rc;
 
     AttnParams a;
     memset(&a, 0, sizeof(a));
@@ -665,6 +676,39 @@
     return run_fill_mask_tokens(w.x_dec, S.mask_token, S.pos_dec_ext, w.perm, B, next, n_vis, S.dec_dim, s);
 }
 
+int Engine::dec0_table(const StreamW& S, int planes, float* x_tmp, bf16* h_tmp, int* perm_tmp, hipStream_t s, const bf16** tab) {
+    Dec0Table& t = dec0_tab[planes - 1];
+    const int Nt = S.n_tok, D = S.dec_dim, H = S.dec_heads;
+    const int64_t plane = (int64_t)Nt * D;
+    if (!t.qkv) {
+        void* p = nullptr;
+        if (int rc = alloc(&p, (size_t)3 * planes * plane * sizeof(bf16), true, false)) return rc;
+        CWM_HIP_CHECK(hipDeviceSynchronize());
+        t.qkv = (bf16*)p;
+    }
+    *tab = t.qkv;
+    if (t.built && t.loads == loads) return 0;
+    const BlockW& w = S.dec[0];
+    int rc;
+    if ((rc = launch_iota(perm_tmp, Nt, s)) || (rc = launch_fill_mask_tokens(x_tmp, S.mask_token, S.pos_dec_ext, perm_tmp, 1, Nt, 0, D, s))) return rc;
+    LayerNormParams ln;
+    memset(&ln, 0, sizeof(ln));
+    ln.x = x_tmp; ln.ldx = D; ln.gamma = w.ln1_g; ln.beta = w.ln1_b; ln.eps = ln_eps; ln.D = D; ln.rows = Nt;
+    ln.out = h_tmp; ln.out_plane = plane; ln.ldo = D;
+    if ((rc = launch_layernorm(ln, planes, s))) return rc;
+    GemmParams g = gemm_base(h_tmp, D, w.qkv, Nt, planes);
+    g.epi = EPI_QKV;
+    g.rows_in = Nt; g.rows_out = Nt; g.map_stride = Nt;
+    g.q_out = t.qkv; g.k_out = t.qkv + planes * plane; g.v_out = t.qkv + 2 * planes * plane;
+    g.qk_plane = plane;
+    g.qkv_dim = D; g.heads = H; g.head_dim = D / H; g.n_tok = Nt;
+    g.q_scale = 1.0f / sqrtf((float)(D / H));
+    if ((rc = run_gemm(g, planes, s, false))) return rc;
+    t.built = true;
+    t.loads = loads;
+    return 0;
+}
+
 int Engine::head_rows(const StreamW& S, const StreamWs& w, int B, int n_out, float* out, int planes, hipStream_t s) {
     const int next = S.n_slots();
     LayerNormParams ln;
diff --git a/counterfactualworldmodels_amd/csrc/gemm.hip b/counterfactualworldmodels_amd/csrc/gemm.hip
--- a/counterfactualworldmodels_amd/csrc/gemm.hip
+++ b/counterfactualworldmodels_amd/csrc/gemm.hip
@@ -241,7 +241,8 @@
 }
 
 
-template <int PLANES, bool HALF>
+
+template <int PLANES, bool HALF, bool HALF_M = false>
 __device__ __forceinline__ void gemm8p_tile(const GemmParams& p, char* smem, int m0, int n0) {
     GEMM_PROF_BEGIN();
     constexpr int HALF_BYTES = 128 * 128;
@@ -335,7 +336,20 @@
     } while (0)
 
     const int nk = p.K / (64 / PLANES);
-    if constexpr (!HALF) {
+    static_assert(!(HALF && HALF_M), "a tile is half-width or half-height, not both");
+    if constexpr (HALF_M) {
+        stage(H_A0{}, 0, 0);
+        stage(H_W0{}, 0, 0);
+        stage(H_W1{}, 0, 0);
+        if (nk > 1) {
+            stage(H_A0{}, 1, 1);
+            stage(H_W0{}, 1, 1);
+            stage(H_W1{}, 1, 1);
+            asm volatile("s_waitcnt vmcnt(6)" ::: "memory");
+        } else {
+            asm volatile("s_waitcnt vmcnt(0)" ::: "memory");
+        }
+    } else if constexpr (!HALF) {
         stage(H_A0{}, 0, 0);
         stage(H_W0{}, 0, 0);
         stage(H_W1{}, 0, 0);
@@ -368,7 +382,8 @@
         const char* base = smem + buf * BUF_BYTES;
         read_w(base, 0, bw0);
         read_a(base, 0);
-        if (t + 1 < nk) stage(H_A1{}, buf ^ 1, t + 1);
+        if constexpr (!HALF_M)
+            if (t + 1 < nk) stage(H_A1{}, buf ^ 1, t + 1);
         CWM_PHASE_BARRIER();
         mfma_quadrant(acc[0][0], bw0);
         CWM_PHASE_BARRIER();
@@ -377,21 +392,24 @@
         CWM_PHASE_BARRIER();
         if constexpr (!HALF) mfma_quadrant(acc[0][1], bw1);
         CWM_PHASE_BARRIER();
-        read_a(base, 1);
+        if constexpr (!HALF_M) read_a(base, 1);
         if (t + 2 < nk) stage(H_W0{}, buf, t + 2);
         CWM_PHASE_BARRIER();
-        if constexpr (!HALF) mfma_quadrant(acc[1][1], bw1);
+        if constexpr (!HALF && !HALF_M) mfma_quadrant(acc[1][1], bw1);
         CWM_PHASE_BARRIER();
         if (t + 2 >= nk) {
             asm volatile("s_waitcnt vmcnt(0)" ::: "memory");
         } else if constexpr (HALF) {
             asm volatile("s_waitcnt vmcnt(4)" ::: "memory");
+        } else if constexpr (HALF_M) {
+            asm volatile("s_waitcnt vmcnt(4)" ::: "memory");
+            stage(H_W1{}, buf, t + 2);
         } else {
             stage(H_W1{}, buf, t + 2);
             asm volatile("s_waitcnt vmcnt(6)" ::: "memory");
         }
         CWM_PHASE_BARRIER();
-        mfma_quadrant(acc[1][0], bw0);
+        if constexpr (!HALF_M) mfma_quadrant(acc[1][0], bw0);
         CWM_PHASE_BARRIER();
     }
     if (wr == 0) CWM_PHASE_BARRIER();
@@ -416,6 +434,9 @@
         if constexpr (HALF)
             epilogue_direct<PLANES, 2>(
                 p, [&](int pi, int i, int j) { return acc[pi][0][i][j]; }, [&](int pi) { return pi * 128 + wr * 64; }, [&](int) { return n0 + wc * 32; }, tab, lane);
+        else if constexpr (HALF_M)
+            epilogue_direct<PLANES, 2>(
+                p, [&](int pi, int i, int j) { return acc[0][pi][i][j]; }, [&](int) { return wr * 64; }, [&](int pi) { return n0 + pi * 128 + wc * 32; }, tab, lane);
         else
             epilogue_direct<PLANES, 4>(
                 p, [&](int pi, int i, int j) { return acc[pi >> 1][pi & 1][i][j]; }, [&](int pi) { return (pi >> 1) * 128 + wr * 64; },
@@ -431,6 +452,10 @@
             epilogue_piece_seq<PLANES, 2>(
                 p, [&](int pi, int i, int j) { return acc[pi][0][i][j]; }, [&](int pi) { return pi * 128 + wr * 64; }, [&](int) { return n0 + wc * 32; },
                 smem + wave * 8192, tab, lane);
+        else if constexpr (HALF_M)
+            epilogue_piece_seq<PLANES, 2>(
+                p, [&](int pi, int i, int j) { return acc[0][pi][i][j]; }, [&](int) { return wr * 64; }, [&](int pi) { return n0 + pi * 128 + wc * 32; },
+                smem + wave * 8192, tab, lane);
         else
             epilogue_piece_seq<PLANES, 4>(
                 p, [&](int pi, int i, int j) { return acc[pi >> 1][pi & 1][i][j]; }, [&](int pi) { return (pi >> 1) * 128 + wr * 64; },
@@ -440,7 +465,7 @@
     }
     const int ncol = (lane >> 4) * 4;
 #pragma unroll
-    for (int qm = 0; qm < 2; ++qm)
+    for (int qm = 0; qm < (HALF_M ? 1 : 2); ++qm)
 #pragma unroll
         for (int i = 0; i < 4; ++i) {
             const int m = m0 + qm * 128 + wr * 64 + i * 16 + (lane & 15);
@@ -471,6 +496,7 @@
     const int in_g = id - g * group_sz;
     const int m0 = (first_m + (in_g % gm)) * 256, n0 = (in_g / gm) * 256;
     if (n0 + 128 >= p.N && !(p.debug & 1024)) gemm8p_tile<PLANES, true>(p, smem, m0, n0);
+    else if (m0 + 128 >= p.M && !(p.debug & 2048)) gemm8p_tile<PLANES, false, true>(p, smem, m0, n0);
     else gemm8p_tile<PLANES, false>(p, smem, m0, n0);
 }
 
@@ -505,7 +531,7 @@
     if (p.epi == EPI_F32) {
         CWM_REQUIRE(p.ldc % 4 == 0 && (!p.resid || p.ldr % 4 == 0), "gemm: ldc/ldr must be multiples of 4");
     } else if (p.epi == EPI_QKV) {
-        CWM_REQUIRE(p.rows_in == p.n_tok && p.N == 3 * p.qkv_dim && p.head_dim % 4 == 0, "gemm: bad QKV epilogue setup");
+        CWM_REQUIRE(p.rows_in > 0 && p.rows_in <= p.n_tok && p.N == 3 * p.qkv_dim && p.head_dim % 4 == 0, "gemm: bad QKV epilogue setup");
         CWM_REQUIRE(p.qkv_dim % 16 == 0, "gemm: QKV epilogue needs the model width (%d) to be a multiple of 16", p.qkv_dim);
     } else {
         CWM_REQUIRE(p.ldo % 4 == 0, "gemm: ldo must be a multiple of 4");
diff --git a/counterfactualworldmodels_amd/csrc/kernels.h b/counterfactualworldmodels_amd/csrc/kernels.h
--- a/counterfactualworldmodels_amd/csrc/kernels.h
+++ b/counterfactualworldmodels_amd/csrc/kernels.h
@@ -14,6 +14,7 @@
     int attn_ksplit = 1;
     int index_fused = 1;
     int prune_last_block = 1;
+    int mask_token_tables = 1;
     int min_lane_rows = 0;
     int conj_ctx_stream = 1;
     int conj_attn = 1;
@@ -172,6 +173,9 @@
 int launch_fill_mask_tokens(float* x_full, const float* mask_token, const float* pos, const int* perm, int B, int Nt, int n_vis, int D, hipStream_t stream);
 int launch_fill_mask_tokens_ragged(float* x_full, const float* mask_token, const float* pos, const int* perm, const int* counts, int B, int Nt, int n_vis_min,
                                    int D, hipStream_t stream);
+
+int launch_dec0_gather(const bf16* tab, const int* perm, bf16* q, bf16* k, bf16* v, int64_t qk_plane, int B, int Nt, int n_vis, int H, int planes, hipStream_t stream);
+int launch_iota(int* perm, int n, hipStream_t stream);
 
 struct UnembedParams {
     const float* y;
diff --git a/counterfactualworldmodels_amd/csrc/model.hip b/counterfactualworldmodels_amd/csrc/model.hip
--- a/counterfactualworldmodels_amd/csrc/model.hip
+++ b/counterfactualworldmodels_amd/csrc/model.hip
@@ -94,7 +94,7 @@
 extern "C" int cwm_model_missing_weights(cwm_model* m, char* buf, int buflen) { return m->eng.missing_weights(buf, buflen); }
 
 
-static int forward_lane(cwm_model* m, const cwm_forward_args* a, int b0, int B, ModelWs lw, hipStream_t s, int stage_lo, int stage_hi) {
+static int forward_lane(cwm_model* m, const cwm_forward_args* a, int b0, int B, ModelWs lw, hipStream_t s, int stage_lo, int stage_hi, const bf16* dec0_tab) {
     const cwm_config& c = m->cfg;
     const StreamW& S = m->st;
     StreamWs& w = lw.st;
@@ -137,7 +137,8 @@
     const bool pruned = Nm > 0 && E.tune.prune_last_block;
     for (int i = 0; i < c.dec_depth; ++i) {
         const int keep = (i == c.dec_depth - 1 && pruned) ? Nm : 0;
-        if (in_range(st_e2d + 1 + i) && (rc = E.run_block(S.dec[i], w.x_dec, B, Nt, S.dec_dim, S.dec_heads, planes, w.sb, s, keep))) return rc;
+        const bf16* tab = i == 0 ? dec0_tab : nullptr;
+        if (in_range(st_e2d + 1 + i) && (rc = E.run_block(S.dec[i], w.x_dec, B, Nt, S.dec_dim, S.dec_heads, planes, w.sb, s, keep, nullptr, tab, Nv, w.perm))) return rc;
     }
     if (!in_range(st_head)) return CWM_OK;
     if ((rc = E.head_rows(S, w, B, Nret, y_tokens, planes, s))) return rc;
@@ -175,6 +176,9 @@
     if (int rc = m->eng.require_weights("cwm_forward")) return rc;
     if (int rc = ensure_workspace(m, B, Nv)) return rc;
     hipStream_t s = (hipStream_t)a->stream;
+    const bf16* dec0_tab = nullptr;
+    if (m->eng.tune.mask_token_tables && Nm > 0 && m->ragged_min == 0)
+        if (int rc = m->eng.dec0_table(m->st, a->mode == CWM_MODE_PARITY ? 2 : 1, m->ws.st.x_dec, m->ws.st.sb.hbuf, m->ws.st.perm, s, &dec0_tab)) return rc;
 
     const int min_rows = m->eng.tune.min_lane_rows > 0 ? m->eng.tune.min_lane_rows : kMinLaneRows;
     int n_lanes = 1;
@@ -187,7 +191,7 @@
     const int n_stages = c.enc_depth + c.dec_depth + 3;
     for (int st = 0; st < n_stages && !rc; ++st)
         for (int l = 0; l < n_lanes && !rc; ++l)
-            rc = forward_lane(m, a, first[l], first[l + 1] - first[l], lane_ws(m, first[l]), m->lane_set.stream(l, s), st, st + 1);
+            rc = forward_lane(m, a, first[l], first[l + 1] - first[l], lane_ws(m, first[l]), m->lane_set.stream(l, s), st, st + 1, dec0_tab);
     m->eng.overlapped = 0;
     if (int jrc = m->lane_set.join(s)) return jrc;
     if (rc) return rc;
```

New measurement: 1952 frames/s (median of 6 runs). 1.01x the previous value.
